# mfathulkr/MA-CJD-Cooperative-Jamming-Decision-Making-via-MARL

Hardware: AMD Instinct MI355X
Metric: env-steps/sec (all GPUs; batch_envs=4096/GPU, 3j/4r) (higher is better)
Workload: dtype f64; 1 GPU; 3 jammers / 4 radars, batch_envs=4096 per GPU, GRU hidden=64; mode=train, hidden=64, train_batch_episodes=32, updates_per_graph=20, hip_graphs=True, gemm_tuning=True, replay_capacity_episodes=8192, mixer_dtype=fp32, mixer=one MFMA launch per direction (f32)

## Files before the change

include/macjd_nets.h:

```cpp
#ifndef MACJD_NETS_H
#define MACJD_NETS_H

#include <stdint.h>

#include "macjd.h"

#ifdef __cplusplus
extern "C" {
#endif

typedef struct macjd_qhead_io {
    int64_t n_rows;
    int32_t H, A, n_agents, greedy_only;
    const float* base;  int64_t base_ld;
    const float* P_all; int64_t p_ld;
    const float* W1;    int64_t w1_ld;
    const float* w2;
    const float* b2;
    float* Q;           int64_t q_ld;
    const void* avail;  int32_t avail_elem_size, reserved;
    int64_t av_se, av_sj, av_sa;
    float epsilon;      float reserved2;
    uint64_t seed, counter;
    const float* eps_dev;
    const uint64_t* counter_dev;
    int32_t* T_out32;
    int64_t* T_out64;
    int64_t t32_se, t32_sj, t64_se, t64_sj;
    float* P_out;       int64_t po_se, po_sj;
    int64_t* argmax_out;
    const int64_t* gather_idx;
    float* q_gather_out;
} macjd_qhead_io;

int macjd_qhead_select(const macjd_qhead_io* io, void* hip_stream);

typedef struct macjd_gru_io {
    int32_t n_nets, B, T, J, H, reserved;
    const float* gi[2];
    const float* w_hh[2];
    const float* b_hh[2];
    const float* h0[2];
    float* h_out[2];
    int64_t h0_sb[2];
    const float* obs;      int64_t obs_sb, obs_sj;   int32_t S, reserved2;
    const int64_t* obs_index;
    const float* fc1_w[2]; const float* fc1_b[2];
    const float* w_ih[2];  const float* b_ih[2];
    float* p_out[2];
    const float* act_w[2][3]; const float* act_b[2][3];
    int32_t Ah, A;
} macjd_gru_io;

int macjd_gru_sequence(const macjd_gru_io* io, void* hip_stream);

typedef struct macjd_mixer_io {
    int64_t M;
    int32_t J, Em;
    const float* q;
    const float* w1_raw;
    const float* b1_raw;
    const float* wf_raw;
    const float* v_raw;
    float* y;
    const float* gy;
    float* gq;
    float* gw1_raw;
    float* gb1_raw;
    float* gwf_raw;
    float* gv_raw;
    int64_t b1_ld;
} macjd_mixer_io;

int macjd_mixer_tail_forward(const macjd_mixer_io* io, void* hip_stream);
int macjd_mixer_tail_backward(const macjd_mixer_io* io, void* hip_stream);

typedef struct macjd_tdloss_io {
    int32_t B, Tm1;
    float gamma, reserved;
    const float* y;
    const float* tq;
    int64_t y_sb, tq_sb;
    int64_t gy_sb, gy_cols;
    const float* reward;       int64_t r_sb, r_st;
    const uint8_t* terminated; int64_t t_sb, t_st;
    const uint8_t* filled;     int64_t f_sb, f_st;
    float* stats;
    float* gy;
} macjd_tdloss_io;

int macjd_td_loss(const macjd_tdloss_io* io, void* hip_stream);
int macjd_td_mask_sum(const macjd_tdloss_io* io, float* out, void* hip_stream);

typedef struct macjd_adam_io {
    int64_t n;
    float lr, beta1, beta2, eps, max_norm, reserved;
    float* param; float* grad ; float* exp_avg; float* exp_avg_sq;
    float* step; float* grad_norm; float* partials;
} macjd_adam_io;

int macjd_clip_adam_step(const macjd_adam_io* io, void* hip_stream);

typedef struct macjd_sampler_io {
    int64_t* idx_out;
    int32_t n, reserved;
    const int32_t* n_stored;
    int64_t* counter;
    uint64_t seed;
} macjd_sampler_io;

int macjd_sample_episodes(const macjd_sampler_io* io, void* hip_stream);
int macjd_clip_adam_step_sample(const macjd_adam_io* io, const macjd_sampler_io* next, void* hip_stream);

typedef struct macjd_wgrad_io {
    int64_t K;
    int32_t M, N;
    const float* gout; int64_t gout_ld;
    const float* inp;  int64_t inp_ld;
    float* dW;         int64_t dw_ld;
    float* db;
    float* workspace;
    const float* outer_vec;
    const float* outer_w;
} macjd_wgrad_io;

int64_t macjd_linear_wgrad_workspace_floats(int64_t K, int32_t M, int32_t N);
int macjd_linear_wgrad(const macjd_wgrad_io* io, void* hip_stream);
#define MACJD_WGRAD_MAX_BATCH 8
int macjd_linear_wgrad_many(const macjd_wgrad_io* ios, int32_t n, void* hip_stream);

typedef struct macjd_gather_io {
    int32_t n_tensors, n_rows;
    const int64_t* idx;
    const void* src[8]; void* dst[8]; int64_t row_bytes[8];
    int64_t dst_row_bytes[8];
} macjd_gather_io;

int macjd_gather_rows(const macjd_gather_io* io, void* hip_stream);

typedef struct macjd_qinput_io {
    int64_t n_rows;
    int32_t H, A;
    const float* h;   int64_t h_ld;
    const void* idx;  int32_t idx_elem_size, reserved;
    const float* P;
    float* out;       int64_t out_ld;
} macjd_qinput_io;

int macjd_qhead_input(const macjd_qinput_io* io, void* hip_stream);

typedef struct macjd_qtaken_io {
    int64_t n_rows;
    int32_t H, A;
    const float* h;   int64_t h_ld;
    const void* idx;  int32_t idx_elem_size, reserved;
    const float* P;
    const float* W1;  int64_t w1_ld;
    const float* b1;  const float* w2;  const float* b2;
    float* x;         int64_t x_ld;
    float* act;       int64_t act_ld;
    float* q;
} macjd_qtaken_io;

int macjd_qhead_taken_supported(int32_t H, int32_t A);
int macjd_qhead_taken(const macjd_qtaken_io* io, void* hip_stream);

typedef struct macjd_layernorm_io {
    int64_t M;
    int32_t S, reserved;
    float eps, reserved2;
    const float* x;  int64_t x_ld;
    const float* gamma;
    const float* beta;
    float* y;        int64_t y_ld;
    float* mean;
    float* rstd;
    float* xhat;     int64_t xhat_ld;
} macjd_layernorm_io;

int macjd_layernorm_forward(const macjd_layernorm_io* io, void* hip_stream);

typedef struct macjd_lnparam_io {
    int32_t C, K;
    const float* W;   int64_t w_ld;
    const float* G;   int64_t g_ld;
    const float* gb;
    float* dgamma;
    float* dbeta;
} macjd_lnparam_io;

int macjd_layernorm_param_grad(const macjd_lnparam_io* io, void* hip_stream);
int macjd_clip_adam_step_ln(const macjd_adam_io* io, const macjd_sampler_io* next, const macjd_lnparam_io* ln,
                            int64_t gamma_off, int64_t beta_off, void* hip_stream);

#define MACJD_ACT_NONE 0
#define MACJD_ACT_RELU 1
#define MACJD_ACT_SIGMOID 2
typedef struct macjd_mlp_io {
    int64_t n_rows;
    int32_t n_layers;
    int32_t dims[4];
    int32_t act[3];
    const float* W[3];
    const float* b[3];
    const float* x;  int64_t x_ld;
    float* y;        int64_t y_ld;
} macjd_mlp_io;

int macjd_mlp_forward(const macjd_mlp_io* io, void* hip_stream);
int macjd_mlp_forward_pair(const macjd_mlp_io* io0, const macjd_mlp_io* io1, void* hip_stream);

typedef struct macjd_splitrelu_bwd_io {
    int64_t M;
    int32_t n_blocks, Cp;
    int32_t width[4];
    const float* g[4];  int64_t g_ld[4];
    const float* g_pass; int64_t gp_ld;
    const float* act;   int64_t act_ld;
    float* gout;        int64_t gout_ld;
    const float* outer_w[4];
} macjd_splitrelu_bwd_io;

int macjd_splitrelu_backward(const macjd_splitrelu_bwd_io* io, void* hip_stream);

typedef struct macjd_rowdot_io {
    int64_t n_rows;
    int32_t K, reserved;
    const float* x;  int64_t x_ld;
    const float* w;
    const float* b;
    float* y;
} macjd_rowdot_io;

int macjd_rowdot(const macjd_rowdot_io* io, void* hip_stream);

typedef struct macjd_grugates_io {
    int64_t n_rows;
    int32_t H, reserved;
    const float* gi;  int64_t gi_ld;
    const float* gh;  int64_t gh_ld;
    const float* h;   int64_t h_ld;
    float* h_out;     int64_t ho_ld;
    float* h_out2;    int64_t ho2_ld;
} macjd_grugates_io;

int macjd_gru_gates(const macjd_grugates_io* io, void* hip_stream);

typedef struct macjd_mixerf_io {
    int64_t M;
    int32_t J, S, Hh, Em;
    int32_t save;
    int32_t operand_dtype;
    float ln_eps;  float reserved_f;
    const float* s;   int64_t s_ld;
    const float* q;
    const float* ln_w; const float* ln_b;
    const float* W1; const float* b1;
    const float* W2; const float* b2;
    const float* Wf2; const float* bf2;
    const float* wV2; const float* bV2;
    float* y;
    float* sn; float* xhat;
    float* act;
    const float* gy;
    float* gq;
    float* gout1;
    float* g_w1raw;
    float* g_wfraw;
    float* g_v;
} macjd_mixerf_io;

int macjd_mixer_fused_supported(int32_t J, int32_t S, int32_t Hh, int32_t Em);
int macjd_mixer_fused_forward(const macjd_mixerf_io* io, void* hip_stream);
int macjd_mixer_fused_forward_pair(const macjd_mixerf_io* saved, const macjd_mixerf_io* plain, void* hip_stream);
int macjd_mixer_fused_backward(const macjd_mixerf_io* io, void* hip_stream);
int macjd_mixer_fused_backward_td(const macjd_mixerf_io* io, const macjd_tdloss_io* td, const float* tot_m, void* hip_stream);
int macjd_mixer_fused_train(const macjd_mixerf_io* eval, const macjd_mixerf_io* target, const macjd_tdloss_io* td,
                            const float* tot_m, void* hip_stream);
typedef struct macjd_mixer_static_io {
    int64_t n_tiles;
    float* sn; float* xhat;
    float* act;
    float* gout1_sum;
    float* g_w1raw_sum;
    float* g_wfraw_sum;
    float* g_v_sum;
} macjd_mixer_static_io;
int macjd_mixer_fused_train_static(const macjd_mixerf_io* eval, const macjd_mixerf_io* target, const macjd_tdloss_io* td,
                                   const float* tot_m, const macjd_mixer_static_io* st, void* hip_stream);

typedef struct macjd_agent_episode_io {
// ... 98 lines not shown
```

ma-cjd-cooperative-jamming-decision-making-via-marl_amd/_native.py:

```python
from __future__ import annotations

import ctypes
import os
from typing import Optional

_PKG_DIR = os.path.dirname(os.path.abspath(__file__))
LIB_NAME = "libmacjd_hip.so"
LIB_PATH = os.environ.get("MACJD_LIB") or os.path.join(_PKG_DIR, LIB_NAME)

ABI_VERSION = 7
STEP_ARITH_F64 = 1
STEP_LANE_KERNEL = 2
STEP_SLOT_KERNEL = 4

EXPORTS = [
    "macjd_abi_version", "macjd_last_error", "macjd_reload_options", "macjd_device_count",
    "macjd_scenario_create", "macjd_scenario_destroy", "macjd_scenario_dims", "macjd_scenario_is_regular",
    "macjd_env_reset", "macjd_env_step", "macjd_env_step_timed",
    "macjd_qhead_select", "macjd_gru_sequence", "macjd_mixer_tail_forward", "macjd_mixer_tail_backward",
    "macjd_mlp_forward", "macjd_mlp_forward_pair", "macjd_td_loss", "macjd_clip_adam_step", "macjd_clip_adam_step_sample", "macjd_clip_adam_step_ln", "macjd_sample_episodes", "macjd_gather_rows",
    "macjd_linear_wgrad", "macjd_linear_wgrad_workspace_floats", "macjd_linear_wgrad_many", "macjd_qhead_input", "macjd_layernorm_forward", "macjd_layernorm_param_grad", "macjd_gru_gates", "macjd_rowdot", "macjd_splitrelu_backward",
    "macjd_mixer_fused_supported", "macjd_mixer_fused_forward", "macjd_mixer_fused_backward", "macjd_mixer_fused_backward_td", "macjd_td_mask_sum",
    "macjd_agent_episode_supported", "macjd_agent_episode", "macjd_env_step_many", "macjd_env_step_many_timed",
    "macjd_qhead_double_q_supported", "macjd_qhead_double_q", "macjd_qhead_taken_supported", "macjd_qhead_taken",
    "macjd_qheads_pair", "macjd_mixer_fused_forward_pair", "macjd_mixer_fused_train", "macjd_mixer_fused_train_static",
    "macjd_scenario_set_scan", "macjd_env_step_scan", "macjd_env_reset_scan",
    "macjd_agent_env_episode_scan_supported", "macjd_agent_env_episode_scan",
    "macjd_scenario_set_scan_pattern",
    "macjd_gru_sequence_backward_supported", "macjd_gru_sequence_backward",
]


class NativeLibraryError(RuntimeError):
    pass


class StepIO(ctypes.Structure):
    _fields_ = [
        ("n_envs", ctypes.c_int64), ("env_offset", ctypes.c_int64), ("seed", ctypes.c_uint64),
        ("flags", ctypes.c_uint32), ("reserved", ctypes.c_uint32),
        ("T", ctypes.c_void_p), ("T_se", ctypes.c_int64), ("T_sx", ctypes.c_int64),
        ("P32", ctypes.c_void_p), ("P64", ctypes.c_void_p), ("P_se", ctypes.c_int64), ("P_sx", ctypes.c_int64),
        ("u", ctypes.c_void_p), ("u_se", ctypes.c_int64), ("u_sx", ctypes.c_int64),
        ("episode", ctypes.c_void_p),
        ("track", ctypes.c_void_p), ("k_se", ctypes.c_int64), ("k_sx", ctypes.c_int64),
        ("step", ctypes.c_void_p),
        ("reward", ctypes.c_void_p), ("r_dpj", ctypes.c_void_p), ("terminated", ctypes.c_void_p),
        ("pd", ctypes.c_void_p), ("pd_se", ctypes.c_int64), ("pd_sx", ctypes.c_int64),
        ("snr_with", ctypes.c_void_p), ("sw_se", ctypes.c_int64), ("sw_sx", ctypes.c_int64),
        ("out64", ctypes.c_void_p), ("pd64", ctypes.c_void_p), ("snr64", ctypes.c_void_p),
        ("prj64", ctypes.c_void_p),
        ("pe_tables", ctypes.c_void_p), ("pe_flags", ctypes.c_void_p), ("pe_stride", ctypes.c_int64),
        ("pe_tile", ctypes.c_int32), ("reserved_pe", ctypes.c_int32),
        ("r_dpj_sum", ctypes.c_void_p),
    ]


class ScanDesc(ctypes.Structure):
    _fields_ = [
        ("n_radars", ctypes.c_int32), ("n_jammers", ctypes.c_int32),
        ("half_beam", ctypes.c_void_p), ("sweep", ctypes.c_void_p), ("sweep_mod", ctypes.c_void_p),
        ("full", ctypes.c_void_p), ("az0", ctypes.c_void_p), ("bear_tgt", ctypes.c_void_p), ("bear_jam", ctypes.c_void_p),
        ("GaPs_side", ctypes.c_void_p), ("snr_no", ctypes.c_void_p), ("snr_no_side", ctypes.c_void_p),
        ("pd_no_side", ctypes.c_void_p), ("gr_side", ctypes.c_void_p),
    ]


class ScanPatternDesc(ctypes.Structure):
    _fields_ = [
        ("n_radars", ctypes.c_int32), ("n_levels", ctypes.c_int32),
        ("inv_width", ctypes.c_void_p), ("GaPs_lvl", ctypes.c_void_p), ("snr_no_lvl", ctypes.c_void_p),
        ("pd_no_lvl", ctypes.c_void_p), ("gr_lvl", ctypes.c_void_p),
    ]


class ScanIO(ctypes.Structure):
    _fields_ = [
        ("theta_a", ctypes.c_void_p), ("a_se", ctypes.c_int64), ("a_sx", ctypes.c_int64),
        ("state", ctypes.c_void_p), ("st_se", ctypes.c_int64), ("st_col0", ctypes.c_int32), ("st_col_step", ctypes.c_int32),
        ("snr_no", ctypes.c_void_p), ("sn_se", ctypes.c_int64), ("sn_sx", ctypes.c_int64),
    ]


class QheadIO(ctypes.Structure):
    _fields_ = [
        ("n_rows", ctypes.c_int64),
        ("H", ctypes.c_int32), ("A", ctypes.c_int32), ("n_agents", ctypes.c_int32), ("greedy_only", ctypes.c_int32),
        ("base", ctypes.c_void_p), ("base_ld", ctypes.c_int64),
        ("P_all", ctypes.c_void_p), ("p_ld", ctypes.c_int64),
        ("W1", ctypes.c_void_p), ("w1_ld", ctypes.c_int64),
        ("w2", ctypes.c_void_p), ("b2", ctypes.c_void_p),
        ("Q", ctypes.c_void_p), ("q_ld", ctypes.c_int64),
        ("avail", ctypes.c_void_p), ("avail_elem_size", ctypes.c_int32), ("reserved", ctypes.c_int32),
        ("av_se", ctypes.c_int64), ("av_sj", ctypes.c_int64), ("av_sa", ctypes.c_int64),
        ("epsilon", ctypes.c_float), ("reserved2", ctypes.c_float),
        ("seed", ctypes.c_uint64), ("counter", ctypes.c_uint64),
        ("eps_dev", ctypes.c_void_p), ("counter_dev", ctypes.c_void_p),
        ("T_out32", ctypes.c_void_p), ("T_out64", ctypes.c_void_p),
        ("t32_se", ctypes.c_int64), ("t32_sj", ctypes.c_int64), ("t64_se", ctypes.c_int64), ("t64_sj", ctypes.c_int64),
        ("P_out", ctypes.c_void_p), ("po_se", ctypes.c_int64), ("po_sj", ctypes.c_int64),
        ("argmax_out", ctypes.c_void_p), ("gather_idx", ctypes.c_void_p), ("q_gather_out", ctypes.c_void_p),
    ]


class GruIO(ctypes.Structure):
    _fields_ = [
        ("n_nets", ctypes.c_int32), ("B", ctypes.c_int32), ("T", ctypes.c_int32), ("J", ctypes.c_int32),
        ("H", ctypes.c_int32), ("reserved", ctypes.c_int32),
        ("gi", ctypes.c_void_p * 2), ("w_hh", ctypes.c_void_p * 2), ("b_hh", ctypes.c_void_p * 2),
        ("h0", ctypes.c_void_p * 2), ("h_out", ctypes.c_void_p * 2), ("h0_sb", ctypes.c_int64 * 2),
        ("obs", ctypes.c_void_p), ("obs_sb", ctypes.c_int64), ("obs_sj", ctypes.c_int64), ("S", ctypes.c_int32), ("reserved2", ctypes.c_int32),
        ("obs_index", ctypes.c_void_p),
        ("fc1_w", ctypes.c_void_p * 2), ("fc1_b", ctypes.c_void_p * 2), ("w_ih", ctypes.c_void_p * 2), ("b_ih", ctypes.c_void_p * 2),
        ("p_out", ctypes.c_void_p * 2), ("act_w", (ctypes.c_void_p * 3) * 2), ("act_b", (ctypes.c_void_p * 3) * 2),
        ("Ah", ctypes.c_int32), ("A", ctypes.c_int32),
    ]


class GruBwdIO(ctypes.Structure):
    _fields_ = [
        ("B", ctypes.c_int32), ("T", ctypes.c_int32), ("J", ctypes.c_int32), ("H", ctypes.c_int32),
        ("gi", ctypes.c_void_p), ("gh", ctypes.c_void_p), ("h_all", ctypes.c_void_p),
        ("h0", ctypes.c_void_p), ("h0_sb", ctypes.c_int64),
        ("w_hh", ctypes.c_void_p), ("dh_all", ctypes.c_void_p),
        ("dgi", ctypes.c_void_p), ("dgh", ctypes.c_void_p), ("dh0", ctypes.c_void_p),
    ]


class MixerIO(ctypes.Structure):
    _fields_ = [
        ("M", ctypes.c_int64), ("J", ctypes.c_int32), ("Em", ctypes.c_int32),
        ("q", ctypes.c_void_p), ("w1_raw", ctypes.c_void_p), ("b1_raw", ctypes.c_void_p),
        ("wf_raw", ctypes.c_void_p), ("v_raw", ctypes.c_void_p), ("y", ctypes.c_void_p),
        ("gy", ctypes.c_void_p), ("gq", ctypes.c_void_p), ("gw1_raw", ctypes.c_void_p),
        ("gb1_raw", ctypes.c_void_p), ("gwf_raw", ctypes.c_void_p), ("gv_raw", ctypes.c_void_p),
        ("b1_ld", ctypes.c_int64),
    ]


class MixerFusedIO(ctypes.Structure):
    _fields_ = [
        ("M", ctypes.c_int64), ("J", ctypes.c_int32), ("S", ctypes.c_int32), ("Hh", ctypes.c_int32), ("Em", ctypes.c_int32),
        ("save", ctypes.c_int32), ("operand_dtype", ctypes.c_int32), ("ln_eps", ctypes.c_float), ("reserved_f", ctypes.c_float),
        ("s", ctypes.c_void_p), ("s_ld", ctypes.c_int64), ("q", ctypes.c_void_p),
        ("ln_w", ctypes.c_void_p), ("ln_b", ctypes.c_void_p), ("W1", ctypes.c_void_p), ("b1", ctypes.c_void_p),
        ("W2", ctypes.c_void_p), ("b2", ctypes.c_void_p), ("Wf2", ctypes.c_void_p), ("bf2", ctypes.c_void_p),
        ("wV2", ctypes.c_void_p), ("bV2", ctypes.c_void_p),
        ("y", ctypes.c_void_p), ("sn", ctypes.c_void_p), ("xhat", ctypes.c_void_p), ("act", ctypes.c_void_p),
        ("gy", ctypes.c_void_p), ("gq", ctypes.c_void_p), ("gout1", ctypes.c_void_p), ("g_w1raw", ctypes.c_void_p),
        ("g_wfraw", ctypes.c_void_p), ("g_v", ctypes.c_void_p),
    ]


class MixerStaticIO(ctypes.Structure):
    _fields_ = [
        ("n_tiles", ctypes.c_int64), ("sn", ctypes.c_void_p), ("xhat", ctypes.c_void_p), ("act", ctypes.c_void_p),
        ("gout1_sum", ctypes.c_void_p), ("g_w1raw_sum", ctypes.c_void_p), ("g_wfraw_sum", ctypes.c_void_p),
        ("g_v_sum", ctypes.c_void_p),
    ]


class AgentEpisodeIO(ctypes.Structure):
    _fields_ = [
        ("n_envs", ctypes.c_int64), ("T", ctypes.c_int32), ("J", ctypes.c_int32), ("H", ctypes.c_int32), ("A", ctypes.c_int32),
        ("greedy_only", ctypes.c_int32), ("reserved", ctypes.c_int32),
        ("gi", ctypes.c_void_p), ("gi_ld", ctypes.c_int64), ("P_all", ctypes.c_void_p), ("p_ld", ctypes.c_int64),
        ("h0", ctypes.c_void_p), ("w_hh", ctypes.c_void_p), ("b_hh", ctypes.c_void_p),
        ("W1", ctypes.c_void_p), ("w1_ld", ctypes.c_int64), ("b1", ctypes.c_void_p), ("w2", ctypes.c_void_p), ("b2", ctypes.c_void_p),
        ("avail", ctypes.c_void_p), ("avail_elem_size", ctypes.c_int32), ("reserved2", ctypes.c_int32),
        ("av_se", ctypes.c_int64), ("av_sj", ctypes.c_int64), ("av_sa", ctypes.c_int64),
        ("eps", ctypes.c_void_p), ("seed", ctypes.c_uint64), ("counter_base", ctypes.c_void_p),
        ("hidden", ctypes.c_void_p), ("T_out", ctypes.c_void_p), ("P_out", ctypes.c_void_p), ("h_final", ctypes.c_void_p),
    ]


class AgentEnvEpisodeScanIO(ctypes.Structure):
    _fields_ = [
        ("n_envs", ctypes.c_int64), ("env_offset", ctypes.c_int64),
        ("T", ctypes.c_int32), ("J", ctypes.c_int32), ("R", ctypes.c_int32), ("H", ctypes.c_int32), ("A", ctypes.c_int32),
        ("S", ctypes.c_int32), ("actor_hidden", ctypes.c_int32), ("greedy_only", ctypes.c_int32),
        ("h0", ctypes.c_void_p), ("fc1_w", ctypes.c_void_p), ("fc1_b", ctypes.c_void_p),
        ("w_ih", ctypes.c_void_p), ("b_ih", ctypes.c_void_p), ("w_hh", ctypes.c_void_p), ("b_hh", ctypes.c_void_p),
        ("a1_w", ctypes.c_void_p), ("a1_b", ctypes.c_void_p), ("a2_w", ctypes.c_void_p), ("a2_b", ctypes.c_void_p),
        ("a3_w", ctypes.c_void_p), ("a3_b", ctypes.c_void_p),
        ("W1", ctypes.c_void_p), ("w1_ld", ctypes.c_int64), ("b1", ctypes.c_void_p), ("w2", ctypes.c_void_p), ("b2", ctypes.c_void_p),
        ("avail", ctypes.c_void_p), ("avail_elem_size", ctypes.c_int32), ("reserved", ctypes.c_int32),
        ("av_se", ctypes.c_int64), ("av_sj", ctypes.c_int64), ("av_sa", ctypes.c_int64),
        ("eps", ctypes.c_void_p), ("seed", ctypes.c_uint64), ("counter_base", ctypes.c_void_p),
        ("env_seed", ctypes.c_uint64), ("episode", ctypes.c_void_p),
        ("track", ctypes.c_void_p), ("k_se", ctypes.c_int64), ("k_sx", ctypes.c_int64), ("step", ctypes.c_void_p),
        ("scan", ScanIO), ("pe_tables", ctypes.c_void_p),
        ("hidden", ctypes.c_void_p), ("T_out", ctypes.c_void_p), ("P_out", ctypes.c_void_p), ("h_final", ctypes.c_void_p),
        ("st_state", ctypes.c_void_p), ("st_obs", ctypes.c_void_p), ("reward", ctypes.c_void_p), ("terminated", ctypes.c_void_p),
        ("rdpj_sum", ctypes.c_void_p),
    ]


class DoubleQIO(ctypes.Structure):
    _fields_ = [
        ("n_rows", ctypes.c_int64), ("H", ctypes.c_int32), ("A", ctypes.c_int32),
        ("h_e", ctypes.c_void_p), ("he_ld", ctypes.c_int64), ("h_t", ctypes.c_void_p), ("ht_ld", ctypes.c_int64),
        ("P_e", ctypes.c_void_p), ("pe_ld", ctypes.c_int64), ("P_t", ctypes.c_void_p), ("pt_ld", ctypes.c_int64),
        ("W1_e", ctypes.c_void_p), ("w1e_ld", ctypes.c_int64), ("b1_e", ctypes.c_void_p), ("w2_e", ctypes.c_void_p), ("b2_e", ctypes.c_void_p),
        ("W1_t", ctypes.c_void_p), ("w1t_ld", ctypes.c_int64), ("b1_t", ctypes.c_void_p), ("w2_t", ctypes.c_void_p), ("b2_t", ctypes.c_void_p),
        ("out", ctypes.c_void_p), ("argmax_out", ctypes.c_void_p), ("p_group", ctypes.c_int64), ("p_inner", ctypes.c_int64),
    ]


class QinputIO(ctypes.Structure):
    _fields_ = [
        ("n_rows", ctypes.c_int64), ("H", ctypes.c_int32), ("A", ctypes.c_int32),
        ("h", ctypes.c_void_p), ("h_ld", ctypes.c_int64),
        ("idx", ctypes.c_void_p), ("idx_elem_size", ctypes.c_int32), ("reserved", ctypes.c_int32),
        ("P", ctypes.c_void_p), ("out", ctypes.c_void_p), ("out_ld", ctypes.c_int64),
    ]


class GruGatesIO(ctypes.Structure):
    _fields_ = [
        ("n_rows", ctypes.c_int64), ("H", ctypes.c_int32), ("reserved", ctypes.c_int32),
        ("gi", ctypes.c_void_p), ("gi_ld", ctypes.c_int64), ("gh", ctypes.c_void_p), ("gh_ld", ctypes.c_int64),
        ("h", ctypes.c_void_p), ("h_ld", ctypes.c_int64),
        ("h_out", ctypes.c_void_p), ("ho_ld", ctypes.c_int64), ("h_out2", ctypes.c_void_p), ("ho2_ld", ctypes.c_int64),
    ]


class RowdotIO(ctypes.Structure):
    _fields_ = [
        ("n_rows", ctypes.c_int64), ("K", ctypes.c_int32), ("reserved", ctypes.c_int32),
        ("x", ctypes.c_void_p), ("x_ld", ctypes.c_int64), ("w", ctypes.c_void_p), ("b", ctypes.c_void_p),
        ("y", ctypes.c_void_p),
    ]


class SplitReluBwdIO(ctypes.Structure):
    _fields_ = [
        ("M", ctypes.c_int64), ("n_blocks", ctypes.c_int32), ("Cp", ctypes.c_int32), ("width", ctypes.c_int32 * 4),
        ("g0", ctypes.c_void_p), ("g1", ctypes.c_void_p), ("g2", ctypes.c_void_p), ("g3", ctypes.c_void_p),
        ("g_ld", ctypes.c_int64 * 4),
        ("g_pass", ctypes.c_void_p), ("gp_ld", ctypes.c_int64),
        ("act", ctypes.c_void_p), ("act_ld", ctypes.c_int64), ("gout", ctypes.c_void_p), ("gout_ld", ctypes.c_int64),
        ("ow0", ctypes.c_void_p), ("ow1", ctypes.c_void_p), ("ow2", ctypes.c_void_p), ("ow3", ctypes.c_void_p),
    ]


class LayerNormIO(ctypes.Structure):
    _fields_ = [
        ("M", ctypes.c_int64), ("S", ctypes.c_int32), ("reserved", ctypes.c_int32),
        ("eps", ctypes.c_float), ("reserved2", ctypes.c_float),
        ("x", ctypes.c_void_p), ("x_ld", ctypes.c_int64), ("gamma", ctypes.c_void_p), ("beta", ctypes.c_void_p),
        ("y", ctypes.c_void_p), ("y_ld", ctypes.c_int64), ("mean", ctypes.c_void_p), ("rstd", ctypes.c_void_p),
        ("xhat", ctypes.c_void_p), ("xhat_ld", ctypes.c_int64),
    ]


class LnParamIO(ctypes.Structure):
    _fields_ = [
        ("C", ctypes.c_int32), ("K", ctypes.c_int32),
        ("W", ctypes.c_void_p), ("w_ld", ctypes.c_int64), ("G", ctypes.c_void_p), ("g_ld", ctypes.c_int64),
        ("gb", ctypes.c_void_p), ("dgamma", ctypes.c_void_p), ("dbeta", ctypes.c_void_p),
    ]


class MlpIO(ctypes.Structure):
    _fields_ = [
        ("n_rows", ctypes.c_int64), ("n_layers", ctypes.c_int32), ("dims", ctypes.c_int32 * 4),
        ("act", ctypes.c_int32 * 3), ("W", ctypes.c_void_p * 3), ("b", ctypes.c_void_p * 3),
        ("x", ctypes.c_void_p), ("x_ld", ctypes.c_int64), ("y", ctypes.c_void_p), ("y_ld", ctypes.c_int64),
    ]


class TdLossIO(ctypes.Structure):
    _fields_ = [
        ("B", ctypes.c_int32), ("Tm1", ctypes.c_int32), ("gamma", ctypes.c_float), ("reserved", ctypes.c_float),
        ("y", ctypes.c_void_p), ("tq", ctypes.c_void_p),
        ("y_sb", ctypes.c_int64), ("tq_sb", ctypes.c_int64), ("gy_sb", ctypes.c_int64), ("gy_cols", ctypes.c_int64),
        ("reward", ctypes.c_void_p), ("r_sb", ctypes.c_int64), ("r_st", ctypes.c_int64),
        ("terminated", ctypes.c_void_p), ("t_sb", ctypes.c_int64), ("t_st", ctypes.c_int64),
        ("filled", ctypes.c_void_p), ("f_sb", ctypes.c_int64), ("f_st", ctypes.c_int64),
        ("stats", ctypes.c_void_p), ("gy", ctypes.c_void_p),
    ]


class AdamIO(ctypes.Structure):
    _fields_ = [
        ("n", ctypes.c_int64), ("lr", ctypes.c_float), ("beta1", ctypes.c_float), ("beta2", ctypes.c_float),
        ("eps", ctypes.c_float), ("max_norm", ctypes.c_float), ("reserved", ctypes.c_float),
        ("param", ctypes.c_void_p), ("grad", ctypes.c_void_p), ("exp_avg", ctypes.c_void_p),
        ("exp_avg_sq", ctypes.c_void_p), ("step", ctypes.c_void_p), ("grad_norm", ctypes.c_void_p),
        ("partials", ctypes.c_void_p),
    ]


class QtakenIO(ctypes.Structure):
    _fields_ = [
        ("n_rows", ctypes.c_int64), ("H", ctypes.c_int32), ("A", ctypes.c_int32),
        ("h", ctypes.c_void_p), ("h_ld", ctypes.c_int64),
        ("idx", ctypes.c_void_p), ("idx_elem_size", ctypes.c_int32), ("reserved", ctypes.c_int32),
        ("P", ctypes.c_void_p),
        ("W1", ctypes.c_void_p), ("w1_ld", ctypes.c_int64),
        ("b1", ctypes.c_void_p), ("w2", ctypes.c_void_p), ("b2", ctypes.c_void_p),
        ("x", ctypes.c_void_p), ("x_ld", ctypes.c_int64),
        ("act", ctypes.c_void_p), ("act_ld", ctypes.c_int64),
        ("q", ctypes.c_void_p),
    ]


class SamplerIO(ctypes.Structure):
    _fields_ = [
        ("idx_out", ctypes.c_void_p), ("n", ctypes.c_int32), ("reserved", ctypes.c_int32),
        ("n_stored", ctypes.c_void_p), ("counter", ctypes.c_void_p), ("seed", ctypes.c_uint64),
    ]


class GatherIO(ctypes.Structure):
    _fields_ = [
        ("n_tensors", ctypes.c_int32), ("n_rows", ctypes.c_int32), ("idx", ctypes.c_void_p),
        ("src", ctypes.c_void_p * 8), ("dst", ctypes.c_void_p * 8), ("row_bytes", ctypes.c_int64 * 8),
        ("dst_row_bytes", ctypes.c_int64 * 8),
    ]


class WgradIO(ctypes.Structure):
    _fields_ = [
        ("K", ctypes.c_int64), ("M", ctypes.c_int32), ("N", ctypes.c_int32),
        ("gout", ctypes.c_void_p), ("gout_ld", ctypes.c_int64), ("inp", ctypes.c_void_p), ("inp_ld", ctypes.c_int64),
        ("dW", ctypes.c_void_p), ("dw_ld", ctypes.c_int64), ("db", ctypes.c_void_p), ("workspace", ctypes.c_void_p),
        ("outer_vec", ctypes.c_void_p), ("outer_w", ctypes.c_void_p),
    ]


_lib: Optional[ctypes.CDLL] = None


def load() -> ctypes.CDLL:
    global _lib
    if _lib is not None:
        return _lib
    if not os.path.exists(LIB_PATH):
        raise NativeLibraryError(
            f"{LIB_PATH} not found. Build it with `python -c 'import __graft_entry__ as g; g.build()'` "
            f"(hipcc --offload-arch=gfx950). There is no CPU fallback for the environment step.")
    try:
        lib = ctypes.CDLL(LIB_PATH)
    except OSError as e:
        raise NativeLibraryError(f"cannot load {LIB_PATH}: {e}") from e
    lib.macjd_abi_version.restype = ctypes.c_int
    lib.macjd_last_error.restype = ctypes.c_char_p
    lib.macjd_device_count.restype = ctypes.c_int
    lib.macjd_reload_options.restype = None
    lib.macjd_scenario_create.restype = ctypes.c_int
    lib.macjd_scenario_create.argtypes = [ctypes.c_void_p, ctypes.POINTER(ctypes.c_void_p)]
    lib.macjd_scenario_destroy.restype = None
    lib.macjd_scenario_destroy.argtypes = [ctypes.c_void_p]
    lib.macjd_scenario_is_regular.restype = ctypes.c_int
    lib.macjd_scenario_is_regular.argtypes = [ctypes.c_void_p]
    lib.macjd_scenario_dims.restype = ctypes.c_int
    lib.macjd_scenario_dims.argtypes = [ctypes.c_void_p] + [ctypes.POINTER(ctypes.c_int32)] * 3
    lib.macjd_env_reset.restype = ctypes.c_int
    lib.macjd_env_reset.argtypes = [ctypes.c_void_p, ctypes.c_int64, ctypes.c_void_p, ctypes.c_int64, ctypes.c_int64,
                                    ctypes.c_void_p, ctypes.c_void_p, ctypes.c_void_p, ctypes.c_void_p]
    lib.macjd_env_step.restype = ctypes.c_int
    lib.macjd_scenario_set_scan.restype = ctypes.c_int
    lib.macjd_scenario_set_scan.argtypes = [ctypes.c_void_p, ctypes.POINTER(ScanDesc)]
    lib.macjd_scenario_set_scan_pattern.restype = ctypes.c_int
    lib.macjd_scenario_set_scan_pattern.argtypes = [ctypes.c_void_p, ctypes.POINTER(ScanPatternDesc)]
    lib.macjd_env_step_scan.restype = ctypes.c_int
    lib.macjd_env_step_scan.argtypes = [ctypes.c_void_p, ctypes.POINTER(StepIO), ctypes.POINTER(ScanIO), ctypes.c_void_p]
    lib.macjd_env_reset_scan.restype = ctypes.c_int
    lib.macjd_env_reset_scan.argtypes = [ctypes.c_void_p, ctypes.c_int64, ctypes.POINTER(ScanIO), ctypes.c_void_p, ctypes.c_void_p]
    lib.macjd_env_step.argtypes = [ctypes.c_void_p, ctypes.POINTER(StepIO), ctypes.c_void_p]
    lib.macjd_env_step_timed.restype = ctypes.c_int
    lib.macjd_env_step_timed.argtypes = [ctypes.c_void_p, ctypes.POINTER(StepIO), ctypes.c_int, ctypes.c_void_p,
                                         ctypes.POINTER(ctypes.c_float)]
    lib.macjd_qhead_select.restype = ctypes.c_int
    lib.macjd_qhead_select.argtypes = [ctypes.POINTER(QheadIO), ctypes.c_void_p]
    lib.macjd_gru_sequence.restype = ctypes.c_int
    lib.macjd_gru_sequence.argtypes = [ctypes.POINTER(GruIO), ctypes.c_void_p]
    lib.macjd_gru_sequence_backward_supported.restype = ctypes.c_int
    lib.macjd_gru_sequence_backward_supported.argtypes = [ctypes.c_int32]
    lib.macjd_gru_sequence_backward.restype = ctypes.c_int
    lib.macjd_gru_sequence_backward.argtypes = [ctypes.POINTER(GruBwdIO), ctypes.c_void_p]
    for name in ("macjd_mixer_tail_forward", "macjd_mixer_tail_backward"):
        getattr(lib, name).restype = ctypes.c_int
        getattr(lib, name).argtypes = [ctypes.POINTER(MixerIO), ctypes.c_void_p]
    lib.macjd_qhead_double_q_supported.restype = ctypes.c_int
    lib.macjd_qhead_double_q_supported.argtypes = [ctypes.c_int32] * 2
    lib.macjd_qhead_double_q.restype = ctypes.c_int
    lib.macjd_qhead_double_q.argtypes = [ctypes.POINTER(DoubleQIO), ctypes.c_void_p]
    lib.macjd_agent_episode_supported.restype = ctypes.c_int
    lib.macjd_agent_episode_supported.argtypes = [ctypes.c_int32] * 3
    lib.macjd_agent_episode.restype = ctypes.c_int
    lib.macjd_agent_episode.argtypes = [ctypes.POINTER(AgentEpisodeIO), ctypes.c_void_p]
    lib.macjd_agent_env_episode_scan_supported.restype = ctypes.c_int
    lib.macjd_agent_env_episode_scan_supported.argtypes = [ctypes.c_int32] * 4
    lib.macjd_agent_env_episode_scan.restype = ctypes.c_int
    lib.macjd_agent_env_episode_scan.argtypes = [ctypes.c_void_p, ctypes.POINTER(AgentEnvEpisodeScanIO), ctypes.c_void_p]
    lib.macjd_env_step_many.restype = ctypes.c_int
    lib.macjd_env_step_many.argtypes = [ctypes.c_void_p, ctypes.POINTER(StepIO), ctypes.c_int32, ctypes.c_int64, ctypes.c_void_p]
    lib.macjd_env_step_many_timed.restype = ctypes.c_int
    lib.macjd_env_step_many_timed.argtypes = [ctypes.c_void_p, ctypes.POINTER(StepIO), ctypes.c_int32, ctypes.c_int64, ctypes.c_int,
                                              ctypes.c_void_p, ctypes.POINTER(ctypes.c_float)]
    lib.macjd_mixer_fused_supported.restype = ctypes.c_int
    lib.macjd_mixer_fused_supported.argtypes = [ctypes.c_int32] * 4
    for name in ("macjd_mixer_fused_forward", "macjd_mixer_fused_backward"):
        getattr(lib, name).restype = ctypes.c_int
        getattr(lib, name).argtypes = [ctypes.POINTER(MixerFusedIO), ctypes.c_void_p]
    lib.macjd_mixer_fused_backward_td.restype = ctypes.c_int
    lib.macjd_mixer_fused_backward_td.argtypes = [ctypes.POINTER(MixerFusedIO), ctypes.POINTER(TdLossIO), ctypes.c_void_p, ctypes.c_void_p]
    lib.macjd_mixer_fused_train.restype = ctypes.c_int
    lib.macjd_mixer_fused_train.argtypes = [ctypes.POINTER(MixerFusedIO), ctypes.POINTER(MixerFusedIO), ctypes.POINTER(TdLossIO),
                                            ctypes.c_void_p, ctypes.c_void_p]
    lib.macjd_mixer_fused_train_static.restype = ctypes.c_int
    lib.macjd_mixer_fused_train_static.argtypes = [ctypes.POINTER(MixerFusedIO), ctypes.POINTER(MixerFusedIO), ctypes.POINTER(TdLossIO),
                                                   ctypes.c_void_p, ctypes.POINTER(MixerStaticIO), ctypes.c_void_p]
    lib.macjd_td_mask_sum.restype = ctypes.c_int
    lib.macjd_td_mask_sum.argtypes = [ctypes.POINTER(TdLossIO), ctypes.c_void_p, ctypes.c_void_p]
    lib.macjd_qhead_taken_supported.restype = ctypes.c_int
    lib.macjd_qhead_taken_supported.argtypes = [ctypes.c_int32, ctypes.c_int32]
    lib.macjd_qhead_taken.restype = ctypes.c_int
    lib.macjd_qhead_taken.argtypes = [ctypes.POINTER(QtakenIO), ctypes.c_void_p]
    lib.macjd_qheads_pair.restype = ctypes.c_int
    lib.macjd_qheads_pair.argtypes = [ctypes.POINTER(QtakenIO), ctypes.POINTER(DoubleQIO), ctypes.c_void_p]
    lib.macjd_mixer_fused_forward_pair.restype = ctypes.c_int
    lib.macjd_mixer_fused_forward_pair.argtypes = [ctypes.POINTER(MixerFusedIO), ctypes.POINTER(MixerFusedIO), ctypes.c_void_p]
    lib.macjd_qhead_input.restype = ctypes.c_int
    lib.macjd_qhead_input.argtypes = [ctypes.POINTER(QinputIO), ctypes.c_void_p]
    lib.macjd_layernorm_forward.restype = ctypes.c_int
    lib.macjd_layernorm_forward.argtypes = [ctypes.POINTER(LayerNormIO), ctypes.c_void_p]
    lib.macjd_gru_gates.restype = ctypes.c_int
    lib.macjd_gru_gates.argtypes = [ctypes.POINTER(GruGatesIO), ctypes.c_void_p]
    lib.macjd_splitrelu_backward.restype = ctypes.c_int
    lib.macjd_splitrelu_backward.argtypes = [ctypes.POINTER(SplitReluBwdIO), ctypes.c_void_p]
    lib.macjd_layernorm_param_grad.restype = ctypes.c_int
    lib.macjd_layernorm_param_grad.argtypes = [ctypes.POINTER(LnParamIO), ctypes.c_void_p]
    lib.macjd_rowdot.restype = ctypes.c_int
    lib.macjd_rowdot.argtypes = [ctypes.POINTER(RowdotIO), ctypes.c_void_p]
    lib.macjd_mlp_forward_pair.restype = ctypes.c_int
    lib.macjd_mlp_forward_pair.argtypes = [ctypes.POINTER(MlpIO), ctypes.POINTER(MlpIO), ctypes.c_void_p]
    lib.macjd_mlp_forward.restype = ctypes.c_int
    lib.macjd_mlp_forward.argtypes = [ctypes.POINTER(MlpIO), ctypes.c_void_p]
    lib.macjd_td_loss.restype = ctypes.c_int
    lib.macjd_td_loss.argtypes = [ctypes.POINTER(TdLossIO), ctypes.c_void_p]
    lib.macjd_clip_adam_step.restype = ctypes.c_int
    lib.macjd_clip_adam_step.argtypes = [ctypes.POINTER(AdamIO), ctypes.c_void_p]
    lib.macjd_clip_adam_step_sample.restype = ctypes.c_int
    lib.macjd_clip_adam_step_sample.argtypes = [ctypes.POINTER(AdamIO), ctypes.POINTER(SamplerIO), ctypes.c_void_p]
    lib.macjd_clip_adam_step_ln.restype = ctypes.c_int
    lib.macjd_clip_adam_step_ln.argtypes = [ctypes.POINTER(AdamIO), ctypes.POINTER(SamplerIO), ctypes.POINTER(LnParamIO),
                                            ctypes.c_int64, ctypes.c_int64, ctypes.c_void_p]
    lib.macjd_sample_episodes.restype = ctypes.c_int
    lib.macjd_sample_episodes.argtypes = [ctypes.POINTER(SamplerIO), ctypes.c_void_p]
    lib.macjd_gather_rows.restype = ctypes.c_int
    lib.macjd_gather_rows.argtypes = [ctypes.POINTER(GatherIO), ctypes.c_void_p]
    lib.macjd_linear_wgrad.restype = ctypes.c_int
    lib.macjd_linear_wgrad.argtypes = [ctypes.POINTER(WgradIO), ctypes.c_void_p]
    lib.macjd_linear_wgrad_many.restype = ctypes.c_int
    lib.macjd_linear_wgrad_many.argtypes = [ctypes.POINTER(WgradIO), ctypes.c_int32, ctypes.c_void_p]
    lib.macjd_linear_wgrad_workspace_floats.restype = ctypes.c_int64
    lib.macjd_linear_wgrad_workspace_floats.argtypes = [ctypes.c_int64, ctypes.c_int32, ctypes.c_int32]
    if lib.macjd_abi_version() != ABI_VERSION:
        raise NativeLibraryError(f"{LIB_NAME}: ABI version {lib.macjd_abi_version()} != expected {ABI_VERSION}")
    _lib = lib
    return lib


def reload_options() -> None:
    load().macjd_reload_options()


def check(rc: int, what: str) -> None:
    if rc != 0:
        msg = load().macjd_last_error()
        raise NativeLibraryError(f"{what} failed ({rc}): {msg.decode() if msg else ''}")


class ScenarioHandle:

    def __init__(self, scenario):
        lib = load()
        desc, keep = scenario.c_desc()
        h = ctypes.c_void_p()
        check(lib.macjd_scenario_create(ctypes.addressof(desc), ctypes.byref(h)), "macjd_scenario_create")
        del keep
        self._h = h
        self._lib = lib
        if getattr(scenario, "scanning", False):
            sdesc, skeep = scenario.c_scan_desc()
            check(lib.macjd_scenario_set_scan(h, ctypes.byref(sdesc)), "macjd_scenario_set_scan")
            del skeep
            if getattr(scenario, "scan_pattern_levels", 0):
                pdesc, pkeep = scenario.c_scan_pattern_desc()
                check(lib.macjd_scenario_set_scan_pattern(h, ctypes.byref(pdesc)), "macjd_scenario_set_scan_pattern")
                del pkeep

    @property
    def ptr(self):
        return self._h

    def close(self):
        if getattr(self, "_h", None):
            self._lib.macjd_scenario_destroy(self._h)
            self._h = None

    def __del__(self):
        try:
            self.close()
        except Exception:
            pass
```

ma-cjd-cooperative-jamming-decision-making-via-marl_amd/core/qmix.py:

```python
from __future__ import annotations

import copy
import os

import numpy as np
import torch
import torch.nn.functional as F
import torch.optim as optim

from .. import hipgraph, ops, options
from .networks import QMixer


def _to(x, dtype, device):
    if isinstance(x, torch.Tensor):
        return x.to(device=device, dtype=dtype)
    return torch.as_tensor(np.asarray(x), device=device).to(dtype)


class QMixLearner:
    def __init__(self, mac, args):
        self.args = args
        self.mac = mac
        self.n_agents = args.n_agents
# ... 479 lines not shown
            if side_work is not None:
                side_work()
            if sums_late is not None:
                sums_late()
            if stats_done is not None:
                torch.cuda.current_stream(eval_q_tot.device).wait_event(stats_done)
                for t_ in (self._last_stats4,):
                    t_.record_stream(torch.cuda.current_stream(eval_q_tot.device))
        else:
            loss, eval_mean, target_mean = ops.td_loss_full(eval_q_tot, target_q_tot, st["reward"], st["terminated"],
                                                            st["filled"], self.args.gamma, T - 1, 1)
            loss.backward()
        if self._world_size() > 1 or self._flat_param is not None:
            self._flatten_grads()
        return loss.detach(), eval_mean.detach(), target_mean.detach()

    def _clip_and_step(self, sample_next=None):
        if self._flat_param is not None:
            g = self.optimizer.param_groups[0]
            held, self._held_ln = getattr(self, "_held_ln", None), None
            ops.clip_adam_step(self._flat_param, self._flat_grad, self._flat_exp_avg, self._flat_exp_avg_sq,
                               self._adam_step, self._grad_norm, self._adam_partials, g["lr"], g["betas"], g["eps"],
                               self.args.grad_norm_clip, sample_next=sample_next, lnparam=held)
            return self._grad_norm
        grad_norm = torch.nn.utils.clip_grad_norm_(self.params, self.args.grad_norm_clip)
        self.optimizer.step()
        return grad_norm.detach() if torch.is_tensor(grad_norm) else torch.as_tensor(grad_norm)

    def _after_step(self):
        if (self.train_step - self.last_target_update_step) >= self.args.target_update_interval:
            self._update_targets()
            self.last_target_update_step = self.train_step

    def _pack_stats(self, loss, grad_norm, ev, tg, sync_stats):
        stats = {"loss": loss, "grad_norm": grad_norm, "eval_qtot_avg": ev, "target_qtot_avg": tg}
        if sync_stats:
            stacked = torch.stack([torch.as_tensor(v, device=self.device, dtype=torch.float32).reshape(())
                                   for v in stats.values()])
            stats = dict(zip(stats.keys(), stacked.tolist()))
        return stats

    def train(self, batch, train_info=None, sync_stats=True):
        self.train_step += 1
        loss, ev, tg = self._forward_backward(batch, int(batch["max_seq_len"]))
        self._allreduce_grads()
        grad_norm = self._clip_and_step()
        if self.train_agent_body:
            for m in (self.mac, self.target_mac):
                m.invalidate_static_inputs()
        self._after_step()
        if not sync_stats and torch.is_tensor(grad_norm) and grad_norm is self._grad_norm_tensor():
            grad_norm = grad_norm.clone()
        return self._pack_stats(loss, grad_norm, ev, tg, sync_stats)

    def _grad_norm_tensor(self):
        return getattr(self, "_grad_norm", None)

    def enable_graphs(self, buffer, batch_size, warmup_iters=3, force_two_graphs=False, updates_per_graph=None,
                      graphed_allreduce=None, prime=True):
        if self.device.type != "cuda":
            raise RuntimeError("enable_graphs needs the learner on a HIP device")
        if self.train_agent_body:
            raise RuntimeError("enable_graphs: train_agent_body is an eager-mode option (the captured, static-observation "
                               "and shared-body updates are built on the frozen agent body); use train()")
        self.release_graphs()
        self._verify_body_shared()
        same_buffer = getattr(self, "_g_buffer", None) is buffer
        self._g_buffer, self._g_B, self._g_T = buffer, int(batch_size), int(buffer.episode_limit)
        self._g_obs_static = bool(getattr(buffer, "obs_static", False)) and options.on("LEARNER_STATIC_OBS")
        self._g_state_static = self._g_obs_static and bool(getattr(buffer, "state_static", False))
        self._g_mixer_static = False
        self._g_actor_in_scan = options.on("ACTOR_IN_SCAN")
        self._g_scan_from_ring = self._g_obs_static and int(buffer.buffers["obs"].shape[-1]) <= 3 * int(self.args.rnn_hidden_dim)
        prev_idx = getattr(self, "_g_idx", None)
        keep_idx = same_buffer and prev_idx is not None and prev_idx.numel() == self._g_B and prev_idx.device == self.device
        self._g_idx = prev_idx if keep_idx else torch.zeros(self._g_B, dtype=torch.int64, device=self.device)
        self._g_dev_sampler = self._flat_param is not None and options.on("DEVICE_SAMPLER")
        if not keep_idx:
            self._g_n_stored = torch.zeros(1, dtype=torch.int32, device=self.device)
        if getattr(self, "_g_draws", None) is None:
            self._g_draws = torch.full((1,), int(getattr(self, "_resume_draws", 0)), dtype=torch.int64, device=self.device)
        if not keep_idx:
            self._g_pop_seen = None
            self._g_idx_fresh = False
        self._g_idx_ring = [(torch.zeros(self._g_B, dtype=torch.int64).pin_memory(), torch.cuda.Event()) for _ in range(8)]
        if buffer.current_size < 1:
            raise RuntimeError("enable_graphs: the replay buffer is empty")

        keys = [k for k in buffer.buffers if k != "avail_actions"]
        srcs = [buffer.buffers[k] for k in keys]
        fused = ops.gather_rows_supported(srcs) and self._g_T >= 2
        if fused:
            T1 = self._g_T + 1
            padded = ("actions_discrete", "actions_continuous")
            stage = {k: torch.zeros((self._g_B, T1 if k in padded else v.shape[1]) + tuple(v.shape[2:]), dtype=v.dtype,
                                    device=v.device) for k, v in zip(keys, srcs)}

        def body_a():
            if fused:
                pre = (None, None)
                if self._g_scan_from_ring and options.get("UPDATE_STREAMS") != "1":
                    pre = self._scan_from_ring_early()
                ops.gather_rows(self._g_idx, srcs, [stage[k] for k in keys])
                return self._forward_backward_full(stage, self._g_T, pre_scan=pre[0], pre_actor=pre[1])
            b = {k: v.index_select(0, self._g_idx) for k, v in zip(keys, srcs)}
            return self._forward_backward(b, self._g_T, validate_actions=False)

        self._graph_body_a = body_a

        was_shared = self._body_is_shared()
        snap_p = [p.detach().clone() for p in self.params]
        snap_o = {id(p): {k: v.clone() for k, v in st.items() if torch.is_tensor(v)}
                  for p, st in self.optimizer.state.items()}
        s = torch.cuda.Stream(device=self.device)
        s.wait_stream(torch.cuda.current_stream(self.device))
        with torch.cuda.stream(s):
            for _ in range(max(1, warmup_iters)):
                body_a()
                self._clip_and_step()
        torch.cuda.current_stream(self.device).wait_stream(s)
        def restore_training_state():
            with torch.no_grad():
                for p, sp in zip(self.params, snap_p):
                    p.copy_(sp)
                for p, st in self.optimizer.state.items():
                    for k, v in st.items():
                        if torch.is_tensor(v):
                            old = snap_o.get(id(p), {}).get(k)
                            v.copy_(old) if old is not None else v.zero_()
            if was_shared:
                self._mark_body_shared()

        restore_training_state()
        self._graph_a, self._graph_b = torch.cuda.CUDAGraph(), torch.cuda.CUDAGraph()
        self._g_graphed_ar = bool(graphed_allreduce if graphed_allreduce is not None
                                  else options.get("GRAPHED_ALLREDUCE") == "1") and self._ar_capturable()
        self._g_single = (self._world_size() <= 1 and not force_two_graphs) or self._g_graphed_ar
        with hipgraph.capture(self._graph_a):
            self._g_out_a = body_a()
            st4 = getattr(self, "_last_stats4", None) if fused else None
            if st4 is not None and st4.numel() == 4:
                self._grad_norm = st4[3]
            self._g_stats4 = st4 if (st4 is not None and st4.numel() == 4) else None
            nxt = (self._g_idx, self._g_n_stored, self._g_draws, self._sampler_seed()) if self._g_dev_sampler else None
            if self._g_single:
                if self._g_graphed_ar:
                    self._allreduce_grads(force=True)
                self._g_out_b = self._clip_and_step(sample_next=nxt)
        if not self._g_single:
            with hipgraph.capture(self._graph_b, pool=self._graph_a.pool()):
                self._g_out_b = self._clip_and_step(sample_next=nxt)
        K = int(updates_per_graph if updates_per_graph is not None else options.get("UPDATES_PER_GRAPH"))
        self._g_multi = None
        if K > 1 and self._g_single and self._g_dev_sampler and fused and self._g_stats4 is not None:
            gm, rows, single_norm = torch.cuda.CUDAGraph(), [], self._grad_norm
            pipelined = (self._g_scan_from_ring and self._g_actor_in_scan and options.get("UPDATE_STREAMS") != "1"
                         and options.on("PIPELINED_GROUP"))
            stage2 = {k: torch.zeros_like(v) for k, v in stage.items()} if pipelined else None
            stages = [stage, stage2]
            self._g_stages = stages
            origin_dev = self.device

            def prefetch(dst, fork=True, draw=True):
                origin = torch.cuda.current_stream(origin_dev)
                ts = self._target_stream
                if isinstance(fork, torch.cuda.Event):
                    ts.wait_event(fork)
                elif fork:
                    ts.wait_stream(origin)
                shared = self._body_is_shared()
                agents = [self.mac.agent] if shared else [self.target_mac.agent, self.mac.agent]
                with torch.cuda.stream(ts), torch.no_grad():
                    if draw:
                        ops.sample_episodes(self._g_idx, self._g_n_stored, self._g_draws, self._sampler_seed())
                    ops.gather_rows(self._g_idx, srcs, [dst[k] for k in keys])
                    tot_m = ops.td_mask_sum(dst["filled"], self._g_T - 1)
                    ev_g = torch.cuda.Event()
                    ev_g.record(ts)
                    h, ps = ops.gru_sequence_from_obs(buffer.buffers["obs"], self._g_idx, agents, self._g_B, self.n_agents,
                                                      self._g_T + 1, with_actor=True)
                    ev_s = torch.cuda.Event()
                    ev_s.record(ts)
                return (([h[0], h[0]] if shared else h), ([ps[0], ps[0]] if shared else ps), (ev_g, ev_s, tot_m))

            with hipgraph.capture(gm, pool=self._graph_a.pool()):
                nxt_batch = None
                for k_upd in range(K):
                    last = k_upd == K - 1
                    box = {}
                    hook = (lambda fork=True: box.__setitem__("next", prefetch(stages[(k_upd + 1) % 2], fork))) if (pipelined and not last) else None
                    if pipelined and nxt_batch is not None:
                        h_pre, p_pre, evs = nxt_batch
                        self._forward_backward_full(stages[k_upd % 2], self._g_T, pre_scan=h_pre, pre_actor=p_pre,
                                                    prefetched=evs, after_join=hook)
                    elif pipelined:
                        pre = self._scan_from_ring_early()
                        ops.gather_rows(self._g_idx, srcs, [stage[k] for k in keys])
                        if self._paired_heads_ok(stage, self._g_T):
                            tot_m0 = ops.td_mask_sum(stage["filled"], self._g_T - 1)
                            scan_done = torch.cuda.Event()
                            scan_done.record(self._target_stream)
                            self._forward_backward_full(stage, self._g_T, pre_scan=pre[0], pre_actor=pre[1],
                                                        prefetched=(None, scan_done, tot_m0), after_join=hook)
                        else:
                            self._forward_backward_full(stage, self._g_T, pre_scan=pre[0], pre_actor=pre[1], after_join=hook)
                    else:
                        body_a()
                    nxt_batch = box.get("next")
                    rows.append(self._last_stats4)
                    self._grad_norm = rows[-1][3]
                    if self._g_graphed_ar:
                        self._allreduce_grads(force=True)
                    self._clip_and_step(sample_next=None if nxt_batch is not None else nxt)
                if pipelined:
                    torch.cuda.current_stream(self.device).wait_stream(self._target_stream)
            self._grad_norm = single_norm
            self._g_multi = (K, gm, rows)
            self._g_pipelined = pipelined
        self._g_shared_body = self._body_is_shared()
        assert self._g_obs_static == (bool(getattr(buffer, "obs_static", False)) and options.on("LEARNER_STATIC_OBS"))
        if prime:
            keep = (self._g_draws.clone(), self._g_idx.clone(), self._g_n_stored.clone())
            self._g_n_stored.fill_(int(buffer.current_size))
            self._g_idx.clamp_(0, max(0, int(buffer.current_size) - 1))
            hipgraph.replay(self._graph_a, self.device)
            if not self._g_single:
                self._allreduce_grads()
                hipgraph.replay(self._graph_b, self.device)
            if self._g_multi is not None:
                self._g_idx.clamp_(0, max(0, int(buffer.current_size) - 1))
                hipgraph.replay(self._g_multi[1], self.device)
            torch.cuda.synchronize(self.device)
            restore_training_state()
            self._g_draws.copy_(keep[0]); self._g_idx.copy_(keep[1]); self._g_n_stored.copy_(keep[2])
        self._graphs_ready = True

    def release_graphs(self):
        graphs = []
        m = getattr(self, "_g_multi", None)
        if m is not None:
            graphs.append(m[1])
        graphs += [getattr(self, "_graph_b", None), getattr(self, "_graph_a", None)]
        self._graphs_ready = False
        self._g_multi = self._g_stages = None
        self._graph_a = self._graph_b = None
        self._graph_body_a = None
        self._g_out_a = self._g_out_b = self._g_stats4 = self._last_stats4 = self._held_ln = None
        if self._flat_param is not None and any(g is not None for g in graphs):
            self._grad_norm = torch.zeros((), dtype=torch.float32, device=self._flat_param.device)
        hipgraph.destroy(graphs, self.device)

    def train_from_buffer(self, indices=None, sync_stats=True, stats_row=None):
        buf = self._g_buffer if getattr(self, "_graphs_ready", False) else None
        if buf is None:
            raise RuntimeError("call enable_graphs(buffer, batch_size) first")
        device_draw = False
        if indices is None:
            if buf.current_size < self._g_B:
                return self._snap(self.train(buf.sample(self._g_B), None, sync_stats=sync_stats), stats_row)
            device_draw = self._g_dev_sampler and self._population_full_length(buf)
            if not device_draw:
                indices = self._sample_rng.choice(buf.current_size, self._g_B, replace=False)
        if not device_draw:
            indices = np.asarray(indices, dtype=np.int64)
            if len(indices) != self._g_B or int(buf.episode_lengths[indices].min()) != self._g_T:
                return self._snap(self.train(buf.sample(len(indices), indices=indices), None, sync_stats=sync_stats), stats_row)
        if self._g_obs_static and not buf.obs_static:
            raise RuntimeError("an episode with unknown / changing observations was stored after enable_graphs() captured "
                               "the static-observation update: call enable_graphs() again")
        if self._g_shared_body and not self._body_is_shared():
            raise RuntimeError("the agent body (fc1 / GRU / actor) of one controller changed after enable_graphs() captured "
                               "the shared-body update: call enable_graphs() again")
        self.train_step += 1
        if device_draw:
            self._device_draw_ready(buf)
        else:
            k = self.train_step % len(self._g_idx_ring)
            slot, ev = self._g_idx_ring[k]
            ev.synchronize()
            slot.numpy()[:] = indices
            self._g_idx.copy_(slot, non_blocking=True)
            ev.record()
        hipgraph.replay(self._graph_a, self.device)
        self._g_idx_fresh = self._g_dev_sampler and (buf.store_count, buf.current_size) == self._g_pop_seen
        if not self._g_single:
            self._allreduce_grads()
            hipgraph.replay(self._graph_b, self.device)
        self._after_step()
        loss, ev, tg = self._g_out_a
        if stats_row is not None and not sync_stats and self._g_stats4 is not None:
            stats_row.copy_(self._g_stats4, non_blocking=True)
            return {"loss": stats_row[0], "grad_norm": stats_row[3], "eval_qtot_avg": stats_row[1], "target_qtot_avg": stats_row[2]}
        return self._snap(self._pack_stats(loss, self._g_out_b, ev, tg, sync_stats), stats_row)

    def _device_draw_ready(self, buf):
        pop = (buf.store_count, buf.current_size)
        if pop != self._g_pop_seen:
            self._g_n_stored.fill_(buf.current_size)
            self._g_pop_seen, self._g_idx_fresh = pop, False
        if not self._g_idx_fresh:
            ops.sample_episodes(self._g_idx, self._g_n_stored, self._g_draws, self._sampler_seed())

    def train_from_buffer_many(self, n, stats_out=None):
        buf = self._g_buffer if getattr(self, "_graphs_ready", False) else None
        if buf is None:
            raise RuntimeError("call enable_graphs(buffer, batch_size) first")
        out, done = [], 0
        while done < n:
            m = self._g_multi
            until_sync = self.args.target_update_interval - (self.train_step - self.last_target_update_step)
            if (m is not None and n - done >= m[0] and until_sync >= m[0] and buf.current_size >= self._g_B
                    and self._population_full_length(buf) and (not self._g_obs_static or buf.obs_static)
                    and (not self._g_shared_body or self._body_is_shared())):
                self._device_draw_ready(buf)
                self.train_step += m[0]
                hipgraph.replay(m[1], self.device)
                self._g_idx_fresh = (buf.store_count, buf.current_size) == self._g_pop_seen
                self._after_step()
                if stats_out is not None:
                    torch.stack(m[2], out=stats_out[done:done + m[0]])
                out += m[2]
                done += m[0]
            else:
                row = stats_out[done] if stats_out is not None else torch.empty(4, dtype=torch.float32, device=self.device)
                self.train_from_buffer(sync_stats=False, stats_row=row)
                out.append(row)
                done += 1
        return out if stats_out is None else stats_out

    def _sampler_seed(self):
        return getattr(self, "_sampler_seed_value", int(getattr(self.args, "seed", 0) or 0))

    def _population_full_length(self, buf):
        key = (buf.store_count, buf.current_size)
        if getattr(self, "_g_full_key", None) != key:
            self._g_full_key = key
            self._g_full = bool((buf.episode_lengths[:buf.current_size] == self._g_T).all())
        return self._g_full

    @staticmethod
    def _snap(stats, stats_row):
        if stats_row is None or not torch.is_tensor(stats["loss"]):
            return stats
        order = ("loss", "eval_qtot_avg", "target_qtot_avg", "grad_norm")
        torch.stack([torch.as_tensor(stats[k], device=stats_row.device, dtype=torch.float32).reshape(()) for k in order],
                    out=stats_row)
        return {k: stats_row[i] for i, k in enumerate(order)}

    def _all_action_q_multi(self, macs, obs, keep_final_hidden=True):
        B, T, J, S = obs.shape
        rows = obs.reshape(B * T * J, S)
        shared = len(macs) == 2 and self._body_is_shared() and {id(m) for m in macs} == {id(self.mac), id(self.target_mac)}
        body_macs = [self.mac] if shared else list(macs)
        side = None
        if rows.is_cuda:
            if getattr(self, "_side_stream", None) is None:
                self._side_stream = torch.cuda.Stream(device=rows.device)
            side, main = self._side_stream, torch.cuda.current_stream(rows.device)
            side.wait_stream(main)
            with torch.cuda.stream(side):
                params = [m.agent.actor_forward(rows) for m in body_macs]
        else:
            params = [m.agent.actor_forward(rows) for m in body_macs]
        gis = [m.agent.gru_input_transform(rows).view(B, T, J, 3 * m.agent.rnn_hidden_dim) for m in body_macs]
        h_alls = ops.gru_sequence_multi(gis, [m.agent.rnn.weight_hh for m in body_macs],
                                        [m.agent.rnn.bias_hh for m in body_macs])
# ... 59 lines not shown
```

ma-cjd-cooperative-jamming-decision-making-via-marl_amd/csrc/macjd_nets.hip:

```cpp
#include <hip/hip_runtime.h>
#include <math.h>
#include <stdint.h>
#include <stdio.h>
#include <stdlib.h>
#include <string.h>
#include <type_traits>

#include "../../include/macjd.h"
#include "../../include/macjd_nets.h"
#include "macjd_err.h"
#include "macjd_tdloss.h"
#include "macjd_philox.h"
#include "macjd_gru_math.h"

namespace macjd {

static int set_nets_err(int code, const char* msg) { return set_err(code, "%s", msg); }

__device__ __forceinline__ bool avail_at(const macjd_qhead_io& io, int64_t e, int j, int a) {
    if (!io.avail) return true;
    const int64_t off = e * io.av_se + (int64_t)j * io.av_sj + (int64_t)a * io.av_sa;
    return (io.avail_elem_size == 8) ? (((const int64_t*)io.avail)[off] != 0)
                                     : (((const int32_t*)io.avail)[off] != 0);
}
// ... 42 lines not shown
            const float* __restrict__ wrow = io.W1 + (int64_t)h * io.w1_ld + H;
            const float wp = wrow[A];
            const float w2h = io.w2[h];
#pragma unroll
            for (int a = 0; a < AMAX; ++a) {
                if (!AT && a >= A) break;
                float t = b4[k] + wrow[a];
                t = fmaf(p[a], wp, t);
                t = fmaxf(t, 0.0f);
                acc[a] = fmaf(t, w2h, acc[a]);
            }
        }
    }
    if (HS > 1) {
        const int lane = threadIdx.x & 63;
        if (wave > 0) {
#pragma unroll
            for (int a = 0; a < AMAX; ++a) {
                if (!AT && a >= A) break;
                s_part[((wave - 1) * AMAX + a) * 64 + lane] = acc[a];
            }
        }
        __syncthreads();
        if (wave > 0 || !row_live) return;
        if constexpr (AMAX > 17) {
#pragma unroll 1
            for (int w = 0; w < HS - 1; ++w)
#pragma unroll
                for (int a = 0; a < AMAX; ++a) {
                    if (!AT && a >= A) break;
                    acc[a] += s_part[(w * AMAX + a) * 64 + lane];
                }
        } else {
#pragma unroll
            for (int w = 0; w < HS - 1; ++w)
#pragma unroll
                for (int a = 0; a < AMAX; ++a) {
                    if (!AT && a >= A) break;
                    acc[a] += s_part[(w * AMAX + a) * 64 + lane];
                }
        }
    }
    const float b2 = io.b2[0];
#pragma unroll
    for (int a = 0; a < AMAX; ++a) {
        if (!AT && a >= A) break;
        acc[a] += b2;
        if (io.Q) io.Q[n * io.q_ld + a] = acc[a];
    }
    if (io.argmax_out) {
        int am = 0;
        float aq = acc[0];
#pragma unroll
        for (int a = 1; a < AMAX; ++a) {
            if (!AT && a >= A) break;
            if (acc[a] > aq) { aq = acc[a]; am = a; }
        }
        io.argmax_out[n] = am;
    }
    if (io.gather_idx && io.q_gather_out) {
        const int64_t gi = io.gather_idx[n];
        float gq = 0.0f;
#pragma unroll
        for (int a = 0; a < AMAX; ++a) {
            if (!AT && a >= A) break;
            gq = ((int64_t)a == gi) ? acc[a] : gq;
        }
        io.q_gather_out[n] = gq;
    }
    if (!io.T_out32 && !io.T_out64) return;

    const int64_t e = n / io.n_agents;
    const int j = (int)(n - e * io.n_agents);
    int best = 0, n_avail = 0;
    float bestq = -INFINITY;
    uint64_t avail_bits = 0;
#pragma unroll
    for (int a = 0; a < AMAX; ++a) {
        if (!AT && a >= A) break;
        const bool av = avail_at(io, e, j, a);
        avail_bits |= av ? (1ull << a) : 0ull;
        n_avail += av ? 1 : 0;
        const float q = av ? acc[a] : -INFINITY;
        if (q > bestq) { bestq = q; best = a; }
    }
    int chosen = best;
    const float epsilon = io.eps_dev ? io.eps_dev[0] : io.epsilon;
    if (!io.greedy_only && epsilon > 0.0f) {
        const uint64_t counter = io.counter + (io.counter_dev ? io.counter_dev[0] : 0ull);
        const Philox4 r = philox4x32_10((uint32_t)n, (uint32_t)((uint64_t)n >> 32), (uint32_t)counter,
                                        (uint32_t)(counter >> 32), (uint32_t)io.seed, (uint32_t)(io.seed >> 32));
        const float u_pick = (float)(r.v[0] >> 8) * (1.0f / 16777216.0f);
        if (u_pick < epsilon) {
            const int pool = n_avail > 0 ? n_avail : A;
            int k = (int)(((uint64_t)r.v[1] * (uint64_t)pool) >> 32);
            chosen = 0;
#pragma unroll
            for (int a = 0; a < AMAX; ++a) {
                if (!AT && a >= A) break;
                const bool av = (n_avail > 0) ? ((avail_bits >> a) & 1ull) : true;
                if (av) { if (k == 0) chosen = a; --k; }
            }
        }
    }
    float pc = 0.0f;
#pragma unroll
    for (int a = 0; a < AMAX; ++a) pc = (a == chosen) ? p[a] : pc;
    if (io.T_out32) io.T_out32[e * io.t32_se + (int64_t)j * io.t32_sj] = chosen;
    if (io.T_out64) io.T_out64[e * io.t64_se + (int64_t)j * io.t64_sj] = chosen;
    if (io.P_out) io.P_out[e * io.po_se + (int64_t)j * io.po_sj] = pc;
}

}

extern "C" int macjd_qhead_select(const macjd_qhead_io* io, void* hip_stream) {
    using namespace macjd;
    if (!io) return set_nets_err(MACJD_EINVAL, "macjd_qhead_select: NULL io");
    if (io->n_rows < 0 || io->H < 1 || io->A < 1 || io->A > 64 || io->n_agents < 1)
        return set_nets_err(MACJD_EINVAL, "macjd_qhead_select: bad n_rows / H / A / n_agents (A <= 64)");
    if (!io->base || !io->P_all || !io->W1 || !io->w2 || !io->b2)
        return set_nets_err(MACJD_EINVAL, "macjd_qhead_select: NULL input");
    if (!io->Q && !io->T_out32 && !io->T_out64 && !io->argmax_out && !(io->gather_idx && io->q_gather_out))
        return set_nets_err(MACJD_EINVAL, "macjd_qhead_select: no output requested");
    if (io->avail && io->avail_elem_size != 4 && io->avail_elem_size != 8)
        return set_nets_err(MACJD_EINVAL, "macjd_qhead_select: avail_elem_size must be 4 or 8");
    if (io->n_rows == 0) return MACJD_OK;
    hipStream_t s = (hipStream_t)hip_stream;
    const bool split = io->n_rows < (1 << 16) && io->H >= 16;
#define MACJD_QHEAD_LAUNCH(AT)                                                                                    \
    do {                                                                                                          \
        if (split)                                                                                                \
            hipLaunchKernelGGL((qhead_select_kernel<AT, QHEAD_HS>), dim3((unsigned)((io->n_rows + 63) / 64)),     \
                               dim3(64 * QHEAD_HS), 0, s, *io);                                                   \
        else                                                                                                      \
            hipLaunchKernelGGL((qhead_select_kernel<AT, 1>), dim3((unsigned)((io->n_rows + 255) / 256)), dim3(256), \
                               0, s, *io);                                                                        \
    } while (0)
    switch (io->A) {
        case 5:  MACJD_QHEAD_LAUNCH(5); break;
        case 7:  MACJD_QHEAD_LAUNCH(7); break;
        case 9:  MACJD_QHEAD_LAUNCH(9); break;
        case 17: MACJD_QHEAD_LAUNCH(17); break;
        case 33: MACJD_QHEAD_LAUNCH(33); break;
        default: MACJD_QHEAD_LAUNCH(0); break;
    }
#undef MACJD_QHEAD_LAUNCH
    hipError_t err = hipGetLastError();
    if (err != hipSuccess) return set_nets_err(MACJD_EDEVICE, hipGetErrorString(err));
    return MACJD_OK;
}

namespace macjd {

template <int H, int NW>
__device__ __forceinline__ void scan_prologue(const macjd_gru_io& io, const int net, const int b, const int j,
                                              float* __restrict__ s_pro, float* __restrict__ s_gi, const int lane,
                                              const int wave, const bool want_gi, const bool want_actor) {
    float* xs = s_pro;
    float* v1 = s_pro + 256;
    float* v2 = s_pro + 512;
    const int64_t row = io.obs_index ? io.obs_index[b] : (int64_t)b;
    const float* x = io.obs + row * io.obs_sb + (int64_t)j * io.obs_sj;
    const int S = io.S;
    for (int k = threadIdx.x; k < S; k += 64 * NW) xs[k] = x[k];
    __syncthreads();
    auto matvec = [&](const float* __restrict__ W, const float* __restrict__ bias, const float* __restrict__ vin, int K,
                      int N, auto&& store) {
        auto body = [&](auto nch_c) {
            constexpr int NCH = decltype(nch_c)::value;
            constexpr int UN = 16 / NCH;
            float xv[NCH];
#pragma unroll
            for (int c = 0; c < NCH; ++c) {
                const int k = lane + 64 * c;
                xv[c] = (k < K) ? vin[k] : 0.0f;
            }
            for (int o0 = wave * UN; o0 < N; o0 += NW * UN) {
                float wv[UN][NCH], a[UN];
#pragma unroll
                for (int uu = 0; uu < UN; ++uu) {
                    const int o = (o0 + uu < N) ? o0 + uu : N - 1;
                    const float* wr = W + (int64_t)o * K;
#pragma unroll
                    for (int c = 0; c < NCH; ++c) {
                        const int k = lane + 64 * c;
                        wv[uu][c] = wr[k < K ? k : K - 1];
                    }
                }
#pragma unroll
                for (int uu = 0; uu < UN; ++uu) {
                    float t = 0.0f;
#pragma unroll
                    for (int c = 0; c < NCH; ++c) t = fmaf(wv[uu][c], xv[c], t);
                    a[uu] = wave_sum(t);
                }
                float mine = 0.0f;
#pragma unroll
                for (int uu = 0; uu < UN; ++uu) mine = (lane == uu) ? a[uu] : mine;
                if (lane < UN && o0 + lane < N) store(o0 + lane, mine + bias[o0 + lane]);
            }
        };
        const int nch = (K + 63) / 64;
        if (nch == 1) body(std::integral_constant<int, 1>{});
        else if (nch == 2) body(std::integral_constant<int, 2>{});
        else body(std::integral_constant<int, 4>{});
    };
    if (want_gi) {
        matvec(io.fc1_w[net], io.fc1_b[net], xs, S, H, [&](int o, float v) { v1[o] = fmaxf(v, 0.0f); });
        __syncthreads();
        matvec(io.w_ih[net], io.b_ih[net], v1, H, 3 * H, [&](int o, float v) { s_gi[o] = v; });
    }
    if (want_actor && io.p_out[net]) {
        const int Ah = io.Ah, A = io.A;
        __syncthreads();
        matvec(io.act_w[net][0], io.act_b[net][0], xs, S, Ah, [&](int o, float v) { v1[o] = fmaxf(v, 0.0f); });
        __syncthreads();
        matvec(io.act_w[net][1], io.act_b[net][1], v1, Ah, Ah, [&](int o, float v) { v2[o] = fmaxf(v, 0.0f); });
        __syncthreads();
        float* po = io.p_out[net] + ((int64_t)b * io.J + j) * A;
        matvec(io.act_w[net][2], io.act_b[net][2], v2, Ah, A, [&](int o, float v) { po[o] = 1.0f / (1.0f + expf(-v)); });
    }
    __syncthreads();
}

template <int H, int NW>
__global__ void __launch_bounds__(64 * NW) gru_sequence_kernel(const macjd_gru_io io) {
    constexpr int U = H / 64;
    constexpr int KW = H / NW;
    const int lane = threadIdx.x & 63;
    const int wave = __builtin_amdgcn_readfirstlane(threadIdx.x >> 6);
    const int net = blockIdx.y;
    const int seq = blockIdx.x;
    const int b = seq / io.J, j = seq - b * io.J;
    const int T = io.T;
    const float* __restrict__ gi = io.gi[net];
    const float* __restrict__ whh = io.w_hh[net];
    const float* __restrict__ bhh = io.b_hh[net];
    float* __restrict__ out = io.h_out[net];

    __shared__ float s_part[2][NW][3][H];
    __shared__ float s_gi[3 * H];
    __shared__ float s_pro[768];
    if (blockIdx.z == 1) {
        scan_prologue<H, NW>(io, net, b, j, s_pro, s_gi, lane, wave, false, true);
        return;
    }

    float w[3][U][KW];
#pragma unroll
    for (int g = 0; g < 3; ++g)
#pragma unroll
        for (int i = 0; i < U; ++i) {
            const float* row = whh + (int64_t)(g * H + lane + 64 * i) * H + wave * KW;
#pragma unroll
            for (int kk = 0; kk < KW; kk += 4) {
                const float4 v = *reinterpret_cast<const float4*>(row + kk);
                w[g][i][kk] = v.x; w[g][i][kk + 1] = v.y; w[g][i][kk + 2] = v.z; w[g][i][kk + 3] = v.w;
            }
        }
    float bias[3][U], h[U], ring[3][3][U];
#pragma unroll
    for (int i = 0; i < U; ++i) {
        const int u = lane + 64 * i;
#pragma unroll
        for (int g = 0; g < 3; ++g) bias[g][i] = bhh[g * H + u];
        h[i] = io.h0[net] ? io.h0[net][(int64_t)b * (io.h0_sb[net] ? io.h0_sb[net] : (int64_t)io.J * H) + (int64_t)j * H + u] : 0.0f;
    }
    const bool gi_inkernel = io.obs != nullptr;
    const bool gi_static = io.reserved != 0 || gi_inkernel;
    if (gi_inkernel) scan_prologue<H, NW>(io, net, b, j, s_pro, s_gi, lane, wave, true, gridDim.z == 1);
    auto gi_row = [&](int t) -> const float* {
        return gi_inkernel ? (const float*)s_gi
                           : gi_static ? gi + ((int64_t)b * io.J + j) * (3 * H)
                                       : gi + (((int64_t)b * T + t) * io.J + j) * (3 * H);
    };
    if (T > 0) {
        const float* r0 = gi_row(0);
        const float* r1 = gi_row(T > 1 ? 1 : 0);
#pragma unroll
        for (int g = 0; g < 3; ++g)
#pragma unroll
            for (int i = 0; i < U; ++i) {
                ring[0][g][i] = r0[g * H + lane + 64 * i];
                ring[1][g][i] = r1[g * H + lane + 64 * i];
            }
    }

    auto step = [&](auto slot_c, int t) {
        constexpr int SLOT = decltype(slot_c)::value;
        constexpr int PRE = (SLOT + 2) % 3;
        {
            const float* rn = gi_row(t + 2 < T ? t + 2 : T - 1);
#pragma unroll
            for (int g = 0; g < 3; ++g)
#pragma unroll
                for (int i = 0; i < U; ++i) ring[PRE][g][i] = rn[g * H + lane + 64 * i];
        }
        float acc[3][U];
#pragma unroll
        for (int g = 0; g < 3; ++g)
#pragma unroll
            for (int i = 0; i < U; ++i) acc[g][i] = 0.0f;
#pragma unroll
        for (int kk = 0; kk < KW; ++kk) {
            const int k = wave * KW + kk;
            float hk;
            if constexpr (U == 1) {
                hk = __int_as_float(__builtin_amdgcn_readlane(__float_as_int(h[0]), k));
            } else {
                const float src = (k < 64) ? h[0] : h[U - 1];
                hk = __int_as_float(__builtin_amdgcn_readlane(__float_as_int(src), k & 63));
            }
#pragma unroll
            for (int g = 0; g < 3; ++g)
#pragma unroll
                for (int i = 0; i < U; ++i) acc[g][i] = fmaf(w[g][i][kk], hk, acc[g][i]);
        }
        const int buf = t & 1;
#pragma unroll
        for (int g = 0; g < 3; ++g)
#pragma unroll
            for (int i = 0; i < U; ++i) s_part[buf][wave][g][lane + 64 * i] = acc[g][i];
        __syncthreads();
#pragma unroll
        for (int i = 0; i < U; ++i) {
            const int u = lane + 64 * i;
            float gh[3];
#pragma unroll
            for (int g = 0; g < 3; ++g) {
                float sacc = 0.0f;
#pragma unroll
                for (int ww = 0; ww < NW; ++ww) sacc += s_part[buf][ww][g][u];
                gh[g] = sacc + bias[g][i];
            }
            const float r = gru_sigmoid(ring[SLOT][0][i] + gh[0]);
            const float z = gru_sigmoid(ring[SLOT][1][i] + gh[1]);
            const float nn = gru_tanh(ring[SLOT][2][i] + r * gh[2]);
            h[i] = (h[i] - nn) * z + nn;
        }
        if (wave == 0) {
            float* orow = out + (((int64_t)b * T + t) * io.J + j) * H;
#pragma unroll
            for (int i = 0; i < U; ++i) orow[lane + 64 * i] = h[i];
        }
    };

    for (int t = 0; t < T; t += 3) {
        step(std::integral_constant<int, 0>{}, t);
        if (t + 1 < T) step(std::integral_constant<int, 1>{}, t + 1);
        if (t + 2 < T) step(std::integral_constant<int, 2>{}, t + 2);
    }
}


typedef float float2v __attribute__((ext_vector_type(2)));
__device__ __forceinline__ float quad_sum(float x) {
    x += __uint_as_float(__builtin_amdgcn_update_dpp(0u, __float_as_uint(x), 0xB1, 0xF, 0xF, false));
    x += __uint_as_float(__builtin_amdgcn_update_dpp(0u, __float_as_uint(x), 0x4E, 0xF, 0xF, false));
    return x;
}
__device__ __forceinline__ float gru_tanh_folded(float x) {
    const float e = __builtin_amdgcn_exp2f(x * 2.885390081777927f);
    return fmaf(-2.0f, __builtin_amdgcn_rcpf(e + 1.0f), 1.0f);
}

template <bool STATIC>
__global__ void __launch_bounds__(256) gru_sequence_units_kernel(const macjd_gru_io io) {
    constexpr int H = 64, NW = 4;
    const int lane = threadIdx.x & 63;
    const int wave = __builtin_amdgcn_readfirstlane(threadIdx.x >> 6);
    const int q = lane & 3;
    const int u = 16 * wave + (lane >> 2);
    const int net = blockIdx.y;
    const int seq = blockIdx.x;
    const int b = seq / io.J, j = seq - b * io.J;
    const int T = io.T;
    const float* __restrict__ gi = io.gi[net];
    const float* __restrict__ whh = io.w_hh[net];
    const float* __restrict__ bhh = io.b_hh[net];
    float* __restrict__ out = io.h_out[net];

    __shared__ __attribute__((aligned(16))) float s_h[2][H];
    __shared__ float s_gi[3 * H];
    __shared__ float s_pro[768];
    if (STATIC && blockIdx.z == 1) {
        scan_prologue<H, NW>(io, net, b, j, s_pro, s_gi, lane, wave, false, true);
        return;
    }

    float2v w2[3][8];
#pragma unroll
    for (int g = 0; g < 3; ++g) {
        const float4* row = reinterpret_cast<const float4*>(whh + (int64_t)(g * H + u) * H + 16 * q);
#pragma unroll
        for (int k4 = 0; k4 < 4; ++k4) {
            const float4 v = row[k4];
            w2[g][2 * k4] = float2v{v.x, v.y};
            w2[g][2 * k4 + 1] = float2v{v.z, v.w};
        }
    }
    float bias[3];
#pragma unroll
    for (int g = 0; g < 3; ++g) bias[g] = bhh[g * H + u];
    float h = io.h0[net] ? io.h0[net][(int64_t)b * (io.h0_sb[net] ? io.h0_sb[net] : (int64_t)io.J * H) + (int64_t)j * H + u] : 0.0f;

    const bool gi_inkernel = STATIC && io.obs != nullptr;
    if (gi_inkernel) scan_prologue<H, NW>(io, net, b, j, s_pro, s_gi, lane, wave, true, gridDim.z == 1);
    float ring[3][3];
    if (STATIC) {
#pragma unroll
        for (int g = 0; g < 3; ++g) {
            const float v = gi_inkernel ? s_gi[g * H + u] : gi[((int64_t)b * io.J + j) * (3 * H) + g * H + u];
            ring[0][g] = v; ring[1][g] = v; ring[2][g] = v;
        }
    } else if (T > 0) {
        const float* r0 = gi + (((int64_t)b * T) * io.J + j) * (3 * H);
        const float* r1 = gi + (((int64_t)b * T + (T > 1 ? 1 : 0)) * io.J + j) * (3 * H);
#pragma unroll
        for (int g = 0; g < 3; ++g) { ring[0][g] = r0[g * H + u]; ring[1][g] = r1[g * H + u]; }
    }
    if (q == 0) s_h[0][u] = h;
    __syncthreads();

    auto step = [&](auto slot_c, int t) {
        constexpr int SLOT = decltype(slot_c)::value;
        constexpr int PRE = (SLOT + 2) % 3;
        const int buf = t & 1;
        const float4* hp = reinterpret_cast<const float4*>(&s_h[buf][16 * q]);
        const float4 h0v = hp[0], h1v = hp[1], h2v = hp[2], h3v = hp[3];
        if constexpr (!STATIC) {
            const float* rn = gi + (((int64_t)b * T + (t + 2 < T ? t + 2 : T - 1)) * io.J + j) * (3 * H);
#pragma unroll
            for (int g = 0; g < 3; ++g) ring[PRE][g] = rn[g * H + u];
        }
        const float2v hv[8] = {float2v{h0v.x, h0v.y}, float2v{h0v.z, h0v.w}, float2v{h1v.x, h1v.y}, float2v{h1v.z, h1v.w},
                               float2v{h2v.x, h2v.y}, float2v{h2v.z, h2v.w}, float2v{h3v.x, h3v.y}, float2v{h3v.z, h3v.w}};
        float gh[3];
        float2v acc[3] = {float2v{0.0f, 0.0f}, float2v{0.0f, 0.0f}, float2v{0.0f, 0.0f}};
#pragma unroll
        for (int kk = 0; kk < 8; ++kk)
#pragma unroll
            for (int g = 0; g < 3; ++g) acc[g] = __builtin_elementwise_fma(w2[g][kk], hv[kk], acc[g]);
#pragma unroll
        for (int g = 0; g < 3; ++g) gh[g] = quad_sum(acc[g].x + acc[g].y) + bias[g];
        const float r = gru_sigmoid(ring[SLOT][0] + gh[0]);
        const float z = gru_sigmoid(ring[SLOT][1] + gh[1]);
        const float nn = gru_tanh_folded(ring[SLOT][2] + r * gh[2]);
        h = (h - nn) * z + nn;
        if (q == 0) {
            s_h[buf ^ 1][u] = h;
            out[(((int64_t)b * T + t) * io.J + j) * H + u] = h;
        }
        __syncthreads();
    };
    for (int t = 0; t < T; t += 3) {
        step(std::integral_constant<int, 0>{}, t);
        if (t + 1 < T) step(std::integral_constant<int, 1>{}, t + 1);
        if (t + 2 < T) step(std::integral_constant<int, 2>{}, t + 2);
    }
}

}

extern "C" int macjd_gru_sequence(const macjd_gru_io* io, void* hip_stream) {
    using namespace macjd;
    if (!io) return set_nets_err(MACJD_EINVAL, "macjd_gru_sequence: NULL io");
    if (io->n_nets < 1 || io->n_nets > 2 || io->B < 0 || io->T < 0 || io->J < 1)
        return set_nets_err(MACJD_EINVAL, "macjd_gru_sequence: bad n_nets / B / T / J");
    if (io->H != 64 && io->H != 128) return set_nets_err(MACJD_EUNSUPPORTED, "macjd_gru_sequence: H must be 64 or 128");
    for (int n = 0; n < io->n_nets; ++n) {
        if ((!io->gi[n] && !io->obs) || !io->w_hh[n] || !io->b_hh[n] || !io->h_out[n])
            return set_nets_err(MACJD_EINVAL, "macjd_gru_sequence: NULL pointer");
        if (io->obs && (!io->fc1_w[n] || !io->fc1_b[n] || !io->w_ih[n] || !io->b_ih[n]))
            return set_nets_err(MACJD_EINVAL, "macjd_gru_sequence: in-kernel input transform needs fc1 / W_ih");
    }
    if (io->obs && (io->S < 1 || io->S > 256))
        return set_nets_err(MACJD_EINVAL, "macjd_gru_sequence: in-kernel input transform needs 1 <= S <= 256");
    for (int n = 0; n < io->n_nets; ++n)
        if (io->obs && io->p_out[n]) {
            if (io->Ah < 1 || io->Ah > 256 || io->A < 1 || io->A > 64)
                return set_nets_err(MACJD_EINVAL, "macjd_gru_sequence: in-kernel actor needs Ah <= 256, A <= 64");
            for (int l = 0; l < 3; ++l)
                if (!io->act_w[n][l] || !io->act_b[n][l])
                    return set_nets_err(MACJD_EINVAL, "macjd_gru_sequence: in-kernel actor needs its three layers");
        }
    if (io->B == 0 || io->T == 0) return MACJD_OK;
    const bool actor = io->obs && (io->p_out[0] || (io->n_nets > 1 && io->p_out[1]));
    const dim3 g((unsigned)(io->B * io->J), (unsigned)io->n_nets, actor ? 2u : 1u);
    hipStream_t s = (hipStream_t)hip_stream;
    const bool ksplit = env_options().gru_ksplit;
    if (io->H == 64 && !ksplit) {
        if (io->obs || io->reserved) hipLaunchKernelGGL(gru_sequence_units_kernel<true>, g, dim3(256), 0, s, *io);
        else hipLaunchKernelGGL(gru_sequence_units_kernel<false>, g, dim3(256), 0, s, *io);
    }
    else if (io->H == 64) hipLaunchKernelGGL((gru_sequence_kernel<64, 4>), g, dim3(256), 0, s, *io);
    else hipLaunchKernelGGL((gru_sequence_kernel<128, 8>), g, dim3(512), 0, s, *io);
    hipError_t err = hipGetLastError();
    if (err != hipSuccess) return set_nets_err(MACJD_EDEVICE, hipGetErrorString(err));
    return MACJD_OK;
}

namespace macjd {

__device__ __forceinline__ float clampf(float x, float lo, float hi) { return fminf(fmaxf(x, lo), hi); }

template <bool BACKWARD>
__global__ void __launch_bounds__(256) mixer_tail_kernel(const macjd_mixer_io io) {
    const int lane = threadIdx.x & 63;
    const int64_t m = (int64_t)blockIdx.x * (blockDim.x >> 6) + (threadIdx.x >> 6);
    if (m >= io.M) return;
    const int J = io.J, Em = io.Em;
    const float* __restrict__ q = io.q + m * J;
    const float* __restrict__ w1r = io.w1_raw + m * (int64_t)J * Em;
    float ysum = 0.0f;
    float gq_acc[MACJD_MAX_JAMMERS];
    if (BACKWARD) {
#pragma unroll
        for (int j = 0; j < MACJD_MAX_JAMMERS; ++j) gq_acc[j] = 0.0f;
    }
    const float gy = BACKWARD ? io.gy[m] : 0.0f;
    for (int e = lane; e < ((Em + 63) & ~63); e += 64) {
        const bool live = e < Em;
        const float b1r = live ? io.b1_raw[m * (io.b1_ld ? io.b1_ld : (int64_t)Em) + e] : 0.0f;
        const float wfr = live ? io.wf_raw[m * Em + e] : 0.0f;
        float hid = clampf(b1r, -5.0f, 5.0f);
        for (int j = 0; j < J; ++j) {
            const float w = live ? clampf(w1r[(int64_t)j * Em + e], 0.0f, 5.0f) : 0.0f;
            hid = fmaf(q[j], w, hid);
        }
        const float h = hid > 0.0f ? hid : expm1f(hid);
        const float wf = clampf(wfr, 0.0f, 5.0f);
        if (!BACKWARD) {
            ysum += live ? h * wf : 0.0f;
        } else if (live) {
            const float ghid = gy * wf * (hid > 0.0f ? 1.0f : h + 1.0f);
            io.gwf_raw[m * Em + e] = (wfr >= 0.0f && wfr <= 5.0f) ? gy * h : 0.0f;
            io.gb1_raw[m * Em + e] = (b1r >= -5.0f && b1r <= 5.0f) ? ghid : 0.0f;
            for (int j = 0; j < J; ++j) {
                const float wr = w1r[(int64_t)j * Em + e];
                io.gw1_raw[m * (int64_t)J * Em + (int64_t)j * Em + e] = (wr >= 0.0f && wr <= 5.0f) ? ghid * q[j] : 0.0f;
                gq_acc[j] += ghid * clampf(wr, 0.0f, 5.0f);
            }
        }
    }
    if (!BACKWARD) {
        const float tot = wave_sum(ysum);
        if (lane == 0) io.y[m] = tot + clampf(io.v_raw[m], -5.0f, 5.0f);
    } else {
        for (int j = 0; j < J; ++j) {
            const float t = wave_sum(gq_acc[j]);
            if (lane == 0) io.gq[m * J + j] = t;
        }
        if (lane == 0) {
            const float vr = io.v_raw[m];
            io.gv_raw[m] = (vr >= -5.0f && vr <= 5.0f) ? gy : 0.0f;
        }
    }
}

static int mixer_launch(const macjd_mixer_io* io, void* hip_stream, bool backward) {
    if (!io) return set_nets_err(MACJD_EINVAL, "macjd_mixer_tail: NULL io");
    if (io->M < 0 || io->J < 1 || io->J > MACJD_MAX_JAMMERS || io->Em < 1)
        return set_nets_err(MACJD_EINVAL, "macjd_mixer_tail: bad M / J / Em");
    if (!io->q || !io->w1_raw || !io->b1_raw || !io->wf_raw || !io->v_raw)
        return set_nets_err(MACJD_EINVAL, "macjd_mixer_tail: NULL input");
    if (!backward && !io->y) return set_nets_err(MACJD_EINVAL, "macjd_mixer_tail_forward: NULL y");
    if (backward && (!io->gy || !io->gq || !io->gw1_raw || !io->gb1_raw || !io->gwf_raw || !io->gv_raw))
        return set_nets_err(MACJD_EINVAL, "macjd_mixer_tail_backward: NULL gradient pointer");
    if (io->M == 0) return MACJD_OK;
    const dim3 g((unsigned)((io->M + 3) / 4)), b(256);
    hipStream_t s = (hipStream_t)hip_stream;
    if (backward) hipLaunchKernelGGL((mixer_tail_kernel<true>), g, b, 0, s, *io);
    else hipLaunchKernelGGL((mixer_tail_kernel<false>), g, b, 0, s, *io);
    hipError_t err = hipGetLastError();
    if (err != hipSuccess) return set_nets_err(MACJD_EDEVICE, hipGetErrorString(err));
    return MACJD_OK;
}

}

extern "C" int macjd_mixer_tail_forward(const macjd_mixer_io* io, void* hip_stream) {
    return macjd::mixer_launch(io, hip_stream, false);
}
extern "C" int macjd_mixer_tail_backward(const macjd_mixer_io* io, void* hip_stream) {
    return macjd::mixer_launch(io, hip_stream, true);
}

namespace macjd {

__global__ void __launch_bounds__(1024) td_loss_kernel(const macjd_tdloss_io io) {
    const float tot_m = td_loss_sums(io, io.gy != nullptr);
    if (!io.gy) return;
    const float scale = 2.0f / tot_m;
    const int cols = (int)io.gy_cols;
    for (int i = threadIdx.x; i < io.B * cols; i += blockDim.x) {
        const int b = i / cols, t = i - b * cols;
        float g = 0.0f;
        if (t < io.Tm1) {
            const float term = io.terminated[b * io.t_sb + t * io.t_st] ? 1.0f : 0.0f;
            const float m = io.filled[b * io.f_sb + t * io.f_st] ? 1.0f : 0.0f;
            const float target = io.reward[b * io.r_sb + t * io.r_st] + io.gamma * (1.0f - term) * io.tq[b * io.tq_sb + t];
            g = scale * m * (io.y[b * io.y_sb + t] - target);
        }
        io.gy[b * io.gy_sb + t] = g;
    }
}

}

namespace macjd {
__global__ void __launch_bounds__(1024) td_mask_sum_kernel(const macjd_tdloss_io io, float* __restrict__ out) {
    __shared__ float s_w[16];
    const int M = io.B * io.Tm1;
    float s = 0.0f;
    for (int i = threadIdx.x; i < M; i += blockDim.x) {
        const int b = i / io.Tm1, t = i - b * io.Tm1;
        s += io.filled[b * io.f_sb + t * io.f_st] ? 1.0f : 0.0f;
    }
    s = wave_sum(s);
    if ((threadIdx.x & 63) == 0) s_w[threadIdx.x >> 6] = s;
    __syncthreads();
    if (threadIdx.x < 64) {
        float t = (threadIdx.x < (blockDim.x >> 6)) ? s_w[threadIdx.x] : 0.0f;
        t = wave_sum(t);
        if (threadIdx.x == 0) out[0] = t;
    }
}
}

extern "C" int macjd_td_mask_sum(const macjd_tdloss_io* io, float* out, void* hip_stream) {
    using namespace macjd;
    if (!io || !out || io->B < 1 || io->Tm1 < 1 || !io->filled) return set_nets_err(MACJD_EINVAL, "macjd_td_mask_sum: bad argument");
    hipLaunchKernelGGL(td_mask_sum_kernel, dim3(1), dim3(1024), 0, (hipStream_t)hip_stream, *io, out);
    hipError_t err = hipGetLastError();
    if (err != hipSuccess) return set_nets_err(MACJD_EDEVICE, hipGetErrorString(err));
    return MACJD_OK;
}

extern "C" int macjd_td_loss(const macjd_tdloss_io* io, void* hip_stream) {
    using namespace macjd;
    if (!io || io->B < 1 || io->Tm1 < 1) return set_nets_err(MACJD_EINVAL, "macjd_td_loss: bad B / Tm1");
    if (!io->y || !io->tq || !io->reward || !io->terminated || !io->filled || !io->stats)
        return set_nets_err(MACJD_EINVAL, "macjd_td_loss: NULL pointer");
    if (io->y_sb < io->Tm1 || io->tq_sb < io->Tm1 || (io->gy && (io->gy_cols < io->Tm1 || io->gy_sb < io->gy_cols)))
        return set_nets_err(MACJD_EINVAL, "macjd_td_loss: bad strides");
    hipLaunchKernelGGL(td_loss_kernel, dim3(1), dim3(1024), 0, (hipStream_t)hip_stream, *io);
    hipError_t err = hipGetLastError();
    if (err != hipSuccess) return set_nets_err(MACJD_EDEVICE, hipGetErrorString(err));
    return MACJD_OK;
}

namespace macjd {

constexpr int ADAM_BLOCKS = 256;

__global__ void __launch_bounds__(256) adam_sqnorm_kernel(const macjd_adam_io io) {
    __shared__ float smem[4];
    float s = 0.0f;
    for (int64_t i = (int64_t)blockIdx.x * blockDim.x + threadIdx.x; i < io.n; i += (int64_t)gridDim.x * blockDim.x) {
        const float g = io.grad[i];
        s = fmaf(g, g, s);
    }
    s = wave_sum(s);
    if ((threadIdx.x & 63) == 0) smem[threadIdx.x >> 6] = s;
    __syncthreads();
    if (threadIdx.x == 0) {
        io.partials[blockIdx.x] = (smem[0] + smem[1]) + (smem[2] + smem[3]);
        if (blockIdx.x == 0) io.step[0] += 1.0f;
    }
}

__global__ void __launch_bounds__(256) adam_sqnorm_ln_kernel(const macjd_adam_io io, const macjd_lnparam_io ln, const int64_t g_off,
                                                             const int64_t b_off, const int nb) {
    __shared__ float smem[8];
    if ((int)blockIdx.x < nb) {
        float s = 0.0f;
        for (int64_t i = (int64_t)blockIdx.x * blockDim.x + threadIdx.x; i < io.n; i += (int64_t)nb * blockDim.x) {
            const bool is_ln = (i >= g_off && i < g_off + ln.K) || (i >= b_off && i < b_off + ln.K);
            const float g = is_ln ? 0.0f : io.grad[i];
            s = fmaf(g, g, s);
        }
        s = wave_sum(s);
        if ((threadIdx.x & 63) == 0) smem[threadIdx.x >> 6] = s;
        __syncthreads();
        if (threadIdx.x == 0) {
            io.partials[blockIdx.x] = (smem[0] + smem[1]) + (smem[2] + smem[3]);
            if (blockIdx.x == 0) io.step[0] += 1.0f;
        }
        return;
    }
    const int k = (int)blockIdx.x - nb;
    float sg = 0.0f, sb = 0.0f;
    for (int c = threadIdx.x; c < ln.C; c += blockDim.x) {
        const float w = ln.W[(int64_t)c * ln.w_ld + k];
        sg = fmaf(w, ln.G[(int64_t)c * ln.g_ld + k], sg);
        sb = fmaf(w, ln.gb[c], sb);
    }
    sg = wave_sum(sg);
    sb = wave_sum(sb);
    if ((threadIdx.x & 63) == 0) { smem[threadIdx.x >> 6] = sg; smem[4 + (threadIdx.x >> 6)] = sb; }
    __syncthreads();
    if (threadIdx.x == 0) {
        const float dg = (smem[0] + smem[1]) + (smem[2] + smem[3]), db = (smem[4] + smem[5]) + (smem[6] + smem[7]);
        ln.dgamma[k] = dg;
        ln.dbeta[k] = db;
        io.partials[nb + k] = fmaf(db, db, dg * dg);
    }
}

__device__ __forceinline__ uint32_t fmix32(uint32_t h) {
    h ^= h >> 16; h *= 0x85ebca6bu; h ^= h >> 13; h *= 0xc2b2ae35u; h ^= h >> 16;
    return h;
}
__device__ __forceinline__ void sample_episodes_block(const macjd_sampler_io& sp) {
    const int64_t c = *sp.counter;
    const int64_t N = (int64_t)*sp.n_stored;
    __syncthreads();
    if (threadIdx.x == 0) *sp.counter = c + 1;
    if (N < 1) return;
    const Philox4 ka = philox4x32_10((uint32_t)c, (uint32_t)((uint64_t)c >> 32), 0x53414d50u, 0u, (uint32_t)sp.seed, (uint32_t)(sp.seed >> 32));
    const Philox4 kb = philox4x32_10((uint32_t)c, (uint32_t)((uint64_t)c >> 32), 0x53414d50u, 1u, (uint32_t)sp.seed, (uint32_t)(sp.seed >> 32));
    const uint32_t key[8] = {ka.v[0], ka.v[1], ka.v[2], ka.v[3], kb.v[0], kb.v[1], kb.v[2], kb.v[3]};
    int k = 2;
    while (((int64_t)1 << k) < N) ++k;
    const int rb = k - k / 2, lb = k / 2;
    const uint32_t rmask = (1u << rb) - 1u, lmask = (1u << lb) - 1u;
    for (int t = threadIdx.x; t < sp.n; t += blockDim.x) {
        if (N < sp.n) { sp.idx_out[t] = t % N; continue; }
        uint32_t x = (uint32_t)t;
        for (int walk = 0; walk < 64; ++walk) {
            uint32_t L = x >> rb, R = x & rmask;
#pragma unroll
            for (int r = 0; r < 8; r += 2) {
                L = (L ^ fmix32(R ^ key[r])) & lmask;
                R = (R ^ fmix32(L ^ key[r + 1])) & rmask;
            }
            x = (L << rb) | R;
            if ((int64_t)x < N) break;
        }
        sp.idx_out[t] = ((int64_t)x < N) ? (int64_t)x : (int64_t)(x % (uint32_t)N);
    }
}

__global__ void __launch_bounds__(256) sample_episodes_kernel(const macjd_sampler_io sp) { sample_episodes_block(sp); }

template <bool SAMPLE>
__global__ void __launch_bounds__(256) adam_update_kernel(const macjd_adam_io io, const int n_partials, const macjd_sampler_io next) {
    __shared__ float s_tot;
    if (threadIdx.x < 64) {
        float s = 0.0f;
        for (int i = threadIdx.x; i < n_partials; i += 64) s += io.partials[i];
        s = wave_sum(s);
        if (threadIdx.x == 0) s_tot = s;
    }
    __syncthreads();
    const float total_norm = sqrtf(s_tot);
    float coef = io.max_norm / (total_norm + 1e-6f);
    coef = coef < 1.0f ? coef : 1.0f;
    const float step = io.step[0];
    const float bc1 = 1.0f - powf(io.beta1, step);
    const float bc2 = 1.0f - powf(io.beta2, step);
    const float step_size = io.lr / bc1;
    const float bc2_sqrt = sqrtf(bc2);
    for (int64_t i = (int64_t)blockIdx.x * blockDim.x + threadIdx.x; i < io.n; i += (int64_t)gridDim.x * blockDim.x) {
        const float g = io.grad[i] * coef;
        io.grad[i] = g;
        float m = io.exp_avg[i], v = io.exp_avg_sq[i];
        m = m + (1.0f - io.beta1) * (g - m);
        v = v * io.beta2 + (1.0f - io.beta2) * g * g;
        io.exp_avg[i] = m;
        io.exp_avg_sq[i] = v;
        const float denom = sqrtf(v) / bc2_sqrt + io.eps;
        io.param[i] -= step_size * (m / denom);
    }
    if (blockIdx.x == 0 && threadIdx.x == 0) io.grad_norm[0] = total_norm;
    if (SAMPLE && blockIdx.x == 0) sample_episodes_block(next);
}

__global__ void __launch_bounds__(256) gather_rows_kernel(const macjd_gather_io io) {
    const int k = blockIdx.y;
    const int row = blockIdx.z;
    const int64_t words = io.row_bytes[k] >> 2;
    const uint32_t* __restrict__ src = (const uint32_t*)((const char*)io.src[k] + io.idx[row] * io.row_bytes[k]);
    const int64_t dpitch = io.dst_row_bytes[k] ? io.dst_row_bytes[k] : io.row_bytes[k];
    uint32_t* __restrict__ dst = (uint32_t*)((char*)io.dst[k] + (int64_t)row * dpitch);
    const bool vec = ((io.row_bytes[k] & 15) == 0) && ((dpitch & 15) == 0) && ((((uintptr_t)io.src[k]) & 15) == 0) &&
                     ((((uintptr_t)io.dst[k]) & 15) == 0);
    if (vec) {
        const int64_t n4 = words >> 2;
        for (int64_t i = (int64_t)blockIdx.x * blockDim.x + threadIdx.x; i < n4; i += (int64_t)gridDim.x * blockDim.x)
            ((uint4*)dst)[i] = ((const uint4*)src)[i];
    } else {
        for (int64_t i = (int64_t)blockIdx.x * blockDim.x + threadIdx.x; i < words; i += (int64_t)gridDim.x * blockDim.x)
            dst[i] = src[i];
    }
}

}

static int sampler_args_ok(const macjd_sampler_io* sp) {
    return sp && sp->idx_out && sp->n >= 1 && sp->n_stored && sp->counter;
}

extern "C" int macjd_sample_episodes(const macjd_sampler_io* io, void* hip_stream) {
    using namespace macjd;
    if (!sampler_args_ok(io)) return set_nets_err(MACJD_EINVAL, "macjd_sample_episodes: bad argument");
    hipLaunchKernelGGL(sample_episodes_kernel, dim3(1), dim3(256), 0, (hipStream_t)hip_stream, *io);
    hipError_t err = hipGetLastError();
    if (err != hipSuccess) return set_nets_err(MACJD_EDEVICE, hipGetErrorString(err));
    return MACJD_OK;
}

extern "C" int macjd_clip_adam_step_sample(const macjd_adam_io* io, const macjd_sampler_io* next, void* hip_stream) {
    using namespace macjd;
    if (!io || io->n < 1 || !io->param || !io->grad || !io->exp_avg || !io->exp_avg_sq || !io->step || !io->grad_norm ||
        !io->partials)
        return set_nets_err(MACJD_EINVAL, "macjd_clip_adam_step: bad argument");
    if (next && !sampler_args_ok(next)) return set_nets_err(MACJD_EINVAL, "macjd_clip_adam_step_sample: bad sampler argument");
    hipStream_t s = (hipStream_t)hip_stream;
    int blocks = (int)((io->n + 255) / 256);
    if (blocks > ADAM_BLOCKS) blocks = ADAM_BLOCKS;
    hipLaunchKernelGGL(adam_sqnorm_kernel, dim3(blocks), dim3(256), 0, s, *io);
    if (next) hipLaunchKernelGGL(adam_update_kernel<true>, dim3(blocks), dim3(256), 0, s, *io, blocks, *next);
    else hipLaunchKernelGGL(adam_update_kernel<false>, dim3(blocks), dim3(256), 0, s, *io, blocks, macjd_sampler_io{});
    hipError_t err = hipGetLastError();
    if (err != hipSuccess) return set_nets_err(MACJD_EDEVICE, hipGetErrorString(err));
    return MACJD_OK;
}

extern "C" int macjd_clip_adam_step(const macjd_adam_io* io, void* hip_stream) {
    return macjd_clip_adam_step_sample(io, nullptr, hip_stream);
}

extern "C" int macjd_clip_adam_step_ln(const macjd_adam_io* io, const macjd_sampler_io* next, const macjd_lnparam_io* ln,
                                       int64_t gamma_off, int64_t beta_off, void* hip_stream) {
    using namespace macjd;
    if (!io || io->n < 1 || !io->param || !io->grad || !io->exp_avg || !io->exp_avg_sq || !io->step || !io->grad_norm ||
        !io->partials)
        return set_nets_err(MACJD_EINVAL, "macjd_clip_adam_step_ln: bad argument");
    if (next && !sampler_args_ok(next)) return set_nets_err(MACJD_EINVAL, "macjd_clip_adam_step_ln: bad sampler argument");
    if (!ln || ln->C < 1 || ln->K < 1 || ln->K > 1024 || !ln->W || !ln->G || !ln->gb || ln->w_ld < ln->K || ln->g_ld < ln->K)
        return set_nets_err(MACJD_EINVAL, "macjd_clip_adam_step_ln: bad LayerNorm argument");
    if (gamma_off < 0 || beta_off < 0 || gamma_off + ln->K > io->n || beta_off + ln->K > io->n ||
        ln->dgamma != io->grad + gamma_off || ln->dbeta != io->grad + beta_off)
        return set_nets_err(MACJD_EINVAL, "macjd_clip_adam_step_ln: dgamma / dbeta must be the named ranges of the gradient vector");
    hipStream_t s = (hipStream_t)hip_stream;
    int blocks = (int)((io->n + 255) / 256);
    if (blocks > ADAM_BLOCKS) blocks = ADAM_BLOCKS;
    hipLaunchKernelGGL(adam_sqnorm_ln_kernel, dim3(blocks + ln->K), dim3(256), 0, s, *io, *ln, gamma_off, beta_off, blocks);
    if (next) hipLaunchKernelGGL(adam_update_kernel<true>, dim3(blocks), dim3(256), 0, s, *io, blocks + ln->K, *next);
    else hipLaunchKernelGGL(adam_update_kernel<false>, dim3(blocks), dim3(256), 0, s, *io, blocks + ln->K, macjd_sampler_io{});
    hipError_t err = hipGetLastError();
    if (err != hipSuccess) return set_nets_err(MACJD_EDEVICE, hipGetErrorString(err));
    return MACJD_OK;
}

extern "C" int macjd_gather_rows(const macjd_gather_io* io, void* hip_stream) {
    using namespace macjd;
    if (!io || io->n_tensors < 1 || io->n_tensors > 8 || io->n_rows < 0 || !io->idx)
        return set_nets_err(MACJD_EINVAL, "macjd_gather_rows: bad argument");
    for (int k = 0; k < io->n_tensors; ++k)
        if (!io->src[k] || !io->dst[k] || io->row_bytes[k] < 4 || (io->row_bytes[k] & 3) || (io->dst_row_bytes[k] & 3) ||
            (io->dst_row_bytes[k] && io->dst_row_bytes[k] < io->row_bytes[k]))
            return set_nets_err(MACJD_EINVAL, "macjd_gather_rows: bad tensor (row bytes must be a positive multiple of 4)");
    if (io->n_rows == 0) return MACJD_OK;
    hipLaunchKernelGGL(gather_rows_kernel, dim3(8, io->n_tensors, io->n_rows), dim3(256), 0, (hipStream_t)hip_stream, *io);
    hipError_t err = hipGetLastError();
    if (err != hipSuccess) return set_nets_err(MACJD_EDEVICE, hipGetErrorString(err));
    return MACJD_OK;
}

namespace macjd {

__global__ void __launch_bounds__(256) qhead_input_kernel(const macjd_qinput_io io) {
    const int W = io.H + io.A + 1;
    const int64_t total = io.n_rows * W;
    for (int64_t i = (int64_t)blockIdx.x * blockDim.x + threadIdx.x; i < total; i += (int64_t)gridDim.x * blockDim.x) {
        const int64_t n = i / W;
        const int c = (int)(i - n * W);
        float v;
        if (c < io.H) {
            v = io.h[n * io.h_ld + c];
        } else if (c < io.H + io.A) {
            const int64_t a = (io.idx_elem_size == 8) ? ((const int64_t*)io.idx)[n] : (int64_t)((const int32_t*)io.idx)[n];
            v = (a == (int64_t)(c - io.H)) ? 1.0f : 0.0f;
        } else {
            v = io.P[n];
        }
        io.out[n * io.out_ld + c] = v;
    }
}

__global__ void __launch_bounds__(256) layernorm_forward_kernel(const macjd_layernorm_io io) {
    const int lane = threadIdx.x & 63;
    const int64_t wave = (int64_t)blockIdx.x * (blockDim.x >> 6) + (threadIdx.x >> 6);
    const int64_t n_waves = (int64_t)gridDim.x * (blockDim.x >> 6);
    const int S = io.S;
    const float inv_s = 1.0f / (float)S;
    for (int64_t m = wave; m < io.M; m += n_waves) {
        const float* __restrict__ x = io.x + m * io.x_ld;
        float v[16];
        float sum = 0.0f;
#pragma unroll
        for (int i = 0; i < 16; ++i) {
            const int c = lane + 64 * i;
            v[i] = (c < S) ? x[c] : 0.0f;
            sum += v[i];
        }
#pragma unroll
        for (int o = 32; o > 0; o >>= 1) sum += __shfl_xor(sum, o);
        const float mean = sum * inv_s;
        float sq = 0.0f;
#pragma unroll
        for (int i = 0; i < 16; ++i) {
            const int c = lane + 64 * i;
            const float d = (c < S) ? v[i] - mean : 0.0f;
            sq = fmaf(d, d, sq);
        }
#pragma unroll
        for (int o = 32; o > 0; o >>= 1) sq += __shfl_xor(sq, o);
        const float rstd = rsqrtf(sq * inv_s + io.eps);
        float* __restrict__ y = io.y + m * io.y_ld;
#pragma unroll
        for (int i = 0; i < 16; ++i) {
            const int c = lane + 64 * i;
            if (c < S) {
                const float g = io.gamma ? io.gamma[c] : 1.0f, b = io.beta ? io.beta[c] : 0.0f;
                y[c] = (v[i] - mean) * rstd * g + b;
                if (io.xhat) io.xhat[m * io.xhat_ld + c] = (v[i] - mean) * rstd;
            }
        }
        if (lane == 0) {
            if (io.mean) io.mean[m] = mean;
            if (io.rstd) io.rstd[m] = rstd;
        }
    }
}

}

extern "C" int macjd_qhead_input(const macjd_qinput_io* io, void* hip_stream) {
    using namespace macjd;
    if (!io || io->n_rows < 0 || io->H < 1 || io->A < 1 || !io->h || !io->idx || !io->P || !io->out)
        return set_nets_err(MACJD_EINVAL, "macjd_qhead_input: bad argument");
    if (io->idx_elem_size != 4 && io->idx_elem_size != 8)
        return set_nets_err(MACJD_EINVAL, "macjd_qhead_input: idx_elem_size must be 4 or 8");
    if (io->h_ld < io->H || io->out_ld < io->H + io->A + 1)
        return set_nets_err(MACJD_EINVAL, "macjd_qhead_input: row stride smaller than the row");
    if (io->n_rows == 0) return MACJD_OK;
    const int64_t total = io->n_rows * (io->H + io->A + 1);
    const int64_t blocks = (total + 255) / 256;
    hipLaunchKernelGGL(qhead_input_kernel, dim3((unsigned)(blocks < 4096 ? blocks : 4096)), dim3(256), 0,
                       (hipStream_t)hip_stream, *io);
    hipError_t err = hipGetLastError();
    if (err != hipSuccess) return set_nets_err(MACJD_EDEVICE, hipGetErrorString(err));
    return MACJD_OK;
}

extern "C" int macjd_layernorm_forward(const macjd_layernorm_io* io, void* hip_stream) {
    using namespace macjd;
    if (!io || io->M < 0 || io->S < 1 || io->S > 1024 || !io->x || !io->y)
        return set_nets_err(MACJD_EINVAL, "macjd_layernorm_forward: bad argument (1 <= S <= 1024)");
    if (io->x_ld < io->S || io->y_ld < io->S)
        return set_nets_err(MACJD_EINVAL, "macjd_layernorm_forward: row stride smaller than the row");
    if (io->M == 0) return MACJD_OK;
    const int64_t blocks = (io->M + 3) / 4;
    hipLaunchKernelGGL(layernorm_forward_kernel, dim3((unsigned)(blocks < 8192 ? blocks : 8192)), dim3(256), 0,
                       (hipStream_t)hip_stream, *io);
    hipError_t err = hipGetLastError();
    if (err != hipSuccess) return set_nets_err(MACJD_EDEVICE, hipGetErrorString(err));
    return MACJD_OK;
}

namespace macjd {

template <bool VEC>
__global__ void __launch_bounds__(256) gru_gates_kernel(const macjd_grugates_io io) {
    const int H = io.H, q = H >> 2;
    const int64_t total = io.n_rows * q;
    for (int64_t i = (int64_t)blockIdx.x * blockDim.x + threadIdx.x; i < total; i += (int64_t)gridDim.x * blockDim.x) {
        const int64_t n = i / q;
        const int u = (int)(i - n * q) * 4;
        const float* gi = io.gi + n * io.gi_ld + u;
        const float* gh = io.gh + n * io.gh_ld + u;
        const float* hpp = io.h + n * io.h_ld + u;
        float ir[4], iz[4], in_[4], hr[4], hz[4], hn[4], hp[4], out[4];
        auto ld4 = [](const float* p, float* d) {
            if (VEC) {
                const float4 v = *reinterpret_cast<const float4*>(p);
                d[0] = v.x; d[1] = v.y; d[2] = v.z; d[3] = v.w;
            } else {
#pragma unroll
                for (int k = 0; k < 4; ++k) d[k] = p[k];
            }
        };
        ld4(gi, ir); ld4(gi + H, iz); ld4(gi + 2 * H, in_);
        ld4(gh, hr); ld4(gh + H, hz); ld4(gh + 2 * H, hn);
        ld4(hpp, hp);
#pragma unroll
        for (int k = 0; k < 4; ++k) {
            const float r = 1.0f / (1.0f + expf(-(ir[k] + hr[k])));
            const float z = 1.0f / (1.0f + expf(-(iz[k] + hz[k])));
            const float nn = 1.0f - 2.0f / (expf(2.0f * (in_[k] + r * hn[k])) + 1.0f);
            out[k] = (hp[k] - nn) * z + nn;
        }
        float* o1 = io.h_out + n * io.ho_ld + u;
        if (VEC) *reinterpret_cast<float4*>(o1) = float4{out[0], out[1], out[2], out[3]};
        else {
#pragma unroll
            for (int k = 0; k < 4; ++k) o1[k] = out[k];
        }
        if (io.h_out2) {
            float* o2 = io.h_out2 + n * io.ho2_ld + u;
            if (VEC) *reinterpret_cast<float4*>(o2) = float4{out[0], out[1], out[2], out[3]};
            else {
#pragma unroll
                for (int k = 0; k < 4; ++k) o2[k] = out[k];
            }
        }
// ... 159 lines not shown
```

ma-cjd-cooperative-jamming-decision-making-via-marl_amd/ops.py:

```python
from __future__ import annotations

import ctypes
import os
from typing import Optional, Tuple

import numpy as np
import torch
import torch.nn.functional as F

from . import _native, options


def _stream(t: torch.Tensor) -> int:
    return torch.cuda.current_stream(t.device).cuda_stream


def _f32c(t: torch.Tensor) -> torch.Tensor:
    if t.dtype != torch.float32:
        t = t.float()
    return t if t.stride(-1) == 1 else t.contiguous()


def _qhead_fill(io: _native.QheadIO, base, P_all, W1, w2, b2, H: int, A: int, n_agents: int):
    io.n_rows, io.H, io.A, io.n_agents = base.shape[0], H, A, n_agents
# ... 297 lines not shown
    a, l1, l2 = agent.actor, agent.fc2_q_head[0], agent.fc2_q_head[2]
    for name, t_ in (("fc1_w", agent.fc1.weight), ("fc1_b", agent.fc1.bias), ("w_ih", agent.rnn.weight_ih),
                     ("b_ih", agent.rnn.bias_ih), ("w_hh", agent.rnn.weight_hh), ("b_hh", agent.rnn.bias_hh),
                     ("a1_w", a[0].weight), ("a1_b", a[0].bias), ("a2_w", a[2].weight), ("a2_b", a[2].bias),
                     ("a3_w", a[4].weight), ("a3_b", a[4].bias), ("b1", l1.bias), ("w2", l2.weight.reshape(-1)),
                     ("b2", l2.bias.reshape(-1))):
        setattr(io, name, f32(t_).data_ptr())
    W1 = l1.weight.detach()
    W1 = W1 if (W1.dtype == torch.float32 and W1.stride(-1) == 1) else W1.float().contiguous()
    keep.append(W1)
    io.W1, io.w1_ld = W1.data_ptr(), W1.stride(0)
    dev = W1.device
    if avail is not None:
        if avail.dtype not in (torch.int32, torch.int64):
            avail = avail.to(torch.int32)
        keep.append(avail)
        io.avail, io.avail_elem_size = avail.data_ptr(), avail.element_size()
        io.av_se, io.av_sj, io.av_sa = avail.stride(0), avail.stride(1), avail.stride(2)
    if eps_sched is not None:
        assert eps_sched.dtype == torch.float32 and eps_sched.numel() >= T and eps_sched.is_contiguous()
        io.eps = eps_sched.data_ptr()
    io.seed = int(seed) & (2 ** 64 - 1)
    if counter_base is not None:
        assert counter_base.dtype in (torch.int64, torch.uint64) and counter_base.numel() >= 1
        io.counter_base = counter_base.data_ptr()
    io.env_seed = int(env_args["seed"]) & (2 ** 64 - 1)
    io.episode = env_args["episode"].data_ptr()
    track, step = env_args["track"], env_args["step"]
    io.track, io.k_se, io.k_sx = track.data_ptr(), track.stride(1), track.stride(0)
    io.step = step.data_ptr()
    ctypes.memmove(ctypes.addressof(io) + _native.AgentEnvEpisodeScanIO.scan.offset, ctypes.addressof(env_args["scan_io"]),
                   ctypes.sizeof(_native.ScanIO))
    io.pe_tables = env_args.get("pe_tables")
    E, J = int(n_envs), int(n_agents)
    sizes = {"state": (T * E * S, torch.float32), "obs": (T * E * J * S, torch.float32),
             "hidden_state": (T * E * J * H, torch.float32), "actions_discrete": (T * E * J, torch.int32),
             "actions_continuous": (T * E * J, torch.float32), "reward": (T * E, torch.float32), "terminated": (T * E, None)}
    for k, (n, dt) in sizes.items():
        t_ = stage[k]
        assert t_.is_contiguous() and t_.device == dev and t_.numel() >= n and (dt is None or t_.dtype == dt), k
    assert stage["terminated"].dtype in (torch.bool, torch.uint8)
    assert stage["state"].shape[-1] == S and stage["obs"].shape[-1] == S
    io.hidden, io.T_out, io.P_out = stage["hidden_state"].data_ptr(), stage["actions_discrete"].data_ptr(), stage["actions_continuous"].data_ptr()
    io.st_state, io.st_obs = stage["state"].data_ptr(), stage["obs"].data_ptr()
    io.reward, io.terminated = stage["reward"].data_ptr(), stage["terminated"].data_ptr()
    if rdpj_sum is not None:
        assert rdpj_sum.is_contiguous() and rdpj_sum.dtype == torch.float32 and rdpj_sum.numel() == 3 * E
        io.rdpj_sum = rdpj_sum.data_ptr()
    if h_final is not None:
        assert h_final.is_contiguous() and h_final.dtype == torch.float32 and h_final.numel() == E * J * H
        io.h_final = h_final.data_ptr()
    with torch.cuda.device(dev):
        _native.check(lib.macjd_agent_env_episode_scan(env_args["handle"], ctypes.byref(io), _stream(W1)),
                      "macjd_agent_env_episode_scan")


def gru_sequence_reference(gi: torch.Tensor, w_hh: torch.Tensor, b_hh: torch.Tensor,
                           h0: Optional[torch.Tensor] = None) -> torch.Tensor:
    B, T, J, H3 = gi.shape
    H = H3 // 3
    h = gi.new_zeros(B * J, H) if h0 is None else h0.reshape(B * J, H)
    out = gi.new_empty(B, T, J, H)
    for t in range(T):
        g = gi[:, t].reshape(B * J, H3)
        gh = F.linear(h, w_hh, b_hh)
        r = torch.sigmoid(g[:, :H] + gh[:, :H])
        z = torch.sigmoid(g[:, H:2 * H] + gh[:, H:2 * H])
        n = torch.tanh(g[:, 2 * H:] + r * gh[:, 2 * H:])
        h = (h - n) * z + n
        out[:, t] = h.view(B, J, H)
    return out


def gru_sequence(gi: torch.Tensor, w_hh: torch.Tensor, b_hh: torch.Tensor,
                 h0: Optional[torch.Tensor] = None) -> torch.Tensor:
    if not gi.is_cuda:
        return gru_sequence_reference(gi, w_hh, b_hh, h0)
    return gru_sequence_multi([gi], [w_hh], [b_hh], [h0])[0]


def gru_sequence_backward(gi, gh, h_all, w_hh, dh_all, h0=None, want_dh0=False):
    lib = _native.load()
    B, T, J, H3 = gi.shape
    H = H3 // 3
    gi, gh, h_all, w_hh, dh_all = (t.detach().float().contiguous() for t in (gi, gh, h_all, w_hh, dh_all))
    assert gh.numel() == gi.numel() and h_all.numel() == B * T * J * H and dh_all.numel() == h_all.numel()
    assert tuple(w_hh.shape) == (H3, H)
    io = _native.GruBwdIO()
    io.B, io.T, io.J, io.H = B, T, J, H
    io.gi, io.gh, io.h_all, io.w_hh, io.dh_all = (t.data_ptr() for t in (gi, gh, h_all, w_hh, dh_all))
    if h0 is not None:
        h0 = h0.detach().float().reshape(B, J, H) if h0.dim() != 3 else h0.detach().float()
        if h0.stride(2) != 1 or h0.stride(1) != H or (B > 1 and h0.stride(0) < J * H):
            h0 = h0.contiguous()
        io.h0, io.h0_sb = h0.data_ptr(), (h0.stride(0) if B > 1 else 0)
    dgi = torch.empty((B, T, J, H3), dtype=torch.float32, device=gi.device)
    dgh = torch.empty((B, T, J, H3), dtype=torch.float32, device=gi.device)
    dh0 = torch.empty((B, J, H), dtype=torch.float32, device=gi.device) if want_dh0 else None
    io.dgi, io.dgh, io.dh0 = dgi.data_ptr(), dgh.data_ptr(), (dh0.data_ptr() if want_dh0 else None)
    with torch.cuda.device(gi.device):
        _native.check(lib.macjd_gru_sequence_backward(ctypes.byref(io), _stream(gi)), "macjd_gru_sequence_backward")
    return dgi, dgh, dh0


class _GruSequenceTrain(torch.autograd.Function):

    @staticmethod
    def forward(ctx, gi, w_hh, b_hh, h0):
        h_all = gru_sequence(gi, w_hh, b_hh, h0)
        ctx.save_for_backward(gi, w_hh, b_hh, h_all, h0)
        return h_all

    @staticmethod
    def backward(ctx, dh_all):
        gi, w_hh, b_hh, h_all, h0 = ctx.saved_tensors
        B, T, J, H3 = gi.shape
        H = H3 // 3
        nd = ctx.needs_input_grad
        h_prev = torch.empty((B, T, J, H), dtype=h_all.dtype, device=h_all.device)
        if h0 is None:
            h_prev[:, 0].zero_()
        else:
            h_prev[:, 0].copy_(h0.detach().reshape(B, J, H))
        if T > 1:
            h_prev[:, 1:].copy_(h_all[:, :T - 1])
        rows_prev = h_prev.view(B * T * J, H)
        gh = F.linear(rows_prev, w_hh.detach(), b_hh.detach())
        dgi, dgh, dh0 = gru_sequence_backward(gi, gh, h_all, w_hh, dh_all, h0=h0, want_dh0=h0 is not None and nd[3])
        dW = db = None
        if nd[1] or nd[2]:
            rows_g = dgh.view(B * T * J, H3)
            if rows_g.shape[0] >= 1024:
                dW, db = linear_wgrad(rows_g, rows_prev, want_bias=True, w_key=grad_key(w_hh), b_key=grad_key(b_hh),
                                      need=(nd[1], nd[2]))
            else:
                dW, db = rows_g.t().matmul(rows_prev), rows_g.sum(0)
        if dh0 is not None:
            dh0 = dh0.view_as(h0)
        return (dgi if nd[0] else None), (dW if nd[1] else None), (db if nd[2] else None), dh0


def gru_sequence_train(gi: torch.Tensor, w_hh: torch.Tensor, b_hh: torch.Tensor,
                       h0: Optional[torch.Tensor] = None) -> torch.Tensor:
    H = gi.shape[-1] // 3
    if (gi.is_cuda and gi.dtype == torch.float32 and w_hh.dtype == torch.float32 and b_hh.dtype == torch.float32
            and (h0 is None or h0.dtype == torch.float32) and not torch.is_autocast_enabled() and gi.shape[1] > 0
            and bool(_native.load().macjd_gru_sequence_backward_supported(int(H)))):
        return _GruSequenceTrain.apply(gi, w_hh, b_hh, h0)
    return gru_sequence_reference(gi, w_hh, b_hh, h0)


def gru_sequence_from_obs(obs, obs_index, agents, B: int, J: int, n_steps: int, with_actor: bool = False):
    lib = _native.load()
    assert obs.is_cuda and obs.dtype == torch.float32 and obs.dim() == 4 and obs.stride(3) == 1 and obs.shape[2] == J
    outs, pouts = [], []
    for start in range(0, len(agents), 2):
        part = agents[start:start + 2]
        H = part[0].rnn_hidden_dim
        if H not in (64, 128):
            raise _native.NativeLibraryError(f"macjd_gru_sequence supports rnn_hidden_dim 64 or 128, got {H}")
        io = _native.GruIO()
        io.n_nets, io.B, io.T, io.J, io.H = len(part), int(B), int(n_steps), int(J), H
        io.obs, io.obs_sb, io.obs_sj, io.S = obs.data_ptr(), obs.stride(0), obs.stride(2), obs.shape[3]
        if obs_index is not None:
            assert obs_index.dtype == torch.int64 and obs_index.is_cuda and obs_index.numel() >= B
            io.obs_index = obs_index.data_ptr()
        keep = []
        for k, a in enumerate(part):
            ts = [t.detach().float().contiguous() for t in (a.rnn.weight_hh, a.rnn.bias_hh, a.fc1.weight, a.fc1.bias,
                                                            a.rnn.weight_ih, a.rnn.bias_ih)]
            keep += ts
            io.w_hh[k], io.b_hh[k], io.fc1_w[k], io.fc1_b[k], io.w_ih[k], io.b_ih[k] = [t.data_ptr() for t in ts]
            o = torch.empty((B, n_steps, J, H), dtype=torch.float32, device=obs.device)
            io.h_out[k] = o.data_ptr()
            outs.append(o)
            if with_actor:
                layers = [(w.detach().float().contiguous(), b_.detach().float().contiguous()) for w, b_, _ in a.actor_layers()]
                keep += [t for pair in layers for t in pair]
                for l, (w, b_) in enumerate(layers):
                    io.act_w[k][l], io.act_b[k][l] = w.data_ptr(), b_.data_ptr()
                io.Ah, io.A = layers[0][0].shape[0], layers[2][0].shape[0]
                pk_ = torch.empty((B, J, io.A), dtype=torch.float32, device=obs.device)
                io.p_out[k] = pk_.data_ptr()
                pouts.append(pk_)
        with torch.cuda.device(obs.device):
            _native.check(lib.macjd_gru_sequence(ctypes.byref(io), _stream(obs)), "macjd_gru_sequence")
    return (outs, pouts) if with_actor else outs


def gru_sequence_multi(gis, w_hhs, b_hhs, h0s=None, n_steps=None):
    n = len(gis)
    h0s = h0s if h0s is not None else [None] * n
    static = n_steps is not None
    if static:
        assert all(g.shape[1] == 1 for g in gis)
    if not gis[0].is_cuda:
        if static:
            gis = [g.expand(-1, int(n_steps), -1, -1) for g in gis]
        return [gru_sequence_reference(g, w, b, h) for g, w, b, h in zip(gis, w_hhs, b_hhs, h0s)]
    lib = _native.load()
    B, T, J, H3 = gis[0].shape
    if static:
        T = int(n_steps)
    H = H3 // 3
    if H not in (64, 128):
        raise _native.NativeLibraryError(f"macjd_gru_sequence supports rnn_hidden_dim 64 or 128, got {H}")
    outs = []
    for start in range(0, n, 2):
        io = _native.GruIO()
        keep = []
        cnt = min(2, n - start)
        io.n_nets, io.B, io.T, io.J, io.H = cnt, B, T, J, H
        io.reserved = 1 if static else 0
        for k in range(cnt):
            g = gis[start + k].detach().float().contiguous()
            w = w_hhs[start + k].detach().float().contiguous()
            bb = b_hhs[start + k].detach().float().contiguous()
            h0 = h0s[start + k]
            if h0 is not None:
                h0 = h0.detach().float().reshape(B, J, H) if h0.dim() != 3 else h0.detach().float()
                if h0.stride(2) != 1 or h0.stride(1) != H:
                    h0 = h0.contiguous()
                io.h0_sb[k] = h0.stride(0)
            o = torch.empty((B, T, J, H), dtype=torch.float32, device=g.device)
            keep += [g, w, bb, h0]
            io.gi[k], io.w_hh[k], io.b_hh[k] = g.data_ptr(), w.data_ptr(), bb.data_ptr()
            io.h0[k] = h0.data_ptr() if h0 is not None else None
            io.h_out[k] = o.data_ptr()
            outs.append(o)
        with torch.cuda.device(gis[0].device):
            _native.check(lib.macjd_gru_sequence(ctypes.byref(io), _stream(gis[0])), "macjd_gru_sequence")
    return outs


def gru_gates(gi, gh, h, out2: Optional[torch.Tensor] = None) -> torch.Tensor:
    N, H = h.shape
    if not h.is_cuda or (H & 3):
        r = torch.sigmoid(gi[:, :H] + gh[:, :H])
        z = torch.sigmoid(gi[:, H:2 * H] + gh[:, H:2 * H])
        n = torch.tanh(gi[:, 2 * H:] + r * gh[:, 2 * H:])
        hn = (h - n) * z + n
        if out2 is not None:
            out2.view(N, H).copy_(hn)
        return hn
    lib = _native.load()
    gi, gh, h = _f32c(gi.detach()), _f32c(gh.detach()), _f32c(h.detach())
    out = torch.empty((N, H), dtype=torch.float32, device=h.device)
    io = _native.GruGatesIO()
    io.n_rows, io.H = N, H
    io.gi, io.gi_ld, io.gh, io.gh_ld = gi.data_ptr(), gi.stride(0), gh.data_ptr(), gh.stride(0)
    io.h, io.h_ld, io.h_out, io.ho_ld = h.data_ptr(), h.stride(0), out.data_ptr(), out.stride(0)
    if out2 is not None:
        o2 = out2.view(N, H)
        assert o2.dtype == torch.float32 and o2.stride(1) == 1 and o2.device == h.device
        io.h_out2, io.ho2_ld = o2.data_ptr(), o2.stride(0)
    with torch.cuda.device(h.device):
        _native.check(lib.macjd_gru_gates(ctypes.byref(io), _stream(h)), "macjd_gru_gates")
    return out


def mixer_tail_reference(q, w1_raw, b1_raw, wf_raw, v_raw):
    M, J = q.shape
    Em = b1_raw.shape[1]
    w1 = torch.clamp(w1_raw, min=0.0, max=5.0).view(M, J, Em)
    b1 = torch.clamp(b1_raw, min=-5.0, max=5.0)
    wf = torch.clamp(wf_raw, min=0.0, max=5.0)
    v = torch.clamp(v_raw, min=-5.0, max=5.0)
    hidden = F.elu((q.unsqueeze(2) * w1).sum(dim=1) + b1)
    return (hidden * wf).sum(dim=1, keepdim=True) + v


def _mixer_io(q, w1_raw, b1_raw, wf_raw, v_raw):
    io = _native.MixerIO()
    io.M, io.J, io.Em = q.shape[0], q.shape[1], b1_raw.shape[1]
    io.q, io.w1_raw, io.b1_raw = q.data_ptr(), w1_raw.data_ptr(), b1_raw.data_ptr()
    io.wf_raw, io.v_raw = wf_raw.data_ptr(), v_raw.data_ptr()
    io.b1_ld = b1_raw.stride(0)
    return io


class _MixerTailHip(torch.autograd.Function):
    @staticmethod
    def forward(ctx, q, w1_raw, b1_raw, wf_raw, v_raw):
        lib = _native.load()
        args = [t.detach().float().contiguous() for t in (q, w1_raw)] + [_f32c(b1_raw.detach())] + \
               [t.detach().float().contiguous() for t in (wf_raw, v_raw)]
        y = torch.empty((q.shape[0], 1), dtype=torch.float32, device=q.device)
        io = _mixer_io(*args)
        io.y = y.data_ptr()
        with torch.cuda.device(q.device):
            _native.check(lib.macjd_mixer_tail_forward(ctypes.byref(io), _stream(q)), "macjd_mixer_tail_forward")
        ctx.save_for_backward(*args)
        return y

    @staticmethod
    def backward(ctx, gy):
        lib = _native.load()
        q, w1_raw, b1_raw, wf_raw, v_raw = ctx.saved_tensors
        gy = gy.detach().float().contiguous()
        gq, gw1 = torch.empty_like(q), torch.empty_like(w1_raw)
        gb1 = torch.empty(b1_raw.shape, dtype=torch.float32, device=q.device)
        gwf, gv = torch.empty_like(wf_raw), torch.empty_like(v_raw)
        io = _mixer_io(q, w1_raw, b1_raw, wf_raw, v_raw)
        io.gy, io.gq, io.gw1_raw = gy.data_ptr(), gq.data_ptr(), gw1.data_ptr()
        io.gb1_raw, io.gwf_raw, io.gv_raw = gb1.data_ptr(), gwf.data_ptr(), gv.data_ptr()
        with torch.cuda.device(q.device):
            _native.check(lib.macjd_mixer_tail_backward(ctypes.byref(io), _stream(q)), "macjd_mixer_tail_backward")
        return gq, gw1, gb1, gwf, gv


def mixer_tail(q, w1_raw, b1_raw, wf_raw, v_raw):
    if not q.is_cuda:
        return mixer_tail_reference(q, w1_raw, b1_raw, wf_raw, v_raw)
    return _MixerTailHip.apply(q, w1_raw, b1_raw, wf_raw, v_raw)


def mixer_fused_supported(J: int, S: int, Hh: int, Em: int, bf16: bool = False) -> bool:
    if bf16 and S <= 16 * (J - (2 if J % 2 == 0 else 1)):
        return False
    return bool(_native.load().macjd_mixer_fused_supported(int(J), int(S), int(Hh), int(Em)))


def _mixerf_io(q, s, p):
    io = _native.MixerFusedIO()
    io.M, io.J, io.S, io.Hh, io.Em = q.shape[0], q.shape[1], p["W1"].shape[1], p["W2"].shape[1], p["Wf2"].shape[0]
    io.ln_eps = float(p["eps"])
    io.operand_dtype = 1 if p.get("bf16") else 0
    io.q = q.data_ptr()
    if s is not None:
        io.s, io.s_ld = s.data_ptr(), s.stride(0)
    for k in ("ln_w", "ln_b", "W1", "b1", "W2", "b2", "Wf2", "bf2", "wV2", "bV2"):
        setattr(io, k, p[k].data_ptr())
    return io


def _mixerf_params(ln_w, ln_b, eps, w_cat, b_cat, W2, b2, Wf2, bf2, wV2, bV2, bf16=False):
    c = lambda t: t.detach() if (t.dtype == torch.float32 and t.is_contiguous()) else t.detach().float().contiguous()
    return {"ln_w": c(ln_w), "ln_b": c(ln_b), "eps": eps, "W1": c(w_cat), "b1": c(b_cat), "W2": c(W2), "b2": c(b2),
            "Wf2": c(Wf2), "bf2": c(bf2), "wV2": c(wV2).reshape(-1), "bV2": c(bV2).reshape(-1), "bf16": bool(bf16)}

# ... 245 lines not shown
    for l, (w, b, act) in enumerate(layers):
        w, b = w.detach().float().contiguous(), b.detach().float().contiguous()
        keep += [w, b]
        io.dims[l], io.W[l], io.b[l], io.act[l] = dims[l], w.data_ptr(), b.data_ptr(), int(act)
    io.dims[len(layers)] = dims[-1]
    io.x, io.x_ld, io.y, io.y_ld = x.data_ptr(), x.stride(0), y.data_ptr(), y.stride(0)
    keep.append(x)
    return io, y, dims


def mlp_forward_pair(x0, layers0, x1, layers1):
    d0 = [layers0[0][0].shape[1]] + [w.shape[0] for w, _, _ in layers0]
    d1 = [layers1[0][0].shape[1]] + [w.shape[0] for w, _, _ in layers1]
    if not (x0.is_cuda and x1.is_cuda and mlp_supported(d0) and mlp_supported(d1)) or x0.numel() == 0 or x1.numel() == 0:
        return mlp_forward(x0, layers0), mlp_forward(x1, layers1)
    lib = _native.load()
    keep = []
    io0, y0, _ = _mlp_io(x0, layers0, keep)
    io1, y1, _ = _mlp_io(x1, layers1, keep)
    with torch.cuda.device(x0.device):
        _native.check(lib.macjd_mlp_forward_pair(ctypes.byref(io0), ctypes.byref(io1), _stream(x0)), "macjd_mlp_forward_pair")
    return y0, y1


def td_loss_reference(y, tq, reward, terminated, filled, gamma):
    targets = reward + gamma * (1 - terminated.float()) * tq
    m = filled.float()
    td = (y - targets.detach()) * m
    return (td ** 2).sum() / m.sum(), y.detach().mean(), targets.mean()


class _TdLossHip(torch.autograd.Function):

    @staticmethod
    def forward(ctx, y_full, tq_full, reward, terminated, filled, gamma, Tm1, tq_off):
        lib = _native.load()
        B, Ty = y_full.shape[0], y_full.shape[1]
        yc, tqc = y_full.detach().float().contiguous(), tq_full.detach().float().contiguous()
        stats = torch.empty(4, dtype=torch.float32, device=yc.device)
        gy = torch.empty((B, Ty, 1), dtype=torch.float32, device=yc.device)
        io = _native.TdLossIO()
        io.B, io.Tm1, io.gamma = B, int(Tm1), float(gamma)
        io.y, io.y_sb = yc.data_ptr(), Ty
        io.tq, io.tq_sb = tqc.data_ptr() + 4 * int(tq_off), tqc.shape[1]
        io.gy, io.gy_sb, io.gy_cols = gy.data_ptr(), Ty, Ty
        io.reward, io.r_sb, io.r_st = reward.data_ptr(), reward.stride(0), reward.stride(1)
        io.terminated, io.t_sb, io.t_st = terminated.data_ptr(), terminated.stride(0), terminated.stride(1)
        io.filled, io.f_sb, io.f_st = filled.data_ptr(), filled.stride(0), filled.stride(1)
        io.stats = stats.data_ptr()
        with torch.cuda.device(yc.device):
            _native.check(lib.macjd_td_loss(ctypes.byref(io), _stream(yc)), "macjd_td_loss")
        ctx.save_for_backward(gy)
        ctx.mark_non_differentiable(stats)
        stats.saved_gy = gy
        return stats[0], stats

    @staticmethod
    def backward(ctx, g_loss, _g_stats):
        (gy,) = ctx.saved_tensors
        return gy * g_loss, None, None, None, None, None, None, None


def td_loss_full(y_full, tq_full, reward, terminated, filled, gamma, Tm1, tq_off):
    loss, stats = _TdLossHip.apply(y_full, tq_full, reward, terminated, filled, gamma, Tm1, tq_off)
    return loss, stats[1], stats[2]


def td_loss_and_grad(y_full, tq_full, reward, terminated, filled, gamma, Tm1, tq_off):
    with torch.no_grad():
        _, stats = _TdLossHip.apply(y_full, tq_full, reward, terminated, filled, gamma, Tm1, tq_off)
    return stats[0], stats[1], stats[2], stats.saved_gy, stats


def td_loss_sums_into(row, y_full, tq_full, reward, terminated, filled, gamma, Tm1, tq_off):
    lib = _native.load()
    io, keep = _tdloss_sums_io(row, y_full, tq_full, reward, terminated, filled, gamma, Tm1, tq_off)
    with torch.cuda.device(row.device):
        _native.check(lib.macjd_td_loss(ctypes.byref(io), _stream(row)), "macjd_td_loss")
    return row


def _tdloss_sums_io(row, y_full, tq_full, reward, terminated, filled, gamma, Tm1, tq_off):
    B, Ty = y_full.shape[0], y_full.shape[1]
    yc, tqc = y_full.detach(), tq_full.detach()
    assert yc.dtype == torch.float32 and tqc.dtype == torch.float32 and yc.is_contiguous() and tqc.is_contiguous()
    assert row.dtype == torch.float32 and row.numel() >= 3 and row.is_contiguous()
    io = _native.TdLossIO()
    io.B, io.Tm1, io.gamma = B, int(Tm1), float(gamma)
    io.y, io.y_sb = yc.data_ptr(), Ty
    io.tq, io.tq_sb = tqc.data_ptr() + 4 * int(tq_off), tqc.shape[1]
    io.reward, io.r_sb, io.r_st = reward.data_ptr(), reward.stride(0), reward.stride(1)
    io.terminated, io.t_sb, io.t_st = terminated.data_ptr(), terminated.stride(0), terminated.stride(1)
    io.filled, io.f_sb, io.f_st = filled.data_ptr(), filled.stride(0), filled.stride(1)
    io.stats, io.gy = row.data_ptr(), None
    return io, (row, yc, tqc, reward, terminated, filled)


def td_mask_sum(filled, Tm1):
    lib = _native.load()
    out = torch.empty(1, dtype=torch.float32, device=filled.device)
    io = _native.TdLossIO()
    io.B, io.Tm1 = filled.shape[0], int(Tm1)
    io.filled, io.f_sb, io.f_st = filled.data_ptr(), filled.stride(0), filled.stride(1)
    with torch.cuda.device(filled.device):
        _native.check(lib.macjd_td_mask_sum(ctypes.byref(io), out.data_ptr(), _stream(filled)), "macjd_td_mask_sum")
    return out


_PENDING_TD = None


def fused_mixer_backward_will_run(y_full) -> bool:
    fn = getattr(y_full, "grad_fn", None)
    for _ in range(4):
        if fn is None:
            return False
        if type(fn).__name__.startswith("_FusedMixer"):
            return True
        nxt = [f for f, _ in fn.next_functions if f is not None]
        if len(nxt) != 1:
            return False
        fn = nxt[0]
    return False


def td_grad_in_mixer_backward(y_full, tq_full, reward, terminated, filled, gamma, Tm1, tq_off, tot_m, stats_row=None):
    global _PENDING_TD
    B, Ty = y_full.shape[0], y_full.shape[1]
    yc, tqc = y_full.detach().float().contiguous(), tq_full.detach().float().contiguous()
    io = _native.TdLossIO()
    io.B, io.Tm1, io.gamma = B, int(Tm1), float(gamma)
    io.y, io.y_sb = yc.data_ptr(), Ty
    io.tq, io.tq_sb = tqc.data_ptr() + 4 * int(tq_off), tqc.shape[1]
    io.gy, io.gy_sb, io.gy_cols = None, Ty, Ty
    io.reward, io.r_sb, io.r_st = reward.data_ptr(), reward.stride(0), reward.stride(1)
    io.terminated, io.t_sb, io.t_st = terminated.data_ptr(), terminated.stride(0), terminated.stride(1)
    io.filled, io.f_sb, io.f_st = filled.data_ptr(), filled.stride(0), filled.stride(1)
    if stats_row is not None:
        assert stats_row.dtype == torch.float32 and stats_row.numel() >= 3 and stats_row.is_contiguous()
        io.stats = stats_row.data_ptr()
    _PENDING_TD = (io, (yc, tqc, reward, terminated, filled, tot_m, stats_row), B * Ty, tot_m)
    return torch.empty((B, Ty, 1), dtype=torch.float32, device=yc.device)


def td_loss(y, tq, reward, terminated, filled, gamma):
    ok = (y.is_cuda and reward.dtype == torch.float32 and terminated.dtype == torch.bool and filled.dtype == torch.bool
          and y.shape[1] > 0)
    if not ok:
        return td_loss_reference(y, tq, reward, terminated, filled, gamma)
    loss, stats = _TdLossHip.apply(y, tq, reward, terminated, filled, gamma, y.shape[1], 0)
    return loss, stats[1], stats[2]


def _sampler_io(idx_out, n_stored, counter, seed):
    assert idx_out.dtype == torch.int64 and idx_out.is_contiguous() and n_stored.dtype == torch.int32 and counter.dtype == torch.int64
    assert idx_out.is_cuda and n_stored.device == idx_out.device and counter.device == idx_out.device
    sp = _native.SamplerIO()
    sp.idx_out, sp.n, sp.n_stored, sp.counter = idx_out.data_ptr(), idx_out.numel(), n_stored.data_ptr(), counter.data_ptr()
    sp.seed = int(seed) & 0xFFFFFFFFFFFFFFFF
    return sp


def sample_episodes(idx_out, n_stored, counter, seed):
    lib = _native.load()
    sp = _sampler_io(idx_out, n_stored, counter, seed)
    with torch.cuda.device(idx_out.device):
        _native.check(lib.macjd_sample_episodes(ctypes.byref(sp), _stream(idx_out)), "macjd_sample_episodes")


def clip_adam_step(param, grad, exp_avg, exp_avg_sq, step, grad_norm, partials, lr, betas, eps, max_norm, sample_next=None,
                   lnparam=None):
    lib = _native.load()
    io = _native.AdamIO()
    io.n, io.lr, io.beta1, io.beta2, io.eps, io.max_norm = param.numel(), lr, betas[0], betas[1], eps, max_norm
    io.param, io.grad, io.exp_avg, io.exp_avg_sq = param.data_ptr(), grad.data_ptr(), exp_avg.data_ptr(), exp_avg_sq.data_ptr()
    io.step, io.grad_norm, io.partials = step.data_ptr(), grad_norm.data_ptr(), partials.data_ptr()
    sp = _sampler_io(*sample_next) if sample_next is not None else None
    spp = ctypes.byref(sp) if sp is not None else None
    held = list(lnparam or [])
    fuse = None
    if len(held) == 1:
        lio, esz, base = held[0].lnparam, grad.element_size(), grad.data_ptr()
        g_off, b_off = (lio.dgamma - base) // esz, (lio.dbeta - base) // esz
        if ((lio.dgamma - base) % esz == 0 and (lio.dbeta - base) % esz == 0 and 0 <= g_off <= grad.numel() - lio.K
                and 0 <= b_off <= grad.numel() - lio.K and partials.numel() >= 256 + lio.K):
            fuse = (lio, int(g_off), int(b_off))
    with torch.cuda.device(param.device):
        if fuse is not None:
            _native.check(lib.macjd_clip_adam_step_ln(ctypes.byref(io), spp, ctypes.byref(fuse[0]), fuse[1], fuse[2],
                                                      _stream(param)), "macjd_clip_adam_step_ln")
            return
        for fn in held:
            fn()
        _native.check(lib.macjd_clip_adam_step_sample(ctypes.byref(io), spp, _stream(param)), "macjd_clip_adam_step")


def gather_rows_supported(srcs) -> bool:
    return len(srcs) <= 8 and all(s.is_cuda and s.is_contiguous() and (s[0].numel() * s.element_size()) % 4 == 0
                                  for s in srcs)


def gather_rows(idx, srcs, dsts):
    lib = _native.load()
    io = _native.GatherIO()
    io.n_tensors, io.n_rows, io.idx = len(srcs), idx.numel(), idx.data_ptr()
    for k, (s_, d_) in enumerate(zip(srcs, dsts)):
        assert d_.is_contiguous() and d_.dtype == s_.dtype and d_.shape[0] == idx.numel() and d_[0].numel() >= s_[0].numel()
        io.src[k], io.dst[k], io.row_bytes[k] = s_.data_ptr(), d_.data_ptr(), s_[0].numel() * s_.element_size()
        io.dst_row_bytes[k] = d_.stride(0) * d_.element_size()
    with torch.cuda.device(idx.device):
        _native.check(lib.macjd_gather_rows(ctypes.byref(io), _stream(idx)), "macjd_gather_rows")


_DEFERRED_WGRAD = None
_DEFERRED_POST = None
_GRAD_DST = None
_DEFERRED_SEEN = None


def grad_key(t):
    return None if t is None else (t.data_ptr(), t.numel())


def _grad_dst(key, shape):
    if not _GRAD_DST or key is None:
        return None
    dst = _GRAD_DST.get(key)
    if dst is None or dst.numel() != int(np.prod(shape)) or not dst.is_contiguous():
        return None
    del _GRAD_DST[key]
    return dst.view(shape)


class deferred_wgrad:

    def __init__(self, grad_dst=None, hold_lnparam=False):
        self._grad_dst = grad_dst
        self._hold, self.held = bool(hold_lnparam), []

    def __enter__(self):
        global _DEFERRED_WGRAD, _DEFERRED_POST, _GRAD_DST, _DEFERRED_SEEN
        self._prev, _DEFERRED_WGRAD = _DEFERRED_WGRAD, []
        self._prev_post, _DEFERRED_POST = _DEFERRED_POST, []
        self._prev_dst, _GRAD_DST = _GRAD_DST, (dict(self._grad_dst) if self._grad_dst else None)
        self._prev_seen, _DEFERRED_SEEN = _DEFERRED_SEEN, set()
        return self

    def __exit__(self, *exc):
        global _DEFERRED_WGRAD, _DEFERRED_POST, _GRAD_DST, _DEFERRED_SEEN
        pending, _DEFERRED_WGRAD = _DEFERRED_WGRAD, self._prev
        post, _DEFERRED_POST = _DEFERRED_POST, self._prev_post
        _GRAD_DST, _DEFERRED_SEEN = self._prev_dst, self._prev_seen
        self._flush(exc, pending)
        if exc[0] is None:
            for fn in post:
                if self._hold and hasattr(fn, "lnparam"):
                    self.held.append(fn)
                else:
                    fn()
        return False

    @staticmethod
    def _flush(exc, pending):
        if exc[0] is None and pending:
            lib = _native.load()
            dev = pending[0][1][0].device
            for lo in range(0, len(pending), 8):
                part = pending[lo:lo + 8]
                arr = (_native.WgradIO * len(part))(*[io for io, _ in part])
                with torch.cuda.device(dev):
                    _native.check(lib.macjd_linear_wgrad_many(arr, len(part), _stream(part[0][1][0])),
                                  "macjd_linear_wgrad_many")


def linear_wgrad(gout, inp, want_bias=True, w_key=None, b_key=None, need=(True, True), outer=None):
    lib = _native.load()
    gout, inp = _f32c(gout), _f32c(inp)
    K, M = gout.shape
    N = inp.shape[1]
    if outer is not None:
        o_vec, o_w = _f32c(outer[0]).reshape(-1).contiguous(), _f32c(outer[1]).reshape(-1).contiguous()
        assert o_vec.numel() == K and o_w.numel() == M
    dW = _grad_dst(w_key, (M, N))
    if dW is None:
        dW = torch.empty((M, N), dtype=torch.float32, device=gout.device)
    db = None
    if want_bias:
        db = _grad_dst(b_key, (M,))
        if db is None:
            db = torch.empty((M,), dtype=torch.float32, device=gout.device)
    ws = torch.empty(int(lib.macjd_linear_wgrad_workspace_floats(K, M, N)), dtype=torch.float32, device=gout.device)
    io = _native.WgradIO()
    io.K, io.M, io.N = K, M, N
    io.gout, io.gout_ld, io.inp, io.inp_ld = gout.data_ptr(), gout.stride(0), inp.data_ptr(), inp.stride(0)
    io.dW, io.dw_ld, io.db, io.workspace = dW.data_ptr(), dW.stride(0), (db.data_ptr() if want_bias else None), ws.data_ptr()
    if outer is not None:
        io.outer_vec, io.outer_w = o_vec.data_ptr(), o_w.data_ptr()
    if _DEFERRED_WGRAD is not None and any(k is not None and k in _DEFERRED_SEEN for k in (w_key, b_key)):
        pending, posts = list(_DEFERRED_WGRAD), list(_DEFERRED_POST)
        del _DEFERRED_WGRAD[:], _DEFERRED_POST[:]
        deferred_wgrad._flush((None, None, None), pending)
        for fn in posts:
            fn()
    elif _DEFERRED_WGRAD is not None:
        _DEFERRED_SEEN.update(k for k in (w_key, b_key) if k is not None)
        unowned = tuple(t for t, n in ((dW, need[0]), (db, need[1])) if t is not None and not n)
        _DEFERRED_WGRAD.append((io, (ws, gout, inp) + unowned + ((o_vec, o_w) if outer is not None else ())))
        return dW, db
    with torch.cuda.device(gout.device):
        _native.check(lib.macjd_linear_wgrad(ctypes.byref(io), _stream(gout)), "macjd_linear_wgrad")
    return dW, db


class _LinearSplitK(torch.autograd.Function):

    @staticmethod
    def forward(ctx, x, weight, bias):
        ctx.save_for_backward(x, weight)
        ctx.has_bias, ctx.b_key = bias is not None, grad_key(bias)
        return F.linear(x, weight, bias)

    @staticmethod
    def backward(ctx, gy):
        x, weight = ctx.saved_tensors
        gx = gy.matmul(weight) if ctx.needs_input_grad[0] else None
        gW = gb = None
        if ctx.needs_input_grad[1] or (ctx.has_bias and ctx.needs_input_grad[2]):
            gW, gb = linear_wgrad(gy.reshape(-1, gy.shape[-1]), x.reshape(-1, x.shape[-1]), want_bias=ctx.has_bias,
                                  w_key=grad_key(weight), b_key=ctx.b_key,
                                  need=(ctx.needs_input_grad[1], ctx.has_bias and ctx.needs_input_grad[2]))
        return gx, gW, (gb if ctx.has_bias else None)


class _MergedLinear(torch.autograd.Function):

    @staticmethod
    def forward(ctx, x, w_cat, b_cat, *params):
        ctx.save_for_backward(x, w_cat)
        ctx.sizes, ctx.b_key = [p.shape[0] for p in params[:len(params) // 2]], grad_key(b_cat)
        return F.linear(x, w_cat, b_cat)

    @staticmethod
    def backward(ctx, gy):
        x, w_cat = ctx.saved_tensors
        gx = gy.matmul(w_cat) if ctx.needs_input_grad[0] else None
        gW, gb = linear_wgrad(gy, x, want_bias=True, w_key=grad_key(w_cat), b_key=ctx.b_key)
        return (gx, None, None) + tuple(gW.split(ctx.sizes, 0)) + tuple(gb.split(ctx.sizes, 0))


def merged_linear(x, w_cat, b_cat, params):
    return _MergedLinear.apply(x, w_cat, b_cat, *params)


def _layernorm_launch(x, weight, bias, eps, want_xhat):
    lib = _native.load()
    x = _f32c(x.detach())
    M, S = x.shape
    y = torch.empty((M, S), dtype=torch.float32, device=x.device)
    mean = torch.empty((M, 1), dtype=torch.float32, device=x.device)
    rstd = torch.empty((M, 1), dtype=torch.float32, device=x.device)
    xhat = torch.empty((M, S), dtype=torch.float32, device=x.device) if want_xhat else None
    io = _native.LayerNormIO()
    io.M, io.S, io.eps = M, S, float(eps)
    io.x, io.x_ld, io.y, io.y_ld = x.data_ptr(), x.stride(0), y.data_ptr(), y.stride(0)
# ... 365 lines not shown
```

ma-cjd-cooperative-jamming-decision-making-via-marl_amd/options.py:

```python
from __future__ import annotations

import os

_DEFAULTS = {
    "UPDATE_STREAMS": "2", "UPDATES_PER_GRAPH": "1", "PIPELINED_GROUP": "1", "SHARED_BODY": "1",
    "LEARNER_STATIC_OBS": "1", "ACTOR_IN_SCAN": "1", "DEVICE_SAMPLER": "1", "LN_IN_SQNORM": "1", "WGRAD_OUTER": "1",
    "QHEAD_TAKEN": "1", "QHEAD_DOUBLE_Q": "1", "QHEAD_DOUBLE_Q_H128": "0", "PAIRED_HEADS": "1", "MIXER_TRAIN": "1", "MIXER_STATIC_STATE": "1", "GRAPHED_ALLREDUCE": "0",
    "CLOSED_LOOP_ROLLOUT": "0",
}
_values = None


def reload() -> None:
    global _values
    _values = {k: os.environ.get("MACJD_" + k, d) for k, d in _DEFAULTS.items()}


def get(name: str) -> str:
    if _values is None:
        reload()
    return _values[name]


def on(name: str) -> bool:
    return get(name) != "0"
```

Before: 35.66 million env-steps/s.

## Fuse episode sampling, row gather, GRU scan and mask sum into one prefetch kernel

```diff
diff --git a/include/macjd_nets.h b/include/macjd_nets.h
--- a/include/macjd_nets.h
+++ b/include/macjd_nets.h
@@ -137,6 +137,18 @@
 } macjd_gather_io;
 
 int macjd_gather_rows(const macjd_gather_io* io, void* hip_stream);
+
+typedef struct macjd_prefetch_io {
+    macjd_gru_io gru;
+    macjd_gather_io gather;
+    macjd_sampler_io sampler;
+    macjd_tdloss_io mask;
+    float* tot_m;
+    int32_t no_draw, gather_blocks;
+} macjd_prefetch_io;
+
+int macjd_prefetch_batch_supported(int32_t n_nets, int32_t H, int32_t B);
+int macjd_prefetch_batch(const macjd_prefetch_io* io, void* hip_stream);
 
 typedef struct macjd_qinput_io {
     int64_t n_rows;
diff --git a/ma-cjd-cooperative-jamming-decision-making-via-marl_amd/_native.py b/ma-cjd-cooperative-jamming-decision-making-via-marl_amd/_native.py
--- a/ma-cjd-cooperative-jamming-decision-making-via-marl_amd/_native.py
+++ b/ma-cjd-cooperative-jamming-decision-making-via-marl_amd/_native.py
@@ -28,6 +28,7 @@
     "macjd_agent_env_episode_scan_supported", "macjd_agent_env_episode_scan",
     "macjd_scenario_set_scan_pattern",
     "macjd_gru_sequence_backward_supported", "macjd_gru_sequence_backward",
+    "macjd_prefetch_batch_supported", "macjd_prefetch_batch",
 ]
 
 
@@ -318,6 +319,13 @@
         ("n_tensors", ctypes.c_int32), ("n_rows", ctypes.c_int32), ("idx", ctypes.c_void_p),
         ("src", ctypes.c_void_p * 8), ("dst", ctypes.c_void_p * 8), ("row_bytes", ctypes.c_int64 * 8),
         ("dst_row_bytes", ctypes.c_int64 * 8),
+    ]
+
+
+class PrefetchIO(ctypes.Structure):
+    _fields_ = [
+        ("gru", GruIO), ("gather", GatherIO), ("sampler", SamplerIO), ("mask", TdLossIO),
+        ("tot_m", ctypes.c_void_p), ("no_draw", ctypes.c_int32), ("gather_blocks", ctypes.c_int32),
     ]
 
 
@@ -451,6 +459,10 @@
                                             ctypes.c_int64, ctypes.c_int64, ctypes.c_void_p]
     lib.macjd_sample_episodes.restype = ctypes.c_int
     lib.macjd_sample_episodes.argtypes = [ctypes.POINTER(SamplerIO), ctypes.c_void_p]
+    lib.macjd_prefetch_batch_supported.restype = ctypes.c_int
+    lib.macjd_prefetch_batch_supported.argtypes = [ctypes.c_int32] * 3
+    lib.macjd_prefetch_batch.restype = ctypes.c_int
+    lib.macjd_prefetch_batch.argtypes = [ctypes.POINTER(PrefetchIO), ctypes.c_void_p]
     lib.macjd_gather_rows.restype = ctypes.c_int
     lib.macjd_gather_rows.argtypes = [ctypes.POINTER(GatherIO), ctypes.c_void_p]
     lib.macjd_linear_wgrad.restype = ctypes.c_int
diff --git a/ma-cjd-cooperative-jamming-decision-making-via-marl_amd/core/qmix.py b/ma-cjd-cooperative-jamming-decision-making-via-marl_amd/core/qmix.py
--- a/ma-cjd-cooperative-jamming-decision-making-via-marl_amd/core/qmix.py
+++ b/ma-cjd-cooperative-jamming-decision-making-via-marl_amd/core/qmix.py
@@ -655,14 +655,20 @@
                 self._g_out_b = self._clip_and_step(sample_next=nxt)
         K = int(updates_per_graph if updates_per_graph is not None else options.get("UPDATES_PER_GRAPH"))
         self._g_multi = None
+        self._g_prefetch_launch = False
         if K > 1 and self._g_single and self._g_dev_sampler and fused and self._g_stats4 is not None:
             gm, rows, single_norm = torch.cuda.CUDAGraph(), [], self._grad_norm
             pipelined = (self._g_scan_from_ring and self._g_actor_in_scan and options.get("UPDATE_STREAMS") != "1"
                          and options.on("PIPELINED_GROUP"))
+            launch_agents = [self.mac.agent] if self._body_is_shared() else [self.target_mac.agent, self.mac.agent]
+            self._g_prefetch_launch = bool(pipelined and options.on("PREFETCH_LAUNCH") and "filled" in keys
+                                           and ops.prefetch_batch_supported(launch_agents, self._g_B, srcs))
             stage2 = {k: torch.zeros_like(v) for k, v in stage.items()} if pipelined else None
             stages = [stage, stage2]
             self._g_stages = stages
             origin_dev = self.device
+
+            unwritten = [0]
 
             def prefetch(dst, fork=True, draw=True):
                 origin = torch.cuda.current_stream(origin_dev)
@@ -673,6 +679,16 @@
                     ts.wait_stream(origin)
                 shared = self._body_is_shared()
                 agents = [self.mac.agent] if shared else [self.target_mac.agent, self.mac.agent]
+                if self._g_prefetch_launch:
+                    with torch.cuda.stream(ts), torch.no_grad():
+                        h, ps, tot_m = ops.prefetch_batch(
+                            buffer.buffers["obs"], agents, self._g_B, self.n_agents, self._g_T + 1,
+                            (self._g_idx, self._g_n_stored, self._g_draws, self._sampler_seed()), srcs, [dst[k] for k in keys],
+                            buffer.buffers["filled"], self._g_T - 1, offset=unwritten[0], draw=draw)
+                        unwritten[0] += 1 if draw else 0
+                        ev = torch.cuda.Event()
+                        ev.record(ts)
+                    return [h[0], h[0]], [ps[0], ps[0]], (ev, ev, tot_m)
                 with torch.cuda.stream(ts), torch.no_grad():
                     if draw:
                         ops.sample_episodes(self._g_idx, self._g_n_stored, self._g_draws, self._sampler_seed())
@@ -714,7 +730,11 @@
                     self._grad_norm = rows[-1][3]
                     if self._g_graphed_ar:
                         self._allreduce_grads(force=True)
-                    self._clip_and_step(sample_next=None if nxt_batch is not None else nxt)
+                    if nxt_batch is not None:
+                        self._clip_and_step(sample_next=None)
+                    else:
+                        self._clip_and_step(sample_next=nxt + (unwritten[0],))
+                        unwritten[0] = 0
                 if pipelined:
                     torch.cuda.current_stream(self.device).wait_stream(self._target_stream)
             self._grad_norm = single_norm
diff --git a/ma-cjd-cooperative-jamming-decision-making-via-marl_amd/csrc/macjd_nets.hip b/ma-cjd-cooperative-jamming-decision-making-via-marl_amd/csrc/macjd_nets.hip
--- a/ma-cjd-cooperative-jamming-decision-making-via-marl_amd/csrc/macjd_nets.hip
+++ b/ma-cjd-cooperative-jamming-decision-making-via-marl_amd/csrc/macjd_nets.hip
@@ -218,14 +218,17 @@
 
 namespace macjd {
 
+__device__ __forceinline__ int64_t scan_obs_row(const macjd_gru_io& io, const int b) {
+    return io.obs_index ? io.obs_index[b] : (int64_t)b;
+}
+
 template <int H, int NW>
-__device__ __forceinline__ void scan_prologue(const macjd_gru_io& io, const int net, const int b, const int j,
+__device__ __forceinline__ void scan_prologue(const macjd_gru_io& io, const int net, const int b, const int j, const int64_t row,
                                               float* __restrict__ s_pro, float* __restrict__ s_gi, const int lane,
                                               const int wave, const bool want_gi, const bool want_actor) {
     float* xs = s_pro;
     float* v1 = s_pro + 256;
     float* v2 = s_pro + 512;
-    const int64_t row = io.obs_index ? io.obs_index[b] : (int64_t)b;
     const float* x = io.obs + row * io.obs_sb + (int64_t)j * io.obs_sj;
     const int S = io.S;
     for (int k = threadIdx.x; k < S; k += 64 * NW) xs[k] = x[k];
@@ -308,7 +311,7 @@
     __shared__ float s_gi[3 * H];
     __shared__ float s_pro[768];
     if (blockIdx.z == 1) {
-        scan_prologue<H, NW>(io, net, b, j, s_pro, s_gi, lane, wave, false, true);
+        scan_prologue<H, NW>(io, net, b, j, scan_obs_row(io, b), s_pro, s_gi, lane, wave, false, true);
         return;
     }
 
@@ -334,7 +337,7 @@
     }
     const bool gi_inkernel = io.obs != nullptr;
     const bool gi_static = io.reserved != 0 || gi_inkernel;
-    if (gi_inkernel) scan_prologue<H, NW>(io, net, b, j, s_pro, s_gi, lane, wave, true, gridDim.z == 1);
+    if (gi_inkernel) scan_prologue<H, NW>(io, net, b, j, scan_obs_row(io, b), s_pro, s_gi, lane, wave, true, gridDim.z == 1);
     auto gi_row = [&](int t) -> const float* {
         return gi_inkernel ? (const float*)s_gi
                            : gi_static ? gi + ((int64_t)b * io.J + j) * (3 * H)
@@ -431,14 +434,14 @@
 }
 
 template <bool STATIC>
-__global__ void __launch_bounds__(256) gru_sequence_units_kernel(const macjd_gru_io io) {
+__device__ __forceinline__ void gru_units_body(const macjd_gru_io& io, const int net, const int seq, const int64_t obs_row,
+                                               const bool actor_only, const bool actor_in_scan, float (*s_h)[64],
+                                               float* s_gi, float* s_pro) {
     constexpr int H = 64, NW = 4;
     const int lane = threadIdx.x & 63;
     const int wave = __builtin_amdgcn_readfirstlane(threadIdx.x >> 6);
     const int q = lane & 3;
     const int u = 16 * wave + (lane >> 2);
-    const int net = blockIdx.y;
-    const int seq = blockIdx.x;
     const int b = seq / io.J, j = seq - b * io.J;
     const int T = io.T;
     const float* __restrict__ gi = io.gi[net];
@@ -446,11 +449,8 @@
     const float* __restrict__ bhh = io.b_hh[net];
     float* __restrict__ out = io.h_out[net];
 
-    __shared__ __attribute__((aligned(16))) float s_h[2][H];
-    __shared__ float s_gi[3 * H];
-    __shared__ float s_pro[768];
-    if (STATIC && blockIdx.z == 1) {
-        scan_prologue<H, NW>(io, net, b, j, s_pro, s_gi, lane, wave, false, true);
+    if (STATIC && actor_only) {
+        scan_prologue<H, NW>(io, net, b, j, obs_row, s_pro, s_gi, lane, wave, false, true);
         return;
     }
 
@@ -471,7 +471,7 @@
     float h = io.h0[net] ? io.h0[net][(int64_t)b * (io.h0_sb[net] ? io.h0_sb[net] : (int64_t)io.J * H) + (int64_t)j * H + u] : 0.0f;
 
     const bool gi_inkernel = STATIC && io.obs != nullptr;
-    if (gi_inkernel) scan_prologue<H, NW>(io, net, b, j, s_pro, s_gi, lane, wave, true, gridDim.z == 1);
+    if (gi_inkernel) scan_prologue<H, NW>(io, net, b, j, obs_row, s_pro, s_gi, lane, wave, true, actor_in_scan);
     float ring[3][3];
     if (STATIC) {
 #pragma unroll
@@ -524,6 +524,16 @@
         if (t + 1 < T) step(std::integral_constant<int, 1>{}, t + 1);
         if (t + 2 < T) step(std::integral_constant<int, 2>{}, t + 2);
     }
+}
+
+template <bool STATIC>
+__global__ void __launch_bounds__(256) gru_sequence_units_kernel(const macjd_gru_io io) {
+    __shared__ __attribute__((aligned(16))) float s_h[2][64];
+    __shared__ float s_gi[3 * 64];
+    __shared__ float s_pro[768];
+    const int seq = blockIdx.x;
+    const int64_t row = (STATIC && io.obs) ? scan_obs_row(io, seq / io.J) : 0;
+    gru_units_body<STATIC>(io, blockIdx.y, seq, row, blockIdx.z == 1, gridDim.z == 1, s_h, s_gi, s_pro);
 }
 
 }
@@ -675,13 +685,13 @@
 }
 
 namespace macjd {
-__global__ void __launch_bounds__(1024) td_mask_sum_kernel(const macjd_tdloss_io io, float* __restrict__ out) {
-    __shared__ float s_w[16];
+template <class RowOf>
+__device__ __forceinline__ void td_mask_sum_body(const macjd_tdloss_io& io, float* __restrict__ out, float* s_w, RowOf row_of) {
     const int M = io.B * io.Tm1;
     float s = 0.0f;
     for (int i = threadIdx.x; i < M; i += blockDim.x) {
         const int b = i / io.Tm1, t = i - b * io.Tm1;
-        s += io.filled[b * io.f_sb + t * io.f_st] ? 1.0f : 0.0f;
+        s += io.filled[row_of(b) * io.f_sb + t * io.f_st] ? 1.0f : 0.0f;
     }
     s = wave_sum(s);
     if ((threadIdx.x & 63) == 0) s_w[threadIdx.x >> 6] = s;
@@ -691,6 +701,11 @@
         t = wave_sum(t);
         if (threadIdx.x == 0) out[0] = t;
     }
+}
+
+__global__ void __launch_bounds__(1024) td_mask_sum_kernel(const macjd_tdloss_io io, float* __restrict__ out) {
+    __shared__ float s_w[16];
+    td_mask_sum_body(io, out, s_w, [](int b) { return (int64_t)b; });
 }
 }
 
@@ -778,34 +793,43 @@
     h ^= h >> 16; h *= 0x85ebca6bu; h ^= h >> 13; h *= 0xc2b2ae35u; h ^= h >> 16;
     return h;
 }
+struct SamplerPerm { uint32_t key[8]; int rb; uint32_t rmask, lmask; };
+__device__ __forceinline__ SamplerPerm sampler_perm(const int64_t c, const uint64_t seed, const int64_t N) {
+    const Philox4 ka = philox4x32_10((uint32_t)c, (uint32_t)((uint64_t)c >> 32), 0x53414d50u, 0u, (uint32_t)seed, (uint32_t)(seed >> 32));
+    const Philox4 kb = philox4x32_10((uint32_t)c, (uint32_t)((uint64_t)c >> 32), 0x53414d50u, 1u, (uint32_t)seed, (uint32_t)(seed >> 32));
+    SamplerPerm p;
+    p.key[0] = ka.v[0]; p.key[1] = ka.v[1]; p.key[2] = ka.v[2]; p.key[3] = ka.v[3];
+    p.key[4] = kb.v[0]; p.key[5] = kb.v[1]; p.key[6] = kb.v[2]; p.key[7] = kb.v[3];
+    int k = 2;
+    while (((int64_t)1 << k) < N) ++k;
+    const int lb = k / 2;
+    p.rb = k - k / 2;
+    p.rmask = (1u << p.rb) - 1u; p.lmask = (1u << lb) - 1u;
+    return p;
+}
+__device__ __forceinline__ int64_t sampler_index(const SamplerPerm& p, const int64_t N, const int n, const int t) {
+    if (N < n) return t % N;
+    uint32_t x = (uint32_t)t;
+    for (int walk = 0; walk < 64; ++walk) {
+        uint32_t L = x >> p.rb, R = x & p.rmask;
+#pragma unroll
+        for (int r = 0; r < 8; r += 2) {
+            L = (L ^ fmix32(R ^ p.key[r])) & p.lmask;
+            R = (R ^ fmix32(L ^ p.key[r + 1])) & p.rmask;
+        }
+        x = (L << p.rb) | R;
+        if ((int64_t)x < N) break;
+    }
+    return ((int64_t)x < N) ? (int64_t)x : (int64_t)(x % (uint32_t)N);
+}
 __device__ __forceinline__ void sample_episodes_block(const macjd_sampler_io& sp) {
-    const int64_t c = *sp.counter;
+    const int64_t c = *sp.counter + (int64_t)sp.reserved;
     const int64_t N = (int64_t)*sp.n_stored;
     __syncthreads();
     if (threadIdx.x == 0) *sp.counter = c + 1;
     if (N < 1) return;
-    const Philox4 ka = philox4x32_10((uint32_t)c, (uint32_t)((uint64_t)c >> 32), 0x53414d50u, 0u, (uint32_t)sp.seed, (uint32_t)(sp.seed >> 32));
-    const Philox4 kb = philox4x32_10((uint32_t)c, (uint32_t)((uint64_t)c >> 32), 0x53414d50u, 1u, (uint32_t)sp.seed, (uint32_t)(sp.seed >> 32));
-    const uint32_t key[8] = {ka.v[0], ka.v[1], ka.v[2], ka.v[3], kb.v[0], kb.v[1], kb.v[2], kb.v[3]};
-    int k = 2;
-    while (((int64_t)1 << k) < N) ++k;
-    const int rb = k - k / 2, lb = k / 2;
-    const uint32_t rmask = (1u << rb) - 1u, lmask = (1u << lb) - 1u;
-    for (int t = threadIdx.x; t < sp.n; t += blockDim.x) {
-        if (N < sp.n) { sp.idx_out[t] = t % N; continue; }
-        uint32_t x = (uint32_t)t;
-        for (int walk = 0; walk < 64; ++walk) {
-            uint32_t L = x >> rb, R = x & rmask;
-#pragma unroll
-            for (int r = 0; r < 8; r += 2) {
-                L = (L ^ fmix32(R ^ key[r])) & lmask;
-                R = (R ^ fmix32(L ^ key[r + 1])) & rmask;
-            }
-            x = (L << rb) | R;
-            if ((int64_t)x < N) break;
-        }
-        sp.idx_out[t] = ((int64_t)x < N) ? (int64_t)x : (int64_t)(x % (uint32_t)N);
-    }
+    const SamplerPerm perm = sampler_perm(c, sp.seed, N);
+    for (int t = threadIdx.x; t < sp.n; t += blockDim.x) sp.idx_out[t] = sampler_index(perm, N, sp.n, t);
 }
 
 __global__ void __launch_bounds__(256) sample_episodes_kernel(const macjd_sampler_io sp) { sample_episodes_block(sp); }
@@ -843,29 +867,70 @@
     if (SAMPLE && blockIdx.x == 0) sample_episodes_block(next);
 }
 
-__global__ void __launch_bounds__(256) gather_rows_kernel(const macjd_gather_io io) {
-    const int k = blockIdx.y;
-    const int row = blockIdx.z;
+__device__ __forceinline__ void gather_rows_body(const macjd_gather_io& io, const int k, const int row, const int64_t src_row,
+                                                 const int part, const int parts) {
     const int64_t words = io.row_bytes[k] >> 2;
-    const uint32_t* __restrict__ src = (const uint32_t*)((const char*)io.src[k] + io.idx[row] * io.row_bytes[k]);
+    const uint32_t* __restrict__ src = (const uint32_t*)((const char*)io.src[k] + src_row * io.row_bytes[k]);
     const int64_t dpitch = io.dst_row_bytes[k] ? io.dst_row_bytes[k] : io.row_bytes[k];
     uint32_t* __restrict__ dst = (uint32_t*)((char*)io.dst[k] + (int64_t)row * dpitch);
     const bool vec = ((io.row_bytes[k] & 15) == 0) && ((dpitch & 15) == 0) && ((((uintptr_t)io.src[k]) & 15) == 0) &&
                      ((((uintptr_t)io.dst[k]) & 15) == 0);
     if (vec) {
         const int64_t n4 = words >> 2;
-        for (int64_t i = (int64_t)blockIdx.x * blockDim.x + threadIdx.x; i < n4; i += (int64_t)gridDim.x * blockDim.x)
+        for (int64_t i = (int64_t)part * blockDim.x + threadIdx.x; i < n4; i += (int64_t)parts * blockDim.x)
             ((uint4*)dst)[i] = ((const uint4*)src)[i];
     } else {
-        for (int64_t i = (int64_t)blockIdx.x * blockDim.x + threadIdx.x; i < words; i += (int64_t)gridDim.x * blockDim.x)
+        for (int64_t i = (int64_t)part * blockDim.x + threadIdx.x; i < words; i += (int64_t)parts * blockDim.x)
             dst[i] = src[i];
     }
 }
 
+__global__ void __launch_bounds__(256) gather_rows_kernel(const macjd_gather_io io) {
+    gather_rows_body(io, blockIdx.y, blockIdx.z, io.idx[blockIdx.z], blockIdx.x, gridDim.x);
+}
+
+constexpr int PREFETCH_MAX_B = 1024;
+constexpr int PREFETCH_ROW_PARTS = 8;
+
+__global__ void __launch_bounds__(256) prefetch_batch_kernel(const macjd_prefetch_io io) {
+    __shared__ __attribute__((aligned(16))) float s_h[2][64];
+    __shared__ float s_gi[3 * 64];
+    __shared__ float s_pro[768];
+    __shared__ int64_t s_idx[PREFETCH_MAX_B];
+    __shared__ float s_w[16];
+    const int B = io.gru.B, BJ = B * io.gru.J, G = io.gather_blocks;
+    const int wg = blockIdx.x;
+    const int64_t N = (int64_t)*io.sampler.n_stored;
+    const bool draw = !io.no_draw && N >= 1;
+    SamplerPerm perm = {};
+    if (draw) perm = sampler_perm(*io.sampler.counter + (int64_t)io.sampler.reserved, io.sampler.seed, N);
+    auto index_of = [&](int t) -> int64_t { return draw ? sampler_index(perm, N, io.sampler.n, t) : io.sampler.idx_out[t]; };
+    if (wg < 2 * BJ) {
+        const bool actor_only = wg >= BJ;
+        const int seq = actor_only ? wg - BJ : wg;
+        gru_units_body<true>(io.gru, 0, seq, index_of(seq / io.gru.J), actor_only, false, s_h, s_gi, s_pro);
+    } else if (wg < 2 * BJ + G) {
+        const int n_parts = PREFETCH_ROW_PARTS * io.gather.n_tensors * B;
+        for (int v = wg - 2 * BJ; v < n_parts; v += G) {
+            const int part = v % PREFETCH_ROW_PARTS, kr = v / PREFETCH_ROW_PARTS;
+            const int k = kr % io.gather.n_tensors, row = kr / io.gather.n_tensors;
+            gather_rows_body(io.gather, k, row, index_of(row), part, PREFETCH_ROW_PARTS);
+        }
+    } else {
+        for (int t = threadIdx.x; t < B; t += blockDim.x) {
+            const int64_t e = index_of(t);
+            s_idx[t] = e;
+            if (draw) io.sampler.idx_out[t] = e;
+        }
+        __syncthreads();
+        td_mask_sum_body(io.mask, io.tot_m, s_w, [&](int b) { return s_idx[b]; });
+    }
+}
+
 }
 
 static int sampler_args_ok(const macjd_sampler_io* sp) {
-    return sp && sp->idx_out && sp->n >= 1 && sp->n_stored && sp->counter;
+    return sp && sp->idx_out && sp->n >= 1 && sp->n_stored && sp->counter && sp->reserved >= 0;
 }
 
 extern "C" int macjd_sample_episodes(const macjd_sampler_io* io, void* hip_stream) {
@@ -921,16 +986,59 @@
     return MACJD_OK;
 }
 
-extern "C" int macjd_gather_rows(const macjd_gather_io* io, void* hip_stream) {
-    using namespace macjd;
-    if (!io || io->n_tensors < 1 || io->n_tensors > 8 || io->n_rows < 0 || !io->idx)
-        return set_nets_err(MACJD_EINVAL, "macjd_gather_rows: bad argument");
+static int gather_tensors_ok(const macjd_gather_io* io) {
+    if (io->n_tensors < 1 || io->n_tensors > 8) return 0;
     for (int k = 0; k < io->n_tensors; ++k)
         if (!io->src[k] || !io->dst[k] || io->row_bytes[k] < 4 || (io->row_bytes[k] & 3) || (io->dst_row_bytes[k] & 3) ||
             (io->dst_row_bytes[k] && io->dst_row_bytes[k] < io->row_bytes[k]))
-            return set_nets_err(MACJD_EINVAL, "macjd_gather_rows: bad tensor (row bytes must be a positive multiple of 4)");
+            return 0;
+    return 1;
+}
+
+extern "C" int macjd_gather_rows(const macjd_gather_io* io, void* hip_stream) {
+    using namespace macjd;
+    if (!io || io->n_tensors < 1 || io->n_tensors > 8 || io->n_rows < 0 || !io->idx)
+        return set_nets_err(MACJD_EINVAL, "macjd_gather_rows: bad argument");
+    if (!gather_tensors_ok(io))
+        return set_nets_err(MACJD_EINVAL, "macjd_gather_rows: bad tensor (row bytes must be a positive multiple of 4)");
     if (io->n_rows == 0) return MACJD_OK;
     hipLaunchKernelGGL(gather_rows_kernel, dim3(8, io->n_tensors, io->n_rows), dim3(256), 0, (hipStream_t)hip_stream, *io);
+    hipError_t err = hipGetLastError();
+    if (err != hipSuccess) return set_nets_err(MACJD_EDEVICE, hipGetErrorString(err));
+    return MACJD_OK;
+}
+
+extern "C" int macjd_prefetch_batch_supported(int32_t n_nets, int32_t H, int32_t B) {
+    return n_nets == 1 && H == 64 && B >= 1 && B <= macjd::PREFETCH_MAX_B && !macjd::env_options().gru_ksplit;
+}
+
+extern "C" int macjd_prefetch_batch(const macjd_prefetch_io* io, void* hip_stream) {
+    using namespace macjd;
+    if (!io) return set_nets_err(MACJD_EINVAL, "macjd_prefetch_batch: NULL io");
+    const macjd_gru_io& g = io->gru;
+    if (!macjd_prefetch_batch_supported(g.n_nets, g.H, g.B))
+        return set_nets_err(MACJD_EUNSUPPORTED, "macjd_prefetch_batch: needs one network, H = 64, 1 <= B <= 1024, the unit-split scan");
+    if (g.T < 1 || g.J < 1 || !g.obs || g.S < 1 || g.S > 256 || !g.w_hh[0] || !g.b_hh[0] || !g.h_out[0] || !g.fc1_w[0] ||
+        !g.fc1_b[0] || !g.w_ih[0] || !g.b_ih[0])
+        return set_nets_err(MACJD_EINVAL, "macjd_prefetch_batch: bad scan argument");
+    if (!g.p_out[0] || g.Ah < 1 || g.Ah > 256 || g.A < 1 || g.A > 64)
+        return set_nets_err(MACJD_EINVAL, "macjd_prefetch_batch: needs the in-kernel actor (Ah <= 256, A <= 64)");
+    for (int l = 0; l < 3; ++l)
+        if (!g.act_w[0][l] || !g.act_b[0][l]) return set_nets_err(MACJD_EINVAL, "macjd_prefetch_batch: needs the actor's three layers");
+    if (!sampler_args_ok(&io->sampler) || io->sampler.n != g.B)
+        return set_nets_err(MACJD_EINVAL, "macjd_prefetch_batch: bad sampler argument (n must be the batch size)");
+    if (io->gather.n_rows != g.B || !gather_tensors_ok(&io->gather))
+        return set_nets_err(MACJD_EINVAL, "macjd_prefetch_batch: bad gather argument (n_rows must be the batch size, row bytes "
+                                          "positive multiples of 4)");
+    if (io->mask.B != g.B || io->mask.Tm1 < 1 || !io->mask.filled || !io->tot_m)
+        return set_nets_err(MACJD_EINVAL, "macjd_prefetch_batch: bad mask-sum argument");
+    if (io->gather_blocks < 0) return set_nets_err(MACJD_EINVAL, "macjd_prefetch_batch: bad gather_blocks");
+    macjd_prefetch_io a = *io;
+    const int n_parts = PREFETCH_ROW_PARTS * a.gather.n_tensors * g.B;
+    if (a.gather_blocks == 0) a.gather_blocks = 256;
+    if (a.gather_blocks > n_parts) a.gather_blocks = n_parts;
+    const unsigned grid = 2u * (unsigned)(g.B * g.J) + (unsigned)a.gather_blocks + 1u;
+    hipLaunchKernelGGL(prefetch_batch_kernel, dim3(grid), dim3(256), 0, (hipStream_t)hip_stream, a);
     hipError_t err = hipGetLastError();
     if (err != hipSuccess) return set_nets_err(MACJD_EDEVICE, hipGetErrorString(err));
     return MACJD_OK;
diff --git a/ma-cjd-cooperative-jamming-decision-making-via-marl_amd/ops.py b/ma-cjd-cooperative-jamming-decision-making-via-marl_amd/ops.py
--- a/ma-cjd-cooperative-jamming-decision-making-via-marl_amd/ops.py
+++ b/ma-cjd-cooperative-jamming-decision-making-via-marl_amd/ops.py
@@ -473,40 +473,47 @@
 
 def gru_sequence_from_obs(obs, obs_index, agents, B: int, J: int, n_steps: int, with_actor: bool = False):
     lib = _native.load()
-    assert obs.is_cuda and obs.dtype == torch.float32 and obs.dim() == 4 and obs.stride(3) == 1 and obs.shape[2] == J
     outs, pouts = [], []
     for start in range(0, len(agents), 2):
-        part = agents[start:start + 2]
-        H = part[0].rnn_hidden_dim
-        if H not in (64, 128):
-            raise _native.NativeLibraryError(f"macjd_gru_sequence supports rnn_hidden_dim 64 or 128, got {H}")
-        io = _native.GruIO()
-        io.n_nets, io.B, io.T, io.J, io.H = len(part), int(B), int(n_steps), int(J), H
-        io.obs, io.obs_sb, io.obs_sj, io.S = obs.data_ptr(), obs.stride(0), obs.stride(2), obs.shape[3]
-        if obs_index is not None:
-            assert obs_index.dtype == torch.int64 and obs_index.is_cuda and obs_index.numel() >= B
-            io.obs_index = obs_index.data_ptr()
-        keep = []
-        for k, a in enumerate(part):
-            ts = [t.detach().float().contiguous() for t in (a.rnn.weight_hh, a.rnn.bias_hh, a.fc1.weight, a.fc1.bias,
-                                                            a.rnn.weight_ih, a.rnn.bias_ih)]
-            keep += ts
-            io.w_hh[k], io.b_hh[k], io.fc1_w[k], io.fc1_b[k], io.w_ih[k], io.b_ih[k] = [t.data_ptr() for t in ts]
-            o = torch.empty((B, n_steps, J, H), dtype=torch.float32, device=obs.device)
-            io.h_out[k] = o.data_ptr()
-            outs.append(o)
-            if with_actor:
-                layers = [(w.detach().float().contiguous(), b_.detach().float().contiguous()) for w, b_, _ in a.actor_layers()]
-                keep += [t for pair in layers for t in pair]
-                for l, (w, b_) in enumerate(layers):
-                    io.act_w[k][l], io.act_b[k][l] = w.data_ptr(), b_.data_ptr()
-                io.Ah, io.A = layers[0][0].shape[0], layers[2][0].shape[0]
-                pk_ = torch.empty((B, J, io.A), dtype=torch.float32, device=obs.device)
-                io.p_out[k] = pk_.data_ptr()
-                pouts.append(pk_)
+        io, o, p_, _keep = _gru_from_obs_io(obs, obs_index, agents[start:start + 2], B, J, n_steps, with_actor)
+        outs += o
+        pouts += p_
         with torch.cuda.device(obs.device):
             _native.check(lib.macjd_gru_sequence(ctypes.byref(io), _stream(obs)), "macjd_gru_sequence")
     return (outs, pouts) if with_actor else outs
+
+
+def _gru_from_obs_io(obs, obs_index, part, B: int, J: int, n_steps: int, with_actor: bool):
+    assert obs.is_cuda and obs.dtype == torch.float32 and obs.dim() == 4 and obs.stride(3) == 1 and obs.shape[2] == J
+    outs, pouts = [], []
+    H = part[0].rnn_hidden_dim
+    if H not in (64, 128):
+        raise _native.NativeLibraryError(f"macjd_gru_sequence supports rnn_hidden_dim 64 or 128, got {H}")
+    io = _native.GruIO()
+    io.n_nets, io.B, io.T, io.J, io.H = len(part), int(B), int(n_steps), int(J), H
+    io.obs, io.obs_sb, io.obs_sj, io.S = obs.data_ptr(), obs.stride(0), obs.stride(2), obs.shape[3]
+    if obs_index is not None:
+        assert obs_index.dtype == torch.int64 and obs_index.is_cuda and obs_index.numel() >= B
+        io.obs_index = obs_index.data_ptr()
+    keep = []
+    for k, a in enumerate(part):
+        ts = [t.detach().float().contiguous() for t in (a.rnn.weight_hh, a.rnn.bias_hh, a.fc1.weight, a.fc1.bias,
+                                                        a.rnn.weight_ih, a.rnn.bias_ih)]
+        keep += ts
+        io.w_hh[k], io.b_hh[k], io.fc1_w[k], io.fc1_b[k], io.w_ih[k], io.b_ih[k] = [t.data_ptr() for t in ts]
+        o = torch.empty((B, n_steps, J, H), dtype=torch.float32, device=obs.device)
+        io.h_out[k] = o.data_ptr()
+        outs.append(o)
+        if with_actor:
+            layers = [(w.detach().float().contiguous(), b_.detach().float().contiguous()) for w, b_, _ in a.actor_layers()]
+            keep += [t for pair in layers for t in pair]
+            for l, (w, b_) in enumerate(layers):
+                io.act_w[k][l], io.act_b[k][l] = w.data_ptr(), b_.data_ptr()
+            io.Ah, io.A = layers[0][0].shape[0], layers[2][0].shape[0]
+            pk_ = torch.empty((B, J, io.A), dtype=torch.float32, device=obs.device)
+            io.p_out[k] = pk_.data_ptr()
+            pouts.append(pk_)
+    return io, outs, pouts, keep
 
 
 def gru_sequence_multi(gis, w_hhs, b_hhs, h0s=None, n_steps=None):
@@ -1058,18 +1065,19 @@
     return loss, stats[1], stats[2]
 
 
-def _sampler_io(idx_out, n_stored, counter, seed):
+def _sampler_io(idx_out, n_stored, counter, seed, offset=0):
     assert idx_out.dtype == torch.int64 and idx_out.is_contiguous() and n_stored.dtype == torch.int32 and counter.dtype == torch.int64
     assert idx_out.is_cuda and n_stored.device == idx_out.device and counter.device == idx_out.device
     sp = _native.SamplerIO()
     sp.idx_out, sp.n, sp.n_stored, sp.counter = idx_out.data_ptr(), idx_out.numel(), n_stored.data_ptr(), counter.data_ptr()
     sp.seed = int(seed) & 0xFFFFFFFFFFFFFFFF
+    sp.reserved = int(offset)
     return sp
 
 
-def sample_episodes(idx_out, n_stored, counter, seed):
-    lib = _native.load()
-    sp = _sampler_io(idx_out, n_stored, counter, seed)
+def sample_episodes(idx_out, n_stored, counter, seed, offset=0):
+    lib = _native.load()
+    sp = _sampler_io(idx_out, n_stored, counter, seed, offset)
     with torch.cuda.device(idx_out.device):
         _native.check(lib.macjd_sample_episodes(ctypes.byref(sp), _stream(idx_out)), "macjd_sample_episodes")
 
@@ -1106,16 +1114,45 @@
                                   for s in srcs)
 
 
-def gather_rows(idx, srcs, dsts):
-    lib = _native.load()
+def _gather_io(n_rows, srcs, dsts):
     io = _native.GatherIO()
-    io.n_tensors, io.n_rows, io.idx = len(srcs), idx.numel(), idx.data_ptr()
+    io.n_tensors, io.n_rows = len(srcs), int(n_rows)
     for k, (s_, d_) in enumerate(zip(srcs, dsts)):
-        assert d_.is_contiguous() and d_.dtype == s_.dtype and d_.shape[0] == idx.numel() and d_[0].numel() >= s_[0].numel()
+        assert d_.is_contiguous() and d_.dtype == s_.dtype and d_.shape[0] == n_rows and d_[0].numel() >= s_[0].numel()
         io.src[k], io.dst[k], io.row_bytes[k] = s_.data_ptr(), d_.data_ptr(), s_[0].numel() * s_.element_size()
         io.dst_row_bytes[k] = d_.stride(0) * d_.element_size()
+    return io
+
+
+def gather_rows(idx, srcs, dsts):
+    lib = _native.load()
+    io = _gather_io(idx.numel(), srcs, dsts)
+    io.idx = idx.data_ptr()
     with torch.cuda.device(idx.device):
         _native.check(lib.macjd_gather_rows(ctypes.byref(io), _stream(idx)), "macjd_gather_rows")
+
+
+def prefetch_batch_supported(agents, B: int, srcs) -> bool:
+    return (len(agents) == 1 and gather_rows_supported(srcs)
+            and bool(_native.load().macjd_prefetch_batch_supported(len(agents), int(agents[0].rnn_hidden_dim), int(B))))
+
+
+def prefetch_batch(obs, agents, B: int, J: int, n_steps: int, sampler, srcs, dsts, filled, Tm1: int, offset: int = 0,
+                   draw: bool = True, gather_blocks: int = 0):
+    lib = _native.load()
+    if not prefetch_batch_supported(agents, B, srcs):
+        raise _native.NativeLibraryError("macjd_prefetch_batch: unsupported shape (one agent body, rnn_hidden_dim 64, B <= 1024)")
+    gio, outs, pouts, _keep = _gru_from_obs_io(obs, None, agents, B, J, n_steps, True)
+    assert sampler[0].numel() == B and filled.dtype == torch.bool and filled.device == obs.device and filled.shape[1] >= Tm1
+    io = _native.PrefetchIO()
+    io.gru, io.gather, io.sampler = gio, _gather_io(B, srcs, dsts), _sampler_io(*sampler[:4], offset)
+    io.mask.B, io.mask.Tm1 = int(B), int(Tm1)
+    io.mask.filled, io.mask.f_sb, io.mask.f_st = filled.data_ptr(), filled.stride(0), filled.stride(1)
+    tot_m = torch.empty(1, dtype=torch.float32, device=obs.device)
+    io.tot_m, io.no_draw, io.gather_blocks = tot_m.data_ptr(), 0 if draw else 1, int(gather_blocks)
+    with torch.cuda.device(obs.device):
+        _native.check(lib.macjd_prefetch_batch(ctypes.byref(io), _stream(obs)), "macjd_prefetch_batch")
+    return outs, pouts, tot_m
 
 
 _DEFERRED_WGRAD = None
diff --git a/ma-cjd-cooperative-jamming-decision-making-via-marl_amd/options.py b/ma-cjd-cooperative-jamming-decision-making-via-marl_amd/options.py
--- a/ma-cjd-cooperative-jamming-decision-making-via-marl_amd/options.py
+++ b/ma-cjd-cooperative-jamming-decision-making-via-marl_amd/options.py
@@ -6,6 +6,7 @@
     "UPDATE_STREAMS": "2", "UPDATES_PER_GRAPH": "1", "PIPELINED_GROUP": "1", "SHARED_BODY": "1",
     "LEARNER_STATIC_OBS": "1", "ACTOR_IN_SCAN": "1", "DEVICE_SAMPLER": "1", "LN_IN_SQNORM": "1", "WGRAD_OUTER": "1",
     "QHEAD_TAKEN": "1", "QHEAD_DOUBLE_Q": "1", "QHEAD_DOUBLE_Q_H128": "0", "PAIRED_HEADS": "1", "MIXER_TRAIN": "1", "MIXER_STATIC_STATE": "1", "GRAPHED_ALLREDUCE": "0",
+    "PREFETCH_LAUNCH": "1",
     "CLOSED_LOOP_ROLLOUT": "0",
 }
 _values = None
```

Result: faster. 37.41 million env-steps/s (median of 6 runs) (+4.9%).
